# iDC-NEU/NeutronStarLite

Hardware: NVIDIA H100
Metric: gcn_aggregated_edges_per_sec (higher is better)
Workload: dtype f32

## Files before the change

### include/nts_b200.h

```cpp
#ifndef NTS_B200_H
#define NTS_B200_H

#include <stddef.h>
#include <stdint.h>

#ifdef __cplusplus
extern "C" {
#endif

typedef uint32_t nts_vid_t;

int nts_version(void);
const char *nts_last_error(void);
int nts_device_count(void);
int nts_set_device(int device);
int nts_device_sm_count(int *sm_count);
int nts_device_synchronize(void);
int nts_device_reset(void);

void *nts_malloc_device(size_t bytes);
int nts_free_device(void *ptr);
void *nts_malloc_pinned(size_t bytes);
int nts_free_pinned(void *ptr);
void *nts_pinned_device_pointer(void *host_ptr);
int nts_memcpy_h2d(void *dst_device, const void *src_host, size_t bytes, void *stream, int sync);
int nts_memcpy_d2h(void *dst_host, const void *src_device, size_t bytes, void *stream, int sync);
int nts_memcpy_d2d(void *dst_device, const void *src_device, size_t bytes, void *stream);
int nts_zero(void *device_ptr, size_t bytes, void *stream);

void *nts_stream_create(int non_blocking);
int nts_stream_destroy(void *stream);
int nts_stream_synchronize(void *stream);
void *nts_event_create(int with_timing);
int nts_event_destroy(void *event);
int nts_event_record(void *event, void *stream);
int nts_stream_wait_event(void *stream, void *event);
int nts_event_elapsed_ms(void *start, void *stop, float *ms);

int nts_segment_gather_sum(const float *input, float *output, const float *weight,
                           const nts_vid_t *indices, const nts_vid_t *offsets, nts_vid_t index_base,
                           nts_vid_t n_rows, uint64_t n_edges, nts_vid_t feature_size, void *stream);

int nts_gather_by_dst_from_src(const float *input, float *output, const float *weight_forward,
                               const nts_vid_t *row_indices, const nts_vid_t *column_offset,
                               nts_vid_t src_start, nts_vid_t src_end, nts_vid_t dst_start,
                               nts_vid_t dst_end, nts_vid_t edges, nts_vid_t batch_size,
                               nts_vid_t feature_size, int with_weight, void *stream);

int nts_gather_by_src_from_dst(const float *input, float *output, const float *weight_backward,
                               const nts_vid_t *row_offset, const nts_vid_t *column_indices,
                               nts_vid_t src_start, nts_vid_t src_end, nts_vid_t dst_start,
                               nts_vid_t dst_end, nts_vid_t edges, nts_vid_t batch_size,
                               nts_vid_t feature_size, int with_weight, void *stream);

int nts_segment_gather_sum_range(const float *input, float *output, const float *weight, const nts_vid_t *indices,
                                 const nts_vid_t *offsets, const nts_vid_t *slot_of, nts_vid_t index_base,
                                 nts_vid_t n_rows, uint64_t edge_begin, uint64_t edge_end, nts_vid_t feature_size,
                                 void *stream);

int nts_segment_gather_sum_bf16(const void *input, nts_vid_t input_ld, float *output, const float *weight,
                                const nts_vid_t *indices, const nts_vid_t *offsets, nts_vid_t n_rows, uint64_t n_edges,
                                nts_vid_t feature_size, void *stream);

typedef struct nts_gather_plan nts_gather_plan;
int nts_gather_plan_pick_slabs(nts_vid_t gather_rows, uint64_t n_edges, nts_vid_t n_rows, nts_vid_t feature_size,
                               uint64_t l2_budget_bytes );
nts_gather_plan *nts_gather_plan_create_hybrid(const nts_vid_t *offsets, const nts_vid_t *indices,
                                               const float *weight, const nts_vid_t *slot_of, nts_vid_t index_base,
                                               nts_vid_t n_rows, uint64_t n_edges, nts_vid_t gather_rows, int n_slabs,
                                               int n_hub_cols, int n_hub_rows, void *stream);
nts_gather_plan *nts_gather_plan_create_tuned_ex(const nts_vid_t *offsets, const nts_vid_t *indices,
                                                 const float *weight, const nts_vid_t *slot_of, nts_vid_t index_base,
                                                 nts_vid_t n_rows, uint64_t n_edges, nts_vid_t gather_rows,
                                                 nts_vid_t feature_size, int gather_dtype, int run_flags,
                                                 void *stream);
typedef struct nts_plan_part {
  const nts_vid_t *offsets, *indices;
  const float *weight;
  const nts_vid_t *slot_of;
  nts_vid_t index_base, index_add, n_rows, row_add;
  uint64_t n_edges;
} nts_plan_part;
nts_gather_plan *nts_gather_plan_create_parts(const nts_plan_part *parts, int n_parts, nts_vid_t n_rows,
                                              nts_vid_t gather_rows, int n_slabs, nts_vid_t feature_size, void *stream);
float nts_gather_plan_tuned_ms(const nts_gather_plan *plan);
int nts_gather_plan_destroy(nts_gather_plan *plan);
int nts_gather_plan_slabs(const nts_gather_plan *plan);
int nts_gather_plan_hubs(const nts_gather_plan *plan, int *cols, int *rows);
int nts_gather_plan_overlap(const nts_gather_plan *plan);
int nts_gather_plan_set_overlap(nts_gather_plan *plan, int overlap);
uint64_t nts_gather_plan_bytes(const nts_gather_plan *plan);
enum { NTS_PLAN_ACCUMULATE = 0, NTS_PLAN_OVERWRITE = 1, NTS_PLAN_COPY_INPUT = 2 };
int nts_gather_plan_run_ex(nts_gather_plan *plan, const float *input, nts_vid_t input_ld, float *output,
                           nts_vid_t feature_size, int flags, void *stream);
int nts_gather_plan_last_launch(const nts_gather_plan *plan, int *launches, int *grid, int *k, int *u, int *outv);
enum { NTS_DTYPE_F32 = 0, NTS_DTYPE_BF16 = 1 };
int nts_gather_plan_run_bf16_ex(nts_gather_plan *plan, const void *input, int input_dtype, nts_vid_t input_ld,
                                float *output, nts_vid_t feature_size, int flags, void *stream);
int nts_gather_plan_set_tuning(int u, int min_blocks, int edges_per_warp);
int nts_gather_plan_set_variant(int variant);

int nts_segment_gather_sum_slots(const float *input, float *output, const float *weight,
                                 const nts_vid_t *indices, const nts_vid_t *offsets,
                                 const nts_vid_t *slot_of, nts_vid_t n_rows, uint64_t n_edges,
                                 nts_vid_t feature_size, void *stream);

int nts_segment_gather_sum_heads(const float *input, float *output, const float *weight,
                                 const nts_vid_t *indices, const nts_vid_t *offsets, const nts_vid_t *slot_of,
                                 nts_vid_t index_base, nts_vid_t n_rows, uint64_t n_edges,
                                 nts_vid_t feature_size, nts_vid_t heads, void *stream);

int nts_aggregate_set_variant(int variant, int edges_per_warp);
int nts_aggregate_last_launch(int *grid, int *block, int *smem_bytes, int *variant);
int nts_aggregate_last_shape(int *vec, int *k, int *u, int *min_blocks, int *tiles);
uint64_t nts_kernel_launch_count(void);

int nts_scatter_src_mirror_to_msg(float *message, const float *src_mirror_feature,
                                  const nts_vid_t *row_indices, const nts_vid_t *column_offset,
                                  const nts_vid_t *mirror_index, nts_vid_t batch_size,
                                  nts_vid_t feature_size, void *stream);
int nts_gather_msg_to_src_mirror(float *src_mirror_feature, const float *message,
                                 const nts_vid_t *row_indices, const nts_vid_t *column_offset,
                                 const nts_vid_t *mirror_index, nts_vid_t batch_size,
                                 nts_vid_t feature_size, void *stream);
int nts_scatter_dst_to_msg(float *message, const float *dst_feature, const nts_vid_t *row_indices,
                           const nts_vid_t *column_offset, nts_vid_t batch_size,
                           nts_vid_t feature_size, void *stream);
int nts_gather_msg_to_dst(float *dst_feature, const float *message, const nts_vid_t *row_indices,
                          const nts_vid_t *column_offset, nts_vid_t batch_size,
                          nts_vid_t feature_size, void *stream);
int nts_edge_softmax_forward(float *msg_output, const float *msg_input, float *msg_cached,
                             const nts_vid_t *row_indices, const nts_vid_t *column_offset,
                             nts_vid_t batch_size, nts_vid_t feature_size, void *stream);
int nts_edge_softmax_backward(float *msg_input_grad, const float *msg_output_grad,
                              const float *msg_cached, const nts_vid_t *row_indices,
                              const nts_vid_t *column_offset, nts_vid_t batch_size,
                              nts_vid_t feature_size, void *stream);
int nts_scatter_grad_back_to_message(const float *input, float *message_grad,
                                     const nts_vid_t *row_indices, const nts_vid_t *column_offset,
                                     nts_vid_t batch_size, nts_vid_t feature_size, void *stream);

int nts_aggregate_dst_fuse_weight_backward(float *mirror_grad, float *edge_weight_grad,
                                           const float *mirror, const float *edge_weight,
                                           const float *dst_grad, const nts_vid_t *row_indices,
                                           const nts_vid_t *column_offset,
                                           const nts_vid_t *mirror_index, nts_vid_t batch_size,
                                           nts_vid_t feature_size, void *stream);
int nts_aggregate_dst_fuse_weight_backward_heads(float *mirror_grad, float *edge_weight_grad,
                                                 const float *mirror, const float *edge_weight,
                                                 const float *dst_grad, const nts_vid_t *row_indices,
                                                 const nts_vid_t *column_offset,
                                                 const nts_vid_t *mirror_index, nts_vid_t batch_size,
                                                 nts_vid_t feature_size, nts_vid_t heads, void *stream);

int nts_gat_softmax_stats(float *seg_max, float *seg_sum, const float *src_score, const float *dst_score,
                          const nts_vid_t *row_indices, const nts_vid_t *column_offset,
                          const nts_vid_t *mirror_index, nts_vid_t batch_size, nts_vid_t heads,
                          float negative_slope, void *stream);
int nts_gat_fused_aggregate_forward(const float *mirror, float *output, const float *src_score,
                                    const float *dst_score, const float *seg_max, const float *seg_sum,
                                    const nts_vid_t *row_indices, const nts_vid_t *column_offset,
                                    const nts_vid_t *mirror_index, nts_vid_t batch_size, uint64_t n_edges,
                                    nts_vid_t feature_size, nts_vid_t heads, float negative_slope, void *stream);
int nts_gat_fused_aggregate_backward(float *mirror_grad, float *src_score_grad, float *dst_score_grad,
                                     const float *mirror, const float *src_score, const float *dst_score,
                                     const float *seg_max, const float *seg_sum, const float *out_dot_grad,
                                     const float *dst_grad, const nts_vid_t *row_indices,
                                     const nts_vid_t *column_offset, const nts_vid_t *mirror_index,
                                     nts_vid_t batch_size, nts_vid_t feature_size, nts_vid_t heads,
                                     float negative_slope, void *stream);
int nts_gat_fused_aggregate_backward_two_pass(float *mirror_grad, float *src_score_grad, float *dst_score_grad,
                                              float *dst_pack, const float *mirror, const float *src_score,
                                              const float *dst_score, const float *seg_max, const float *seg_sum,
                                              const float *out_dot_grad, const float *dst_grad,
                                              const nts_vid_t *row_indices, const nts_vid_t *column_offset,
                                              const nts_vid_t *mirror_index, const nts_vid_t *slot_row_offset,
                                              const nts_vid_t *slot_column_indices, nts_vid_t batch_size,
                                              nts_vid_t mirror_size, nts_vid_t feature_size, nts_vid_t heads,
                                              float negative_slope, void *stream);
int nts_gat_fused_aggregate_forward_bf16(const void *mirror, float *output, const float *src_score,
                                         const float *dst_score, const float *seg_max, const float *seg_sum,
                                         const nts_vid_t *row_indices, const nts_vid_t *column_offset,
                                         const nts_vid_t *mirror_index, nts_vid_t batch_size, uint64_t n_edges,
                                         nts_vid_t feature_size, nts_vid_t ld, nts_vid_t heads, float negative_slope,
                                         void *stream);
int nts_gat_fused_aggregate_backward_two_pass_bf16(float *mirror_grad, float *src_score_grad, float *dst_score_grad,
                                                   float *dst_pack, const void *mirror, const float *src_score,
                                                   const float *dst_score, const float *seg_max, const float *seg_sum,
                                                   const float *out_dot_grad, const void *dst_grad,
                                                   const nts_vid_t *row_indices, const nts_vid_t *column_offset,
                                                   const nts_vid_t *mirror_index, const nts_vid_t *slot_row_offset,
                                                   const nts_vid_t *slot_column_indices, nts_vid_t batch_size,
                                                   nts_vid_t mirror_size, nts_vid_t feature_size, nts_vid_t ld,
                                                   nts_vid_t heads, float negative_slope, void *stream);
int nts_rows_to_bf16(const void *src, int src_dtype, nts_vid_t lds, void *dst, nts_vid_t n_rows, nts_vid_t feature_size,
                     nts_vid_t ld, void *stream);

int nts_deserialize_records(float *mirror, const float *records, nts_vid_t n_records,
                            nts_vid_t feature_size, nts_vid_t partition_start,
                            nts_vid_t partition_end, void *stream);
int nts_aggregate_records(float *aggregate, const float *records, nts_vid_t n_records,
                          nts_vid_t feature_size, nts_vid_t partition_start,
                          nts_vid_t partition_end, void *stream);

int nts_gather_rows(float *dst, const float *src, const nts_vid_t *rows, nts_vid_t n_rows,
                    nts_vid_t feature_size, void *stream);
int nts_gather_rows_sharded(float *dst, const float *const *shards, const nts_vid_t *shard_offsets, int n_shards,
                            nts_vid_t shard_pitch, const nts_vid_t *ids, nts_vid_t n, nts_vid_t feature_size,
                            void *stream);
int nts_gather_rows_sharded_bf16(void *dst, int dst_dtype, nts_vid_t dst_ld, const void *const *shards,
                                 const nts_vid_t *shard_offsets, int n_shards, nts_vid_t shard_pitch,
                                 const nts_vid_t *ids, nts_vid_t n, nts_vid_t feature_size, void *stream);
int nts_segment_gather_sum_sharded(float *output, const void *const *shards, int shard_dtype,
                                   const nts_vid_t *shard_offsets, int n_shards, nts_vid_t shard_pitch,
                                   const float *weight, const nts_vid_t *indices, const nts_vid_t *offsets,
                                   nts_vid_t n_rows, uint64_t edge_begin, uint64_t edge_end, nts_vid_t feature_size,
                                   void *stream);
int nts_gat_softmax_stats_sharded(float *seg_max, float *seg_sum, const void *const *score_shards,
                                  const nts_vid_t *shard_offsets, int n_shards, nts_vid_t score_pitch,
                                  const float *dst_score, const nts_vid_t *indices, const nts_vid_t *offsets,
                                  nts_vid_t n_rows, uint64_t edge_begin, uint64_t edge_end, nts_vid_t heads,
                                  float negative_slope, void *stream);
int nts_gat_aggregate_sharded(float *output, const void *const *shards, int shard_dtype,
                              const nts_vid_t *shard_offsets, int n_shards, nts_vid_t shard_pitch,
                              const void *const *score_shards, nts_vid_t score_pitch, const float *dst_score,
                              const float *seg_max, const float *seg_sum, const nts_vid_t *indices,
                              const nts_vid_t *offsets, nts_vid_t n_rows, uint64_t edge_begin, uint64_t edge_end,
                              nts_vid_t feature_size, nts_vid_t heads, float negative_slope, void *stream);
int nts_scatter_add_rows(float *dst, const float *src, const nts_vid_t *rows, nts_vid_t n_rows,
                         nts_vid_t feature_size, void *stream);
int nts_scatter_add_rows_atomic(float *dst, const float *src, const nts_vid_t *rows, nts_vid_t n_rows,
                                nts_vid_t feature_size, void *stream);

int nts_adam_update(float *W, float *M, float *V, const float *grad, uint64_t n, float weight_decay, float beta1,
                    float beta2, float alpha, float epsilon, void *stream);
int nts_embedding_step(float *rows, float *adam_m, float *adam_v, uint32_t *mask, uint32_t *positions,
                       uint32_t *touched, const void *const *outboxes, int n_ranks, nts_vid_t capacity,
                       nts_vid_t row_lo, nts_vid_t row_hi, nts_vid_t pitch, nts_vid_t feature_size,
                       float weight_decay, float beta1, float beta2, float alpha, float epsilon, void *stream);

#define NTS_IPC_HANDLE_BYTES 64
int nts_ipc_get_handle(void *device_ptr, unsigned char handle[NTS_IPC_HANDLE_BYTES]);
void *nts_ipc_open_handle(const unsigned char handle[NTS_IPC_HANDLE_BYTES]);
int nts_ipc_close_handle(void *peer_ptr);
int nts_signal_set(uint32_t *flag, uint32_t value, void *stream);
int nts_signal_wait_geq(const uint32_t *flag, uint32_t value, void *stream);

typedef struct nts_exchange nts_exchange;
typedef struct nts_exchange_chunk {
  const nts_vid_t *column_offset;
  const nts_vid_t *slots;
  const float *weight_forward;
  const nts_vid_t *row_offset_compact;
  const nts_vid_t *column_indices;
  const float *weight_backward;
  uint64_t edges;
} nts_exchange_chunk;
typedef struct nts_exchange_desc {
  int partitions, rank;
  nts_vid_t owned_vertices, dst_start;
  const nts_vid_t *local_column_offset, *local_row_indices, *local_row_offset, *local_column_indices;
  const float *local_weight_forward, *local_weight_backward;
  nts_vid_t local_edges;
  const nts_exchange_chunk *chunks;
  const nts_vid_t *need_count;
  const nts_vid_t *send_count;
  const nts_vid_t *send_rows_all;
  const nts_vid_t *fwd_push_offset;
  const nts_vid_t *bwd_push_offset;
  const nts_vid_t *local_need;
  nts_vid_t local_need_count;
} nts_exchange_desc;

nts_exchange *nts_exchange_create(const nts_exchange_desc *desc);
int nts_exchange_destroy(nts_exchange *ex);
uint64_t nts_exchange_required_floats(const nts_exchange *ex, nts_vid_t feature_size);
uint64_t nts_exchange_required_floats_bf16(const nts_exchange *ex, nts_vid_t feature_size);
uint64_t nts_exchange_capacity_floats(const nts_exchange *ex);
int nts_exchange_release_peers(nts_exchange *ex);
int nts_exchange_reserve(nts_exchange *ex, uint64_t floats_per_buffer, int n_buffers);
int nts_exchange_handles(nts_exchange *ex, unsigned char window_handle[64], unsigned char flags_handle[64]);
int nts_exchange_open_peers(nts_exchange *ex, const unsigned char *window_handles, const unsigned char *flag_handles);
int nts_exchange_forward(nts_exchange *ex, const float *x, float *y, nts_vid_t feature_size, void *stream);
int nts_exchange_backward(nts_exchange *ex, const float *g, float *dx, nts_vid_t feature_size, void *stream);
int nts_exchange_forward_bf16(nts_exchange *ex, const void *x, int x_dtype, float *y, nts_vid_t feature_size,
                              void *stream);
int nts_exchange_backward_bf16(nts_exchange *ex, const float *g, float *dx, nts_vid_t feature_size, void *stream);
int nts_exchange_set_trace(nts_exchange *ex, int enable);
int nts_exchange_last_timeline(nts_exchange *ex, float *ms, int capacity);
int nts_exchange_last_paths(const nts_exchange *ex, int *kind, int *epoch, int *buffer, int *mode,
                            uint32_t *kernel_peers, uint32_t *dma_peers, int *push_vec, uint32_t *plan_chunks,
                            int *bf16_staging);
int nts_exchange_fetch_mirrors(nts_exchange *ex, const float *x, float *mirror, nts_vid_t feature_size, void *stream);
int nts_exchange_return_mirror_grads(nts_exchange *ex, const float *mirror_grad, float *dx, nts_vid_t feature_size,
                                     void *stream);

typedef struct nts_host_chunk {
  const nts_vid_t *column_offset, *row_indices, *row_offset, *column_indices;
  const float *edge_weight_forward, *edge_weight_backward;
  nts_vid_t src_start, src_end, dst_start, dst_end;
  uint64_t edges;
} nts_host_chunk;
typedef struct nts_exchange_plan nts_exchange_plan;
nts_exchange_plan *nts_exchange_plan_create(const nts_host_chunk *chunks, int partitions, int rank);
void nts_exchange_plan_destroy(nts_exchange_plan *plan);
const nts_vid_t *nts_exchange_plan_need(const nts_exchange_plan *plan, int i, nts_vid_t *count);
uint64_t nts_exchange_plan_packed_rows(const nts_exchange_plan *plan);
int nts_exchange_plan_pack_needs(const nts_exchange_plan *plan, nts_vid_t *need_counts, nts_vid_t *need_rows);
int nts_exchange_plan_set_peer_needs(nts_exchange_plan *plan, int j, const nts_vid_t *need_counts,
                                     const nts_vid_t *need_rows);
int nts_exchange_plan_finalize(nts_exchange_plan *plan);
typedef struct nts_exchange_plan_view {
  int partitions, rank;
  nts_vid_t owned_vertices, recv_total, send_total, backward_rows;
  uint64_t remote_edges;
  const nts_vid_t *need_count, *send_count, *peer_bwd_offset;
  const nts_vid_t *fwd_push_offset, *bwd_push_offset;
  const nts_vid_t *remote_column_offset, *remote_slots;
  const float *remote_weight;
  const nts_vid_t *backward_offsets, *backward_indices;
  const float *backward_weight;
  const nts_vid_t *send_rows_all;
} nts_exchange_plan_view;
int nts_exchange_plan_get_view(const nts_exchange_plan *plan, nts_exchange_plan_view *view);
int nts_exchange_plan_chunk(const nts_exchange_plan *plan, int i, const nts_vid_t **slots,
                            const nts_vid_t **row_offset_compact);
typedef struct nts_device_chunk {
  const nts_vid_t *column_offset, *row_indices, *row_offset, *column_indices;
  const float *edge_weight_forward, *edge_weight_backward;
} nts_device_chunk;
nts_exchange *nts_exchange_create_from_plan(nts_exchange_plan *plan, const nts_device_chunk *device_chunks);

int nts_host_degrees(const nts_vid_t *edges_src_dst, uint64_t n_edges, nts_vid_t n_vertices,
                     nts_vid_t *out_degree, nts_vid_t *in_degree);
int nts_host_partition_offsets(const nts_vid_t *edges_src_dst, uint64_t n_edges, nts_vid_t n_vertices,
                               int partitions, nts_vid_t *partition_offset);
int nts_host_chunk_edge_counts(const nts_vid_t *edges_src_dst, uint64_t n_edges,
                               const nts_vid_t *partition_offset, int partitions, int rank,
                               uint64_t *counts);
int nts_host_build_chunk(const nts_vid_t *edges_src_dst, uint64_t n_edges, nts_vid_t n_vertices,
                         const nts_vid_t *partition_offset, int partitions, int rank, int src_partition,
                         const nts_vid_t *out_degree, const nts_vid_t *in_degree,
                         nts_vid_t *column_offset, nts_vid_t *row_indices, float *edge_weight_forward,
                         nts_vid_t *row_offset, nts_vid_t *column_indices, float *edge_weight_backward,
                         unsigned char *source_active);
int nts_host_mirror_index(const nts_vid_t *edges_src_dst, uint64_t n_edges, nts_vid_t n_vertices,
                          const nts_vid_t *partition_offset, int rank, nts_vid_t *mirror_index,
                          nts_vid_t *owned);

typedef struct nts_graph_build nts_graph_build;
enum { NTS_GRAPH_BUILD_DIST = 1 };
enum { NTS_INDEX_I32 = 0, NTS_INDEX_I64 = 1 };
nts_graph_build *nts_graph_build_from_file(const char *path, nts_vid_t n_vertices, int partitions, int rank,
                                           const nts_vid_t *partition_offset, uint64_t block_edges, int flags,
                                           void *stream);
nts_graph_build *nts_graph_build_from_device(const void *src, const void *dst, int index_dtype, uint64_t n_edges,
                                             nts_vid_t n_vertices, int partitions, int rank,
                                             const nts_vid_t *partition_offset, const void *out_degree,
                                             const void *in_degree, int flags, void *stream);
int nts_graph_build_info(const nts_graph_build *build, nts_vid_t *partition_offset, uint64_t *chunk_edges,
                         nts_vid_t *owned_mirrors, uint64_t *scratch_peak_bytes, double *pass_seconds);
int nts_graph_build_export_chunk(const nts_graph_build *build, int i, nts_vid_t *column_offset, nts_vid_t *row_indices,
                                 float *edge_weight_forward, nts_vid_t *row_offset, nts_vid_t *column_indices,
                                 float *edge_weight_backward, unsigned char *source_active, void *stream);
int nts_graph_build_export_dist(const nts_graph_build *build, nts_vid_t *mirror_index, nts_vid_t *column_offset,
                                nts_vid_t *row_indices, void *stream);
int nts_graph_build_export_degrees(const nts_graph_build *build, nts_vid_t *out_degree, nts_vid_t *in_degree,
                                   void *stream);
int nts_graph_build_destroy(nts_graph_build *build);

#define NTS_SAMPLER_INCLUDE_DST 1u
typedef struct nts_sampler nts_sampler;
typedef struct nts_sample_hop_view {
  nts_vid_t n_dst, n_src;
  uint64_t n_edges;
  const nts_vid_t *dst;
  const nts_vid_t *column_offset;
  const nts_vid_t *row_indices;
  const nts_vid_t *row_global;
  const float *weight;
  const nts_vid_t *src;
  const nts_vid_t *row_offset;
  const nts_vid_t *column_indices;
  const float *weight_backward;
} nts_sample_hop_view;
nts_sampler *nts_sampler_create(const nts_vid_t *column_offset, const nts_vid_t *row_indices, const float *edge_weight,
                                nts_vid_t n_vertices, uint64_t n_edges, nts_vid_t max_seeds, int hops,
                                const int *fanout, void *stream);
nts_sampler *nts_sampler_create_ex(const nts_vid_t *column_offset, const nts_vid_t *row_indices,
                                   const float *edge_weight, nts_vid_t n_vertices, uint64_t n_edges,
                                   nts_vid_t max_seeds, int hops, const int *fanout, uint32_t flags, void *stream);
nts_sampler *nts_sampler_create_sharded(const nts_vid_t *const *column_offsets, const nts_vid_t *const *row_indices,
                                        const float *const *edge_weights, const nts_vid_t *shard_offsets,
                                        int n_shards, nts_vid_t max_seeds, int hops, const int *fanout,
                                        uint32_t flags, void *stream);
int nts_sampler_sample(nts_sampler *sampler, const nts_vid_t *seeds, nts_vid_t n_seeds, uint64_t seed, uint64_t step,
                       void *stream);
int nts_sampler_hop_view(const nts_sampler *sampler, int hop, nts_sample_hop_view *view);
int nts_sampler_hop_dst_pos(const nts_sampler *sampler, int hop, const nts_vid_t **dst_pos);
uint64_t nts_sampler_bytes(const nts_sampler *sampler);
int nts_sampler_destroy(nts_sampler *sampler);
int nts_sample_transpose(const nts_vid_t *column_offset, const nts_vid_t *row_indices, const float *weight,
                         nts_vid_t n_dst, nts_vid_t n_src, uint64_t n_edges, nts_vid_t *row_offset,
                         nts_vid_t *column_indices, float *weight_backward, void *stream);

int nts_merge_chunk_csc(const nts_vid_t *const *column_offsets, const nts_vid_t *const *row_indices,
                        const float *const *edge_weights, int n_chunks, nts_vid_t n_dst, uint64_t n_edges,
                        nts_vid_t *column_offset, nts_vid_t *row_indices_out, float *edge_weight_out, void *stream);

int nts_host_read_feature_label_mask(const char *feature_path, const char *label_path, const char *mask_path,
                                     nts_vid_t feature_size, nts_vid_t v_begin, nts_vid_t v_end, float *features,
                                     int64_t *labels, int32_t *masks);
int nts_host_read_feature_binary(const char *path, nts_vid_t feature_size, nts_vid_t v_begin, nts_vid_t v_end,
                                 float *features);

#ifdef __cplusplus
}
#endif
#endif
```

### neutronstarlite_b200/_lib.py

```python
from __future__ import annotations

import ctypes as C
import os
import re

import numpy as np
import torch

PKG = os.path.dirname(os.path.abspath(__file__))
ROOT = os.path.dirname(PKG)
LIB_PATH = os.path.join(PKG, "lib", "libnts_b200.so")
HEADER = os.path.join(ROOT, "include", "nts_b200.h")

_vp = C.c_void_p
_u32 = C.c_uint32
_u64 = C.c_uint64
_int = C.c_int
_sz = C.c_size_t

SIGNATURES = {
    "nts_version": (_int, []),
    "nts_last_error": (C.c_char_p, []),
    "nts_device_count": (_int, []),
    "nts_set_device": (_int, [_int]),
    "nts_device_sm_count": (_int, [C.POINTER(_int)]),
    "nts_device_synchronize": (_int, []),
    "nts_device_reset": (_int, []),
    "nts_malloc_device": (_vp, [_sz]),
    "nts_free_device": (_int, [_vp]),
    "nts_malloc_pinned": (_vp, [_sz]),
    "nts_free_pinned": (_int, [_vp]),
    "nts_pinned_device_pointer": (_vp, [_vp]),
    "nts_memcpy_h2d": (_int, [_vp, _vp, _sz, _vp, _int]),
    "nts_memcpy_d2h": (_int, [_vp, _vp, _sz, _vp, _int]),
    "nts_memcpy_d2d": (_int, [_vp, _vp, _sz, _vp]),
    "nts_zero": (_int, [_vp, _sz, _vp]),
    "nts_stream_create": (_vp, [_int]),
    "nts_stream_destroy": (_int, [_vp]),
    "nts_stream_synchronize": (_int, [_vp]),
    "nts_event_create": (_vp, [_int]),
    "nts_event_destroy": (_int, [_vp]),
    "nts_event_record": (_int, [_vp, _vp]),
    "nts_stream_wait_event": (_int, [_vp, _vp]),
    "nts_event_elapsed_ms": (_int, [_vp, _vp, C.POINTER(C.c_float)]),
    "nts_segment_gather_sum": (_int, [_vp, _vp, _vp, _vp, _vp, _u32, _u32, _u64, _u32, _vp]),
    "nts_gather_by_dst_from_src": (_int, [_vp, _vp, _vp, _vp, _vp, _u32, _u32, _u32, _u32, _u32, _u32, _u32, _int, _vp]),
    "nts_gather_by_src_from_dst": (_int, [_vp, _vp, _vp, _vp, _vp, _u32, _u32, _u32, _u32, _u32, _u32, _u32, _int, _vp]),
    "nts_segment_gather_sum_range": (_int, [_vp, _vp, _vp, _vp, _vp, _vp, _u32, _u32, _u64, _u64, _u32, _vp]),
    "nts_segment_gather_sum_bf16": (_int, [_vp, _u32, _vp, _vp, _vp, _vp, _u32, _u64, _u32, _vp]),
    "nts_segment_gather_sum_sharded": (_int, [_vp, _vp, _int, _vp, _int, _u32, _vp, _vp, _vp, _u32, _u64, _u64, _u32,
                                              _vp]),
    "nts_gat_softmax_stats_sharded": (_int, [_vp, _vp, _vp, _vp, _int, _u32, _vp, _vp, _vp, _u32, _u64, _u64, _u32,
                                             C.c_float, _vp]),
    "nts_gat_aggregate_sharded": (_int, [_vp, _vp, _int, _vp, _int, _u32, _vp, _u32, _vp, _vp, _vp, _vp, _vp, _u32,
                                         _u64, _u64, _u32, _u32, C.c_float, _vp]),
    "nts_gather_plan_pick_slabs": (_int, [_u32, _u64, _u32, _u32, _u64]),
    "nts_gather_plan_create_hybrid": (_vp, [_vp, _vp, _vp, _vp, _u32, _u32, _u64, _u32, _int, _int, _int, _vp]),
    "nts_gather_plan_create_parts": (_vp, [_vp, _int, _u32, _u32, _int, _u32, _vp]),
    "nts_gather_plan_tuned_ms": (C.c_float, [_vp]),
    "nts_gather_plan_destroy": (_int, [_vp]),
    "nts_gather_plan_slabs": (_int, [_vp]),
    "nts_gather_plan_hubs": (_int, [_vp, C.POINTER(_int), C.POINTER(_int)]),
    "nts_gather_plan_overlap": (_int, [_vp]),
    "nts_gather_plan_set_overlap": (_int, [_vp, _int]),
    "nts_gather_plan_bytes": (_u64, [_vp]),
    "nts_gather_plan_run_ex": (_int, [_vp, _vp, _u32, _vp, _u32, _int, _vp]),
    "nts_gather_plan_run_bf16_ex": (_int, [_vp, _vp, _int, _u32, _vp, _u32, _int, _vp]),
    "nts_gather_plan_create_tuned_ex": (_vp, [_vp, _vp, _vp, _vp, _u32, _u32, _u64, _u32, _u32, _int, _int, _vp]),
    "nts_gather_plan_last_launch": (_int, [_vp] + [C.POINTER(_int)] * 5),
    "nts_gather_plan_set_tuning": (_int, [_int, _int, _int]),
    "nts_gather_plan_set_variant": (_int, [_int]),
    "nts_segment_gather_sum_slots": (_int, [_vp, _vp, _vp, _vp, _vp, _vp, _u32, _u64, _u32, _vp]),
    "nts_segment_gather_sum_heads": (_int, [_vp, _vp, _vp, _vp, _vp, _vp, _u32, _u32, _u64, _u32, _u32, _vp]),
    "nts_aggregate_set_variant": (_int, [_int, _int]),
    "nts_aggregate_last_launch": (_int, [C.POINTER(_int)] * 4),
    "nts_aggregate_last_shape": (_int, [C.POINTER(_int)] * 5),
    "nts_kernel_launch_count": (_u64, []),
    "nts_scatter_src_mirror_to_msg": (_int, [_vp, _vp, _vp, _vp, _vp, _u32, _u32, _vp]),
    "nts_gather_msg_to_src_mirror": (_int, [_vp, _vp, _vp, _vp, _vp, _u32, _u32, _vp]),
    "nts_scatter_dst_to_msg": (_int, [_vp, _vp, _vp, _vp, _u32, _u32, _vp]),
    "nts_gather_msg_to_dst": (_int, [_vp, _vp, _vp, _vp, _u32, _u32, _vp]),
    "nts_edge_softmax_forward": (_int, [_vp, _vp, _vp, _vp, _vp, _u32, _u32, _vp]),
    "nts_edge_softmax_backward": (_int, [_vp, _vp, _vp, _vp, _vp, _u32, _u32, _vp]),
    "nts_scatter_grad_back_to_message": (_int, [_vp, _vp, _vp, _vp, _u32, _u32, _vp]),
    "nts_aggregate_dst_fuse_weight_backward": (_int, [_vp, _vp, _vp, _vp, _vp, _vp, _vp, _vp, _u32, _u32, _vp]),
    "nts_aggregate_dst_fuse_weight_backward_heads": (_int, [_vp] * 8 + [_u32, _u32, _u32, _vp]),
    "nts_gat_softmax_stats": (_int, [_vp] * 7 + [_u32, _u32, C.c_float, _vp]),
    "nts_gat_fused_aggregate_forward": (_int, [_vp] * 9 + [_u32, _u64, _u32, _u32, C.c_float, _vp]),
    "nts_gat_fused_aggregate_backward": (_int, [_vp] * 13 + [_u32, _u32, _u32, C.c_float, _vp]),
    "nts_gat_fused_aggregate_backward_two_pass": (_int, [_vp] * 16 + [_u32, _u32, _u32, _u32, C.c_float, _vp]),
    "nts_gat_fused_aggregate_forward_bf16": (_int, [_vp] * 9 + [_u32, _u64, _u32, _u32, _u32, C.c_float, _vp]),
    "nts_gat_fused_aggregate_backward_two_pass_bf16": (_int, [_vp] * 16 + [_u32] * 5 + [C.c_float, _vp]),
    "nts_rows_to_bf16": (_int, [_vp, _int, _u32, _vp, _u32, _u32, _u32, _vp]),
    "nts_deserialize_records": (_int, [_vp, _vp, _u32, _u32, _u32, _u32, _vp]),
    "nts_aggregate_records": (_int, [_vp, _vp, _u32, _u32, _u32, _u32, _vp]),
    "nts_gather_rows": (_int, [_vp, _vp, _vp, _u32, _u32, _vp]),
    "nts_gather_rows_sharded": (_int, [_vp, _vp, _vp, _int, _u32, _vp, _u32, _u32, _vp]),
    "nts_gather_rows_sharded_bf16": (_int, [_vp, _int, _u32, _vp, _vp, _int, _u32, _vp, _u32, _u32, _vp]),
    "nts_scatter_add_rows": (_int, [_vp, _vp, _vp, _u32, _u32, _vp]),
    "nts_scatter_add_rows_atomic": (_int, [_vp, _vp, _vp, _u32, _u32, _vp]),
    "nts_ipc_get_handle": (_int, [_vp, C.c_char_p]),
    "nts_ipc_open_handle": (_vp, [C.c_char_p]),
    "nts_ipc_close_handle": (_int, [_vp]),
    "nts_adam_update": (_int, [_vp, _vp, _vp, _vp, _u64] + [C.c_float] * 5 + [_vp]),
    "nts_embedding_step": (_int, [_vp] * 7 + [_int, _u32, _u32, _u32, _u32, _u32] + [C.c_float] * 5 + [_vp]),
    "nts_signal_set": (_int, [_vp, _u32, _vp]),
    "nts_signal_wait_geq": (_int, [_vp, _u32, _vp]),
    "nts_host_degrees": (_int, [_vp, _u64, _u32, _vp, _vp]),
    "nts_host_partition_offsets": (_int, [_vp, _u64, _u32, _int, _vp]),
    "nts_host_chunk_edge_counts": (_int, [_vp, _u64, _vp, _int, _int, _vp]),
    "nts_host_build_chunk": (_int, [_vp, _u64, _u32, _vp, _int, _int, _int, _vp, _vp, _vp, _vp, _vp, _vp, _vp, _vp, _vp]),
    "nts_host_mirror_index": (_int, [_vp, _u64, _u32, _vp, _int, _vp, _vp]),
    "nts_host_read_feature_label_mask": (_int, [C.c_char_p, C.c_char_p, C.c_char_p, _u32, _u32, _u32, _vp, _vp, _vp]),
    "nts_host_read_feature_binary": (_int, [C.c_char_p, _u32, _u32, _u32, _vp]),
    "nts_graph_build_from_file": (_vp, [C.c_char_p, _u32, _int, _int, _vp, _u64, _int, _vp]),
    "nts_graph_build_from_device": (_vp, [_vp, _vp, _int, _u64, _u32, _int, _int, _vp, _vp, _vp, _int, _vp]),
    "nts_graph_build_info": (_int, [_vp] * 6),
    "nts_graph_build_export_chunk": (_int, [_vp, _int] + [_vp] * 8),
    "nts_graph_build_export_dist": (_int, [_vp] * 5),
    "nts_graph_build_export_degrees": (_int, [_vp] * 4),
    "nts_graph_build_destroy": (_int, [_vp]),
}



class ExchangeChunk(C.Structure):
    _fields_ = [
        ("column_offset", _vp), ("slots", _vp), ("weight_forward", _vp), ("row_offset_compact", _vp),
        ("column_indices", _vp), ("weight_backward", _vp), ("edges", _u64),
    ]


class ExchangeDesc(C.Structure):
    _fields_ = [
        ("partitions", _int), ("rank", _int), ("owned_vertices", _u32), ("dst_start", _u32),
        ("local_column_offset", _vp), ("local_row_indices", _vp), ("local_row_offset", _vp),
        ("local_column_indices", _vp), ("local_weight_forward", _vp), ("local_weight_backward", _vp),
        ("local_edges", _u32),
        ("chunks", C.POINTER(ExchangeChunk)),
        ("need_count", C.POINTER(_u32)), ("send_count", C.POINTER(_u32)),
        ("send_rows_all", _vp), ("fwd_push_offset", C.POINTER(_u32)), ("bwd_push_offset", C.POINTER(_u32)),
        ("local_need", _vp), ("local_need_count", _u32),
    ]


class DeviceChunk(C.Structure):
    _fields_ = [
        ("column_offset", _vp), ("row_indices", _vp), ("row_offset", _vp), ("column_indices", _vp),
        ("edge_weight_forward", _vp), ("edge_weight_backward", _vp),
    ]


SIGNATURES.update({
    "nts_exchange_create": (_vp, [C.POINTER(ExchangeDesc)]),
    "nts_exchange_destroy": (_int, [_vp]),
    "nts_exchange_required_floats": (_u64, [_vp, _u32]),
    "nts_exchange_capacity_floats": (_u64, [_vp]),
    "nts_exchange_release_peers": (_int, [_vp]),
    "nts_exchange_reserve": (_int, [_vp, _u64, _int]),
    "nts_exchange_handles": (_int, [_vp, C.c_char_p, C.c_char_p]),
    "nts_exchange_open_peers": (_int, [_vp, C.c_char_p, C.c_char_p]),
    "nts_exchange_forward": (_int, [_vp, _vp, _vp, _u32, _vp]),
    "nts_exchange_backward": (_int, [_vp, _vp, _vp, _u32, _vp]),
    "nts_exchange_forward_bf16": (_int, [_vp, _vp, _int, _vp, _u32, _vp]),
    "nts_exchange_backward_bf16": (_int, [_vp, _vp, _vp, _u32, _vp]),
    "nts_exchange_required_floats_bf16": (_u64, [_vp, _u32]),
    "nts_exchange_set_trace": (_int, [_vp, _int]),
    "nts_exchange_last_timeline": (_int, [_vp, C.POINTER(C.c_float), _int]),
    "nts_exchange_last_paths": (_int, [_vp] + [C.POINTER(_int)] * 4 + [C.POINTER(_u32)] * 2 +
                                [C.POINTER(_int), C.POINTER(_u32), C.POINTER(_int)]),
    "nts_exchange_fetch_mirrors": (_int, [_vp, _vp, _vp, _u32, _vp]),
    "nts_exchange_return_mirror_grads": (_int, [_vp, _vp, _vp, _u32, _vp]),
})



class HostChunk(C.Structure):
    _fields_ = [
        ("column_offset", _vp), ("row_indices", _vp), ("row_offset", _vp), ("column_indices", _vp),
        ("edge_weight_forward", _vp), ("edge_weight_backward", _vp),
        ("src_start", _u32), ("src_end", _u32), ("dst_start", _u32), ("dst_end", _u32), ("edges", _u64),
    ]


class ExchangePlanView(C.Structure):
    _fields_ = [
        ("partitions", _int), ("rank", _int),
        ("owned_vertices", _u32), ("recv_total", _u32), ("send_total", _u32), ("backward_rows", _u32),
        ("remote_edges", _u64),
        ("need_count", C.POINTER(_u32)), ("send_count", C.POINTER(_u32)), ("peer_bwd_offset", C.POINTER(_u32)),
        ("fwd_push_offset", C.POINTER(_u32)), ("bwd_push_offset", C.POINTER(_u32)),
        ("remote_column_offset", C.POINTER(_u32)), ("remote_slots", C.POINTER(_u32)),
        ("remote_weight", C.POINTER(C.c_float)),
        ("backward_offsets", C.POINTER(_u32)), ("backward_indices", C.POINTER(_u32)),
        ("backward_weight", C.POINTER(C.c_float)),
        ("send_rows_all", C.POINTER(_u32)),
    ]


SIGNATURES.update({
    "nts_exchange_plan_create": (_vp, [C.POINTER(HostChunk), _int, _int]),
    "nts_exchange_plan_destroy": (None, [_vp]),
    "nts_exchange_plan_need": (C.POINTER(_u32), [_vp, _int, C.POINTER(_u32)]),
    "nts_exchange_plan_packed_rows": (_u64, [_vp]),
    "nts_exchange_plan_pack_needs": (_int, [_vp, _vp, _vp]),
    "nts_exchange_plan_set_peer_needs": (_int, [_vp, _int, _vp, _vp]),
    "nts_exchange_plan_finalize": (_int, [_vp]),
    "nts_exchange_plan_get_view": (_int, [_vp, C.POINTER(ExchangePlanView)]),
    "nts_exchange_plan_chunk": (_int, [_vp, _int, C.POINTER(C.POINTER(_u32)), C.POINTER(C.POINTER(_u32))]),
    "nts_exchange_create_from_plan": (_vp, [_vp, C.POINTER(DeviceChunk)]),
})


class SampleHopView(C.Structure):
    _fields_ = [
        ("n_dst", _u32), ("n_src", _u32), ("n_edges", _u64),
        ("dst", _vp), ("column_offset", _vp), ("row_indices", _vp), ("row_global", _vp), ("weight", _vp),
        ("src", _vp), ("row_offset", _vp), ("column_indices", _vp), ("weight_backward", _vp),
    ]


SIGNATURES.update({
    "nts_sampler_create": (_vp, [_vp, _vp, _vp, _u32, _u64, _u32, _int, C.POINTER(_int), _vp]),
    "nts_sampler_create_ex": (_vp, [_vp, _vp, _vp, _u32, _u64, _u32, _int, C.POINTER(_int), _u32, _vp]),
    "nts_sampler_sample": (_int, [_vp, _vp, _u32, _u64, _u64, _vp]),
    "nts_sampler_hop_view": (_int, [_vp, _int, C.POINTER(SampleHopView)]),
    "nts_sampler_hop_dst_pos": (_int, [_vp, _int, C.POINTER(_vp)]),
    "nts_sampler_bytes": (_u64, [_vp]),
    "nts_sampler_destroy": (_int, [_vp]),
    "nts_sample_transpose": (_int, [_vp, _vp, _vp, _u32, _u32, _u64, _vp, _vp, _vp, _vp]),
    "nts_sampler_create_sharded": (_vp, [C.POINTER(_vp), C.POINTER(_vp), C.POINTER(_vp), C.POINTER(_u32), _int, _u32,
                                         _int, C.POINTER(_int), _u32, _vp]),
    "nts_merge_chunk_csc": (_int, [C.POINTER(_vp), C.POINTER(_vp), C.POINTER(_vp), _int, _u32, _u64, _vp, _vp, _vp,
                                   _vp]),
})

_lib = None


class NtsError(RuntimeError):
    pass


def header_symbols():
    text = open(HEADER).read()
    text = re.sub(r"/\*.*?\*/", "", text, flags=re.S)
    return sorted(set(re.findall(r"\b(nts_[a-z0-9_]+)\s*\(", text)))


def load():
    global _lib
    if _lib is not None:
        return _lib
    if not os.path.exists(LIB_PATH):
        raise NtsError("libnts_b200.so not found at %s - run `python -m neutronstarlite_b200.build` "
                       "(there is no CPU fallback)" % LIB_PATH)
    lib = C.CDLL(LIB_PATH, mode=C.RTLD_GLOBAL)
    for name, (res, args) in SIGNATURES.items():
        fn = getattr(lib, name)
        fn.restype = res
        fn.argtypes = args
    _lib = lib
    return lib


def last_error():
    return load().nts_last_error().decode(errors="replace")


def check(rc, what=""):
    if rc != 0:
        raise NtsError("libnts_b200 %s failed (rc=%d): %s" % (what, rc, last_error()))


def call(name, *args):
    rc = getattr(load(), name)(*args)
    check(rc, name)


def checked(handle, what):
    if not handle:
        raise NtsError("%s failed: %s" % (what, last_error()))
    return handle


def stream(device=None):
    return torch.cuda.current_stream(device).cuda_stream


class _DeviceArray:

    def __init__(self, ptr, n, typestr):
        self.__cuda_array_interface__ = {"shape": (int(n),), "typestr": typestr, "data": (int(ptr), False),
                                         "version": 2, "strides": None}


_TYPESTR = {torch.int32: "<i4", torch.float32: "<f4"}


def borrowed(ptr, n, dtype, device):
    if n == 0:
        return torch.empty(0, dtype=dtype, device=device)
    return torch.as_tensor(_DeviceArray(ptr, n, _TYPESTR[dtype]), device=device)


def device_ids(ids, bound, device, name, what):
    if torch.is_tensor(ids) and ids.is_cuda:
        if ids.dtype.is_floating_point or ids.dtype.is_complex or ids.dtype == torch.bool:
            raise NtsError("%s must be an integer tensor, not %s" % (name, ids.dtype))
        if ids.numel() and (int(ids.min()) < 0 or int(ids.max()) >= bound):
            raise NtsError("%s must be in [0, %d)" % (what, bound))
        return ids.reshape(-1).to(device=device, dtype=torch.int32).contiguous()
    a = np.asarray(ids.numpy() if torch.is_tensor(ids) else ids).reshape(-1).astype(np.int64)
    if a.size and (a.min() < 0 or a.max() >= bound):
        raise NtsError("%s must be in [0, %d)" % (what, bound))
    return torch.from_numpy(a.astype(np.int32)).to(device)
```

### neutronstarlite_b200/csrc/nts_plan.cu

```cuda
#include <cub/cub.cuh>
#include <cuda_bf16.h>

#include <algorithm>
#include <type_traits>
#include <vector>

#include "nts_common.cuh"

struct nts_gather_plan {
  uint32_t n_rows = 0;
  uint64_t n_edges = 0;
  uint32_t gather_rows = 0;
  int slabs = 1;
  uint32_t slab_rows = 0;
  uint2 *pairs = nullptr;
  uint32_t *voff = nullptr;
  std::vector<uint64_t> slab_edge;
  float *workspace = nullptr;
  size_t workspace_floats = 0;
  __nv_bfloat16 *workspace_bf16 = nullptr;
  size_t workspace_bf16_elems = 0;
  int hub_cols = 0, hub_rows = 0;
  uint32_t *hub_col_ids = nullptr;
  uint32_t *hub_row_ids = nullptr;
  uint32_t lda_c = 0, lda_r = 0;
  float *dense = nullptr;
  size_t dense_floats = 0;
  int overlap = 0;
  int last_grid = 0, last_launches = 0, last_k = 0, last_u = 0, last_outv = 0;
  float tuned_ms = 0.f;
};

namespace nts {

static int g_plan_u = 0, g_plan_minb = 0, g_plan_q = 0, g_plan_variant = 0;

__device__ __forceinline__ uint32_t plan_gathered_row(const nts_plan_part &pt, uint32_t e) {
  const uint32_t id = __ldg(pt.indices + e);
  return (pt.slot_of ? __ldg(pt.slot_of + id) : id - pt.index_base) + pt.index_add;
}

constexpr uint32_t kNoHub = 0xffffffffu;

template <class KeyT>
__global__ void plan_keys_kernel(nts_plan_part pt, uint32_t e_off, uint32_t n_rows, uint32_t slab_rows, uint32_t slabs,
                                 const uint32_t *__restrict__ col_slot, const uint32_t *__restrict__ row_slot,
                                 uint32_t lda_c, uint64_t dc_cells, uint32_t lda_r, KeyT *__restrict__ key,
                                 uint32_t *__restrict__ val) {
  for (uint64_t e = (uint64_t)blockIdx.x * blockDim.x + threadIdx.x; e < pt.n_edges; e += (uint64_t)gridDim.x * blockDim.x) {
    const uint32_t r = find_row(pt.offsets, pt.n_rows, (uint32_t)e) + pt.row_add;
    const uint32_t g = plan_gathered_row(pt, (uint32_t)e);
    uint32_t s = g / slab_rows;
    if (s >= slabs)
      s = slabs - 1;
    KeyT k = (KeyT)s * n_rows + r;
    if constexpr (sizeof(KeyT) == 8) {
      const uint64_t n_keys = (uint64_t)slabs * n_rows;
      const uint32_t cs = __ldg(col_slot + g), rs = __ldg(row_slot + r);
      if (cs != kNoHub)
        k = n_keys + (uint64_t)cs * lda_c + r;
      else if (rs != kNoHub)
        k = n_keys + dc_cells + (uint64_t)g * lda_r + rs;
    }
    key[e_off + e] = k;
    val[e_off + e] = e_off + (uint32_t)e;
  }
}

__global__ void plan_pairs_kernel(const uint32_t *__restrict__ perm, const nts_plan_part *__restrict__ parts,
                                  uint32_t n_edges, uint2 *__restrict__ pairs) {
  for (uint64_t i = (uint64_t)blockIdx.x * blockDim.x + threadIdx.x; i < n_edges; i += (uint64_t)gridDim.x * blockDim.x) {
    uint32_t e = perm ? __ldg(perm + i) : (uint32_t)i;
    const nts_plan_part *pt = parts;
    for (; e >= pt->n_edges; pt++)
      e -= (uint32_t)pt->n_edges;
    const float wt = pt->weight ? __ldg(pt->weight + e) : 1.f;
    pairs[i] = make_uint2(plan_gathered_row(*pt, e), __float_as_uint(wt));
  }
}

template <class KeyT>
__global__ void plan_offsets_kernel(const KeyT *__restrict__ sorted_key, uint32_t n_edges, uint32_t n_keys,
                                    uint32_t *__restrict__ voff) {
  for (uint64_t k = (uint64_t)blockIdx.x * blockDim.x + threadIdx.x; k <= n_keys; k += (uint64_t)gridDim.x * blockDim.x) {
    uint32_t lo = 0, hi = n_edges;
    while (lo < hi) {
      uint32_t mid = lo + ((hi - lo) >> 1);
      if (__ldg(sorted_key + mid) < (KeyT)k)
        lo = mid + 1;
      else
        hi = mid;
    }
    voff[k] = lo;
  }
}

__global__ void plan_ref_count_kernel(const uint32_t *__restrict__ idx, const uint32_t *__restrict__ slot_of,
                                      uint32_t base, uint32_t n_edges, uint32_t *__restrict__ cnt) {
  for (uint64_t e = (uint64_t)blockIdx.x * blockDim.x + threadIdx.x; e < n_edges; e += (uint64_t)gridDim.x * blockDim.x) {
    const uint32_t id = __ldg(idx + e);
    atomicAdd(cnt + (slot_of ? __ldg(slot_of + id) : id - base), 1u);
  }
}

__global__ void plan_cell_sum_kernel(const uint64_t *__restrict__ cell_key, const uint32_t *__restrict__ run_start,
                                     const uint32_t *__restrict__ run_len, uint32_t n_runs,
                                     const uint32_t *__restrict__ perm, const float *__restrict__ w, uint64_t n_keys,
                                     float *__restrict__ dense) {
  const uint32_t lane = threadIdx.x & 31;
  for (uint64_t run = ((uint64_t)blockIdx.x * blockDim.x + threadIdx.x) >> 5; run < n_runs;
       run += ((uint64_t)gridDim.x * blockDim.x) >> 5) {
    const uint32_t b = __ldg(run_start + run), n = __ldg(run_len + run);
    float s = 0.f;
    for (uint32_t j = lane; j < n; j += 32)
      s += w ? __ldg(w + __ldg(perm + b + j)) : 1.f;
#pragma unroll
    for (int o = 16; o > 0; o >>= 1)
      s += __shfl_xor_sync(0xffffffffu, s, o);
    if (lane == 0)
      dense[__ldg(cell_key + run) - n_keys] = s;
  }
}

__global__ void pad_rows_kernel(const float *__restrict__ src, uint32_t lds, float *__restrict__ dst, uint32_t n_rows,
                                uint32_t F, uint32_t ld) {
  const uint64_t total = (uint64_t)n_rows * ld;
  for (uint64_t i = (uint64_t)blockIdx.x * blockDim.x + threadIdx.x; i < total; i += (uint64_t)gridDim.x * blockDim.x) {
    const uint64_t r = i / ld;
    const uint32_t c = (uint32_t)(i - r * ld);
    dst[i] = c < F ? __ldg(src + r * lds + c) : 0.f;
  }
}

template <class S>
__global__ void bf16_rows_kernel(const S *__restrict__ src, uint32_t lds, uint4 *__restrict__ dst, uint32_t n_rows,
                                 uint32_t F, uint32_t ld) {
  const uint32_t ld8 = ld / 8;
  const uint64_t total = (uint64_t)n_rows * ld8;
  for (uint64_t i = (uint64_t)blockIdx.x * blockDim.x + threadIdx.x; i < total; i += (uint64_t)gridDim.x * blockDim.x) {
    const uint64_t r = i / ld8;
    const uint32_t c = (uint32_t)(i - r * ld8) * 8;
    const S *s = src + r * lds;
    uint32_t w[4];
#pragma unroll
    for (int j = 0; j < 4; j++) {
      const uint32_t c0 = c + 2 * j, c1 = c0 + 1;
      if constexpr (std::is_same<S, float>::value) {
        const __nv_bfloat162 h = __floats2bfloat162_rn(c0 < F ? __ldg(s + c0) : 0.f, c1 < F ? __ldg(s + c1) : 0.f);
        w[j] = *reinterpret_cast<const uint32_t *>(&h);
      } else {
        const uint16_t *u = reinterpret_cast<const uint16_t *>(s);
        w[j] = (c0 < F ? (uint32_t)__ldg(u + c0) : 0u) | ((c1 < F ? (uint32_t)__ldg(u + c1) : 0u) << 16);
      }
    }
    dst[i] = make_uint4(w[0], w[1], w[2], w[3]);
  }
}

constexpr int kPlanWarps = 8;

template <int OUTV, bool ATOMIC>
__device__ __forceinline__ void flush_chunk(float *__restrict__ orow, uint32_t col, uint32_t F, float4 a) {
  if constexpr (OUTV == 4) {
    float4 *p = reinterpret_cast<float4 *>(orow + col);
    if constexpr (ATOMIC) {
      asm volatile("red.global.add.v4.f32 [%0], {%1, %2, %3, %4};" ::"l"(p), "f"(a.x), "f"(a.y), "f"(a.z), "f"(a.w)
                   : "memory");
    } else {
      float4 o = *p;
      o.x += a.x, o.y += a.y, o.z += a.z, o.w += a.w;
      *p = o;
    }
  } else if constexpr (OUTV == 2) {
    float2 *p = reinterpret_cast<float2 *>(orow + col);
    if constexpr (ATOMIC) {
      asm volatile("red.global.add.v2.f32 [%0], {%1, %2};" ::"l"(p), "f"(a.x), "f"(a.y) : "memory");
      if (col + 2 < F)
        asm volatile("red.global.add.v2.f32 [%0], {%1, %2};" ::"l"(p + 1), "f"(a.z), "f"(a.w) : "memory");
    } else {
      float2 o = p[0];
      o.x += a.x, o.y += a.y;
      p[0] = o;
      if (col + 2 < F) {
        float2 o1 = p[1];
        o1.x += a.z, o1.y += a.w;
        p[1] = o1;
      }
    }
  } else {
    const float v[4] = {a.x, a.y, a.z, a.w};
#pragma unroll
    for (int i = 0; i < 4; i++)
      if (col + i < F) {
        if constexpr (ATOMIC)
          atomicAdd(orow + col + i, v[i]);
        else
          orow[col + i] += v[i];
      }
  }
}

template <class T> struct GatherT;
template <> struct GatherT<float> {
  using chunk = float4;
  static constexpr int V = 4;
  __device__ static __forceinline__ void widen(const float4 &c, float (&v)[4]) {
    v[0] = c.x, v[1] = c.y, v[2] = c.z, v[3] = c.w;
  }
};
template <> struct GatherT<__nv_bfloat16> {
  using chunk = uint4;
  static constexpr int V = 8;
  __device__ static __forceinline__ void widen(const uint4 &c, float (&v)[8]) {
    const uint32_t u[4] = {c.x, c.y, c.z, c.w};
#pragma unroll
    for (int i = 0; i < 4; i++) {
      v[2 * i] = __uint_as_float(u[i] << 16);
      v[2 * i + 1] = __uint_as_float(u[i] & 0xffff0000u);
    }
  }
};

template <class T, int K, int U, int OUTV, int G>
__device__ __forceinline__ void planned_gather_body(unsigned char *smem_raw, uint32_t vblock,
                                                    const typename GatherT<T>::chunk *__restrict__ in, uint32_t ldc,
                                                    float *__restrict__ out, uint32_t F,
                                                    const uint2 *__restrict__ pairs, const uint32_t *__restrict__ off,
                                                    uint32_t n_rows, uint32_t e_begin, uint32_t e_end, uint32_t Q,
                                                    uint32_t tiles, uint32_t tile_vecs) {
  static_assert(G == 1 || K == 1, "virtual warps are for rows narrower than a warp");
  using Chunk = typename GatherT<T>::chunk;
  constexpr int V = GatherT<T>::V;
  constexpr uint32_t GS = 32 / G;
  const uint32_t lane = threadIdx.x & (GS - 1);
  const uint32_t vwarp_in_block = threadIdx.x / GS;
  const uint64_t gwarp = (uint64_t)vblock * (kPlanWarps * G) + vwarp_in_block;
  const uint32_t tile = (uint32_t)(gwarp % tiles);
  const uint64_t q = gwarp / tiles;
  const uint64_t e0_64 = e_begin + q * (uint64_t)Q;

  uint64_t *bar = reinterpret_cast<uint64_t *>(smem_raw);
  uint2 *s_pair = reinterpret_cast<uint2 *>(smem_raw + 16);
  uint32_t cta_e_base = 0, bulk_bytes = 0;
  {
    const uint64_t cta_w0 = (uint64_t)vblock * (kPlanWarps * G);
    const uint64_t first_q = cta_w0 / tiles;
    const uint64_t last_q = (cta_w0 + kPlanWarps * G - 1) / tiles;
    uint64_t ce0 = e_begin + first_q * (uint64_t)Q;
    uint64_t ce1 = e_begin + (last_q + 1) * (uint64_t)Q;
    if (ce1 > e_end)
      ce1 = e_end;
    if (ce0 < ce1) {
      cta_e_base = (uint32_t)(ce0 & ~1ull);
      const uint32_t n_el = (uint32_t)(ce1 - cta_e_base);
      bulk_bytes = (n_el * 8u) & ~15u;
      if (threadIdx.x == 0) {
        mbar_init(bar, 1);
        asm volatile("fence.mbarrier_init.release.cluster;" ::: "memory");
        if (n_el & 1u)
          s_pair[n_el - 1] = __ldg(pairs + cta_e_base + n_el - 1);
      }
      __syncthreads();
      if (threadIdx.x == 0 && bulk_bytes) {
        mbar_expect_tx(bar, bulk_bytes);
        bulk_g2s(s_pair, pairs + cta_e_base, bulk_bytes, bar);
      }
    }
  }
  if (e0_64 >= e_end)
    return;
  const uint32_t e0 = (uint32_t)e0_64;
  const uint32_t e1 = (e0_64 + Q < e_end) ? e0 + Q : e_end;

  const uint32_t c0 = tile * tile_vecs + lane;
  bool act[K];
#pragma unroll
  for (int k = 0; k < K; k++)
    act[k] = (k * GS + lane) < tile_vecs && (c0 + k * GS) < ldc;

  uint32_t row = find_row(off, n_rows, e0);
  uint32_t row_end = __ldg(off + row + 1);
  bool row_started_inside = __ldg(off + row) >= e0;

  float acc[K][V];
#pragma unroll
  for (int k = 0; k < K; k++)
#pragma unroll
    for (int j = 0; j < V; j++)
      acc[k][j] = 0.f;

  auto flush = [&](bool whole) {
    float *orow = out + (size_t)row * F;
#pragma unroll
    for (int k = 0; k < K; k++) {
#pragma unroll
      for (int h = 0; h < V; h += 4) {
        const uint32_t col = (c0 + k * GS) * V + h;
        const float4 a = make_float4(acc[k][h], acc[k][h + 1], acc[k][h + 2], acc[k][h + 3]);
        if (act[k] && col < F) {
          if (whole)
            flush_chunk<OUTV, false>(orow, col, F, a);
          else
            flush_chunk<OUTV, true>(orow, col, F, a);
        }
      }
#pragma unroll
      for (int j = 0; j < V; j++)
        acc[k][j] = 0.f;
    }
  };
  auto advance = [&](uint32_t ee) {
    flush(row_started_inside);
    do {
      row++;
      row_end = __ldg(off + row + 1);
    } while (ee >= row_end);
    row_started_inside = true;
  };

  if (bulk_bytes)
    mbar_wait(bar, 0);

  const uint2 *sp = s_pair - cta_e_base;
  uint32_t e = e0;
  auto fma_chunk = [&](int k, float w, const Chunk &c) {
    float x[V];
    GatherT<T>::widen(c, x);
#pragma unroll
    for (int j = 0; j < V; j++)
      acc[k][j] = fmaf(w, x[j], acc[k][j]);
  };
  for (; e + U <= e1; e += U) {
    Chunk v[U][K];
    float wu[U];
#pragma unroll
    for (int u = 0; u < U; u++) {
      const uint2 pr = sp[e + u];
      wu[u] = __uint_as_float(pr.y);
      const Chunk *p = in + (size_t)pr.x * ldc + c0;
#pragma unroll
      for (int k = 0; k < K; k++)
        if (act[k])
          v[u][k] = __ldg(p + k * GS);
    }
#pragma unroll
    for (int u = 0; u < U; u++) {
      if (e + u >= row_end)
        advance(e + u);
#pragma unroll
      for (int k = 0; k < K; k++)
        if (act[k])
          fma_chunk(k, wu[u], v[u][k]);
    }
  }
  for (; e < e1; e++) {
    const uint2 pr = sp[e];
    const float wj = __uint_as_float(pr.y);
    const Chunk *p = in + (size_t)pr.x * ldc + c0;
    Chunk v1[K];
#pragma unroll
    for (int k = 0; k < K; k++)
      if (act[k])
        v1[k] = __ldg(p + k * GS);
    if (e >= row_end)
      advance(e);
#pragma unroll
    for (int k = 0; k < K; k++)
      if (act[k])
        fma_chunk(k, wj, v1[k]);
  }
  flush(row_started_inside && row_end <= e1);
}

template <class T, int K, int U, int OUTV, int MINB, int G = 1>
__global__ void __launch_bounds__(kPlanWarps * 32, MINB)
    planned_gather_sum_kernel(const typename GatherT<T>::chunk *__restrict__ in, uint32_t ldc, float *__restrict__ out,
                              uint32_t F, const uint2 *__restrict__ pairs, const uint32_t *__restrict__ off,
                              uint32_t n_rows, uint32_t e_begin, uint32_t e_end, uint32_t Q, uint32_t tiles,
                              uint32_t tile_vecs) {
  extern __shared__ __align__(16) unsigned char smem_raw[];
  planned_gather_body<T, K, U, OUTV, G>(smem_raw, blockIdx.x, in, ldc, out, F, pairs, off, n_rows, e_begin, e_end, Q,
                                        tiles, tile_vecs);
}

struct PlanShape;
template <int K, int STAGES, int OUTV, int MINB>
__global__ void __launch_bounds__(kPlanWarps * 32, MINB)
    planned_gather_sum_tma_kernel(const float4 *__restrict__ in, uint32_t ld4, float *__restrict__ out, uint32_t F,
                                  const uint2 *__restrict__ pairs, const uint32_t *__restrict__ off, uint32_t n_rows,
                                  uint32_t e_begin, uint32_t e_end, uint32_t Q, uint32_t tiles, uint32_t tile_vecs,
                                  uint32_t pair_bytes) {
  const uint32_t lane = threadIdx.x & 31;
  const uint32_t warp_in_block = threadIdx.x >> 5;
  const uint64_t gwarp = (uint64_t)blockIdx.x * kPlanWarps + warp_in_block;
  const uint32_t tile = (uint32_t)(gwarp % tiles);
  const uint64_t q = gwarp / tiles;
  const uint64_t e0_64 = e_begin + q * (uint64_t)Q;

  extern __shared__ __align__(16) unsigned char smem_raw[];
  uint64_t *bar = reinterpret_cast<uint64_t *>(smem_raw);
  uint2 *s_pair = reinterpret_cast<uint2 *>(smem_raw + 16);
  const uint32_t ring_bytes = 8u * STAGES + 8u * (STAGES & 1) + STAGES * tile_vecs * 16u;
  unsigned char *ring = smem_raw + 16 + pair_bytes + (size_t)warp_in_block * ring_bytes;
  uint64_t *sbar = reinterpret_cast<uint64_t *>(ring);
  float4 *sbuf = reinterpret_cast<float4 *>(ring + 8u * STAGES + 8u * (STAGES & 1));
  uint32_t cta_e_base = 0, bulk_bytes = 0;
  {
    const uint64_t cta_w0 = (uint64_t)blockIdx.x * kPlanWarps;
    const uint64_t first_q = cta_w0 / tiles;
    const uint64_t last_q = (cta_w0 + kPlanWarps - 1) / tiles;
    uint64_t ce0 = e_begin + first_q * (uint64_t)Q;
    uint64_t ce1 = e_begin + (last_q + 1) * (uint64_t)Q;
    if (ce1 > e_end)
      ce1 = e_end;
    if (lane == 0)
      for (int s = 0; s < STAGES; s++)
        mbar_init(sbar + s, 1);
    if (ce0 < ce1) {
      cta_e_base = (uint32_t)(ce0 & ~1ull);
      const uint32_t n_el = (uint32_t)(ce1 - cta_e_base);
      bulk_bytes = (n_el * 8u) & ~15u;
      if (threadIdx.x == 0) {
        mbar_init(bar, 1);
        if (n_el & 1u)
          s_pair[n_el - 1] = __ldg(pairs + cta_e_base + n_el - 1);
      }
    }
    asm volatile("fence.mbarrier_init.release.cluster;" ::: "memory");
    __syncthreads();
    if (threadIdx.x == 0 && bulk_bytes) {
      mbar_expect_tx(bar, bulk_bytes);
      bulk_g2s(s_pair, pairs + cta_e_base, bulk_bytes, bar);
    }
  }
  if (e0_64 >= e_end)
    return;
  const uint32_t e0 = (uint32_t)e0_64;
  const uint32_t e1 = (e0_64 + Q < e_end) ? e0 + Q : e_end;
  const uint32_t c0 = tile * tile_vecs + lane;
  const uint32_t my_vecs = min(tile_vecs, ld4 - tile * tile_vecs);
  const uint32_t row_bytes = my_vecs * 16u;
  bool act[K];
#pragma unroll
  for (int k = 0; k < K; k++)
    act[k] = (k * 32 + lane) < my_vecs;

  uint32_t row = find_row(off, n_rows, e0);
  uint32_t row_end = __ldg(off + row + 1);
  bool row_started_inside = __ldg(off + row) >= e0;
  float4 acc[K];
#pragma unroll
  for (int k = 0; k < K; k++)
    zero_vec(acc[k]);
  auto flush = [&](bool whole) {
    float *orow = out + (size_t)row * F;
#pragma unroll
    for (int k = 0; k < K; k++) {
      const uint32_t col = (c0 + k * 32) * 4;
      if (act[k] && col < F) {
        if (whole)
          flush_chunk<OUTV, false>(orow, col, F, acc[k]);
        else
          flush_chunk<OUTV, true>(orow, col, F, acc[k]);
      }
      zero_vec(acc[k]);
    }
  };
  auto advance = [&](uint32_t ee) {
    flush(row_started_inside);
    do {
      row++;
      row_end = __ldg(off + row + 1);
    } while (ee >= row_end);
    row_started_inside = true;
  };
  if (bulk_bytes)
    mbar_wait(bar, 0);
  const uint2 *sp = s_pair - cta_e_base;
  auto issue = [&](uint32_t e, uint32_t stage) {
    const uint32_t src_row = sp[e].x;
    mbar_expect_tx(sbar + stage, row_bytes);
    bulk_g2s(sbuf + (size_t)stage * tile_vecs, in + (size_t)src_row * ld4 + tile * tile_vecs, row_bytes, sbar + stage);
  };
  if (lane == 0)
    for (uint32_t s = 0; s < STAGES && e0 + s < e1; s++)
      issue(e0 + s, s);
  uint32_t stage = 0, parity = 0;
  for (uint32_t e = e0; e < e1; e++) {
    const float w = __uint_as_float(sp[e].y);
    mbar_wait(sbar + stage, parity);
    const float4 *b = sbuf + (size_t)stage * tile_vecs + lane;
    float4 v[K];
#pragma unroll
    for (int k = 0; k < K; k++)
      if (act[k])
        v[k] = b[k * 32];
    if (e >= row_end)
      advance(e);
#pragma unroll
    for (int k = 0; k < K; k++)
      if (act[k])
        fma_vec(acc[k], w, v[k]);
    __syncwarp();
    if (lane == 0 && e + STAGES < e1)
      issue(e + STAGES, stage);
    if (++stage == STAGES) {
      stage = 0;
      parity ^= 1u;
    }
  }
  flush(row_started_inside && row_end <= e1);
}

template <int K, int STAGES, int OUTV, int MINB>
static int launch_planned_tma(nts_gather_plan *pl, const PlanShape &sh, const float4 *in, uint32_t ld4, float *out,
                              uint32_t F, uint32_t Q, cudaStream_t st);

struct PlanShape {
  int k, u, outv, minb, g;
  uint32_t tiles, tile_vecs;
};

template <class T, int K, int U, int OUTV, int MINB, int G = 1>
static int launch_planned(nts_gather_plan *pl, const PlanShape &sh, const T *in_rows, uint32_t ldc, float *out,
                          uint32_t F, uint32_t Q, cudaStream_t st) {
  auto kern = planned_gather_sum_kernel<T, K, U, OUTV, MINB, G>;
  const auto *in = reinterpret_cast<const typename GatherT<T>::chunk *>(in_rows);
  const size_t smem = 16 + ((size_t)kPlanWarps * G * Q + 4) * 8;
  NTS_CUDA_OK(cudaFuncSetAttribute(kern, cudaFuncAttributeMaxDynamicSharedMemorySize, (int)smem));
  pl->last_launches = 0;
  for (int s = 0; s < pl->slabs; s++) {
    const uint64_t eb = pl->slab_edge[s], ee = pl->slab_edge[s + 1];
    if (ee <= eb)
      continue;
    const uint64_t quanta = (ee - eb + Q - 1) / Q;
    const uint64_t blocks = (quanta * sh.tiles + kPlanWarps * G - 1) / (kPlanWarps * G);
    NTS_ARG_CHECK(blocks <= 0x7fffffffull, "aggregation grid too large");
    kern<<<(unsigned)blocks, kPlanWarps * 32, smem, st>>>(in, ldc, out, F, pl->pairs, pl->voff + (size_t)s * pl->n_rows,
                                                          pl->n_rows, (uint32_t)eb, (uint32_t)ee, Q, sh.tiles,
                                                          sh.tile_vecs);
    NTS_LAUNCH_CHECK();
    pl->last_grid = (int)blocks;
    pl->last_launches++;
  }
  return 0;
}

template <int K, int STAGES, int OUTV, int MINB>
static int launch_planned_tma(nts_gather_plan *pl, const PlanShape &sh, const float4 *in, uint32_t ld4, float *out,
                              uint32_t F, uint32_t Q, cudaStream_t st) {
  auto kern = planned_gather_sum_tma_kernel<K, STAGES, OUTV, MINB>;
  const uint32_t pair_bytes = (kPlanWarps * Q + 4) * 8;
  const uint32_t ring_bytes = 8u * STAGES + 8u * (STAGES & 1) + STAGES * sh.tile_vecs * 16u;
  const size_t smem = 16 + pair_bytes + (size_t)kPlanWarps * ring_bytes;
  NTS_ARG_CHECK(smem <= 227 * 1024, "row-staging ring does not fit shared memory");
  NTS_CUDA_OK(cudaFuncSetAttribute(kern, cudaFuncAttributeMaxDynamicSharedMemorySize, (int)smem));
  pl->last_launches = 0;
  for (int s = 0; s < pl->slabs; s++) {
    const uint64_t eb = pl->slab_edge[s], ee = pl->slab_edge[s + 1];
    if (ee <= eb)
      continue;
    const uint64_t quanta = (ee - eb + Q - 1) / Q;
    const uint64_t blocks = (quanta * sh.tiles + kPlanWarps - 1) / kPlanWarps;
    NTS_ARG_CHECK(blocks <= 0x7fffffffull, "aggregation grid too large");
    kern<<<(unsigned)blocks, kPlanWarps * 32, smem, st>>>(in, ld4, out, F, pl->pairs, pl->voff + (size_t)s * pl->n_rows,
                                                          pl->n_rows, (uint32_t)eb, (uint32_t)ee, Q, sh.tiles,
                                                          sh.tile_vecs, pair_bytes);
    NTS_LAUNCH_CHECK();
    pl->last_grid = (int)blocks;
    pl->last_launches++;
  }
  return 0;
}

#define NTS_PLAN_TMA_CASE(K_, S_, B_)                                                                               \
  if (sh.k == K_ && stages == S_ && sh.minb == B_) {                                                                \
    if (sh.outv == 4)                                                                                               \
      return launch_planned_tma<K_, S_, 4, B_>(pl, sh, in4, ld4, out, F, Q, st);                                    \
    if (sh.outv == 2)                                                                                               \
      return launch_planned_tma<K_, S_, 2, B_>(pl, sh, in4, ld4, out, F, Q, st);                                    \
    return launch_planned_tma<K_, S_, 1, B_>(pl, sh, in4, ld4, out, F, Q, st);                                      \
  }

#define NTS_PLAN_CASE_G(U_, B_, G_)                                                                                 \
  if (sh.k == 1 && sh.u == U_ && sh.minb == B_ && sh.g == G_) {                                                     \
    if (sh.outv == 4)                                                                                               \
      return launch_planned<T, 1, U_, 4, B_, G_>(pl, sh, in, ldc, out, F, Q, st);                                   \
    if (sh.outv == 2)                                                                                               \
      return launch_planned<T, 1, U_, 2, B_, G_>(pl, sh, in, ldc, out, F, Q, st);                                   \
    return launch_planned<T, 1, U_, 1, B_, G_>(pl, sh, in, ldc, out, F, Q, st);                                     \
  }

#define NTS_PLAN_CASE(K_, U_, B_)                                                                                   \
  if (sh.k == K_ && sh.u == U_ && sh.minb == B_) {                                                                  \
    if (sh.outv == 4)                                                                                               \
      return launch_planned<T, K_, U_, 4, B_>(pl, sh, in, ldc, out, F, Q, st);                                       \
    if (sh.outv == 2)                                                                                               \
      return launch_planned<T, K_, U_, 2, B_>(pl, sh, in, ldc, out, F, Q, st);                                       \
    return launch_planned<T, K_, U_, 1, B_>(pl, sh, in, ldc, out, F, Q, st);                                         \
  }

constexpr int kHubBM = 128, kHubBN = 128, kHubBK = 16, kHubThreads = 256;

__device__ __forceinline__ void p_cp_async16(void *smem_dst, const void *gmem_src, bool full) {
  asm volatile("cp.async.cg.shared.global [%0], [%1], 16, %2;" ::"r"(smem_u32(smem_dst)), "l"(gmem_src),
               "r"(full ? 16 : 0)
               : "memory");
}

template <int TN, class TB> struct HubSmem {
  static constexpr uint32_t kBN = 16 * TN;
  float As[2][kHubBK][kHubBM];
  TB Bs[2][kHubBK][kBN];
};

template <class TB, int OUTV, bool SPLIT, bool STORE, int TN, int KKU>
__device__ __forceinline__ void hub_gemm_tile(HubSmem<TN, TB> &sm, uint32_t tile, const float *__restrict__ At,
                                              uint32_t lda, uint32_t M, uint32_t k_lo, uint32_t k_hi, uint32_t k_split,
                                              const TB *__restrict__ B, uint32_t ldb,
                                              const uint32_t *__restrict__ colmap, float *__restrict__ out, uint32_t F,
                                              const uint32_t *__restrict__ rowmap, uint32_t m_tiles, uint32_t n_tiles) {
  static_assert(!(SPLIT && STORE), "split-K partials must be added, not stored");
  constexpr bool kBf16 = std::is_same<TB, __nv_bfloat16>::value;
  constexpr uint32_t kBV = 16 / sizeof(TB);
  constexpr uint32_t kBN = HubSmem<TN, TB>::kBN;
  constexpr uint32_t kBChunks = kHubBK * kBN / kBV;
  auto &As = sm.As;
  auto &Bs = sm.Bs;
  const uint32_t t = threadIdx.x;
  const uint32_t n_tile = tile % n_tiles, rest = tile / n_tiles;
  const uint32_t m0 = (rest % m_tiles) * kHubBM, n0 = n_tile * kBN;
  const uint32_t k_begin = k_lo + (rest / m_tiles) * k_split;
  const uint32_t k_end = min(k_hi, k_begin + k_split);
  if (k_begin >= k_end)
    return;
  const uint32_t n_kt = (k_end - k_begin + kHubBK - 1) / kHubBK;

  auto load = [&](uint32_t kt, int buf) {
#pragma unroll
    for (int i = 0; i < 2; i++) {
      const uint32_t c = t + i * kHubThreads, kk = c >> 5, c4 = (c & 31) * 4;
      const uint32_t k = k_begin + kt * kHubBK + kk;
      const bool a_ok = k < k_end && m0 + c4 < lda;
      p_cp_async16(&As[buf][kk][c4], a_ok ? At + (size_t)k * lda + m0 + c4 : At, a_ok);
    }
#pragma unroll
    for (int i = 0; i < (int)((kBChunks + kHubThreads - 1) / kHubThreads); i++) {
      constexpr uint32_t kRowChunks = kBN / kBV;
      const uint32_t c = t + i * kHubThreads, kk = c / kRowChunks, cv = (c % kRowChunks) * kBV;
      if (kBChunks % kHubThreads != 0 && c >= kBChunks)
        break;
      const uint32_t k = k_begin + kt * kHubBK + kk;
      const bool b_ok = k < k_end && n0 + cv < ldb;
      const uint32_t brow = b_ok ? (colmap ? __ldg(colmap + k) : k) : 0;
      p_cp_async16(&Bs[buf][kk][cv], B + (size_t)brow * ldb + (b_ok ? n0 + cv : 0), b_ok);
    }
    asm volatile("cp.async.commit_group;" ::: "memory");
  };
  auto read_b4 = [&](int buf, int kk, uint32_t n) -> float4 {
    if constexpr (kBf16) {
      const uint2 u = *reinterpret_cast<const uint2 *>(&Bs[buf][kk][n]);
      return make_float4(__uint_as_float(u.x << 16), __uint_as_float(u.x & 0xffff0000u), __uint_as_float(u.y << 16),
                         __uint_as_float(u.y & 0xffff0000u));
    } else {
      return *reinterpret_cast<const float4 *>(&Bs[buf][kk][n]);
    }
  };

  const uint32_t tx = t & 15, ty = t >> 4;
  float acc[8][TN];
#pragma unroll
  for (int i = 0; i < 8; i++)
#pragma unroll
    for (int j = 0; j < TN; j++)
      acc[i][j] = 0.f;

  load(0, 0);
  for (uint32_t kt = 0; kt < n_kt; kt++) {
    const int buf = kt & 1;
    if (kt + 1 < n_kt) {
      load(kt + 1, buf ^ 1);
      asm volatile("cp.async.wait_group 1;" ::: "memory");
    } else {
      asm volatile("cp.async.wait_group 0;" ::: "memory");
    }
    __syncthreads();
#pragma unroll(KKU)
    for (int kk = 0; kk < kHubBK; kk++) {
      const float4 a0 = *reinterpret_cast<const float4 *>(&As[buf][kk][ty * 4]);
      const float4 a1 = *reinterpret_cast<const float4 *>(&As[buf][kk][64 + ty * 4]);
      const float a[8] = {a0.x, a0.y, a0.z, a0.w, a1.x, a1.y, a1.z, a1.w};
      float b[TN];
#pragma unroll
      for (int h = 0; h < TN / 4; h++) {
        const float4 bh = read_b4(buf, kk, h * 64 + tx * 4);
        b[4 * h] = bh.x, b[4 * h + 1] = bh.y, b[4 * h + 2] = bh.z, b[4 * h + 3] = bh.w;
      }
#pragma unroll
      for (int i = 0; i < 8; i++)
#pragma unroll
        for (int j = 0; j < TN; j++)
          acc[i][j] = fmaf(a[i], b[j], acc[i][j]);
    }
    __syncthreads();
  }

#pragma unroll
  for (int i = 0; i < 8; i++) {
    const uint32_t m = m0 + (i >> 2) * 64 + ty * 4 + (i & 3);
    if (m >= M)
      continue;
    float *orow = out + (size_t)(rowmap ? __ldg(rowmap + m) : m) * F;
#pragma unroll
    for (int j = 0; j < TN / 4; j++) {
      const uint32_t col = n0 + j * 64 + tx * 4;
      const float4 a = make_float4(acc[i][j * 4], acc[i][j * 4 + 1], acc[i][j * 4 + 2], acc[i][j * 4 + 3]);
      if (col < F) {
        if constexpr (STORE)
          store_chunk_checked<OUTV>(orow, col, F, a);
        else
          flush_chunk<OUTV, SPLIT>(orow, col, F, a);
      }
    }
  }
}

template <class TB, int OUTV, bool SPLIT, bool STORE>
__global__ void __launch_bounds__(kHubThreads, 2)
    hub_block_gemm_kernel(const float *__restrict__ At, uint32_t lda, uint32_t M, uint32_t K, uint32_t k_split,
                          const TB *__restrict__ B, uint32_t ldb, const uint32_t *__restrict__ colmap,
                          float *__restrict__ out, uint32_t F, const uint32_t *__restrict__ rowmap, uint32_t m_tiles,
                          uint32_t n_tiles) {
  __shared__ __align__(16) HubSmem<8, TB> sm;
  hub_gemm_tile<TB, OUTV, SPLIT, STORE, 8, kHubBK>(sm, blockIdx.x, At, lda, M, 0, K, k_split, B, ldb, colmap, out, F,
                                                   rowmap, m_tiles, n_tiles);
}

static uint32_t hub_row_k_split(uint32_t K, uint32_t m_tiles, uint32_t n_tiles) {
  const uint64_t want = (uint64_t)sm_count() * 2 * 4;
  const uint64_t splits = (want + (uint64_t)m_tiles * n_tiles - 1) / ((uint64_t)m_tiles * n_tiles);
  const uint32_t k_split = (uint32_t)((K + splits - 1) / splits);
  return std::max<uint32_t>((k_split + kHubBK - 1) / kHubBK * kHubBK, 16 * kHubBK);
}

template <class TB, int OUTV>
static int launch_hub_blocks(nts_gather_plan *pl, const TB *in, uint32_t ldb, float *out, uint32_t F, bool rows,
                             bool overwrite, cudaStream_t st) {
  const uint32_t n_tiles = (F + kHubBN - 1) / kHubBN;
  if (pl->hub_cols) {
    const uint32_t m_tiles = (pl->n_rows + kHubBM - 1) / kHubBM;
    const uint64_t blocks = (uint64_t)m_tiles * n_tiles;
    NTS_ARG_CHECK(blocks <= 0x7fffffffull, "hub column block grid too large");
    auto kern = overwrite ? hub_block_gemm_kernel<TB, OUTV, false, true> : hub_block_gemm_kernel<TB, OUTV, false, false>;
    kern<<<(unsigned)blocks, kHubThreads, 0, st>>>(pl->dense, pl->lda_c, pl->n_rows, (uint32_t)pl->hub_cols,
                                                   (uint32_t)pl->hub_cols, in, ldb, pl->hub_col_ids, out, F, nullptr,
                                                   m_tiles, n_tiles);
    NTS_LAUNCH_CHECK();
  }
  if (pl->hub_rows && rows) {
    const uint32_t m_tiles = (pl->hub_rows + kHubBM - 1) / kHubBM;
    const uint32_t K = pl->gather_rows;
    const uint32_t k_split = hub_row_k_split(K, m_tiles, n_tiles);
    const uint64_t splits = (K + k_split - 1) / k_split;
    hub_block_gemm_kernel<TB, OUTV, true, false><<<(unsigned)(splits * m_tiles * n_tiles), kHubThreads, 0, st>>>(
        pl->dense + (size_t)pl->hub_cols * pl->lda_c, pl->lda_r, (uint32_t)pl->hub_rows, K, k_split, in, ldb, nullptr,
        out, F, pl->hub_row_ids, m_tiles, n_tiles);
    NTS_LAUNCH_CHECK();
  }
  return 0;
}

struct HubRowArgs {
  const float *At;
  uint32_t lda, M;
  uint32_t k_lo, k_hi, k_split;
  const uint32_t *rowmap;
  uint32_t m_tiles, n_tiles, n_gemm;
  uint32_t period;
};

template <class T, int K, int U, int OUTV, int MINB, int G>
__global__ void __launch_bounds__(kPlanWarps * 32, MINB)
    planned_slab_hub_kernel(const typename GatherT<T>::chunk *__restrict__ in, uint32_t ldc, float *__restrict__ out,
                            uint32_t F, const uint2 *__restrict__ pairs, const uint32_t *__restrict__ off,
                            uint32_t n_rows, uint32_t e_begin, uint32_t e_end, uint32_t Q, uint32_t tiles,
                            uint32_t tile_vecs, const HubRowArgs hub) {
  static_assert(kPlanWarps * 32 == kHubThreads, "both bodies run 256 threads");
  constexpr int TN = MINB <= 2 ? 8 : 4;
  extern __shared__ __align__(16) unsigned char smem_raw[];
  const uint32_t b = blockIdx.x, grp = b / hub.period;
  if (grp < hub.n_gemm && b - grp * hub.period == hub.period - 1)
    hub_gemm_tile<T, OUTV, true, false, TN, TN == 8 ? kHubBK : 4>(
        *reinterpret_cast<HubSmem<TN, T> *>(smem_raw), grp, hub.At, hub.lda, hub.M, hub.k_lo, hub.k_hi, hub.k_split,
        reinterpret_cast<const T *>(in), ldc * GatherT<T>::V, nullptr, out, F, hub.rowmap, hub.m_tiles, hub.n_tiles);
  else
    planned_gather_body<T, K, U, OUTV, G>(smem_raw, b - min(grp, hub.n_gemm), in, ldc, out, F, pairs, off, n_rows,
                                          e_begin, e_end, Q, tiles, tile_vecs);
}

template <class T, int K, int U, int OUTV, int MINB, int G = 1>
static int launch_fused(nts_gather_plan *pl, const PlanShape &sh, const T *in_rows, uint32_t ldc, float *out,
                        uint32_t F, uint32_t Q, cudaStream_t st) {
  constexpr int TN = MINB <= 2 ? 8 : 4;
  auto kern = planned_slab_hub_kernel<T, K, U, OUTV, MINB, G>;
  const auto *in = reinterpret_cast<const typename GatherT<T>::chunk *>(in_rows);
  const size_t smem = std::max(16 + ((size_t)kPlanWarps * G * Q + 4) * 8, sizeof(HubSmem<TN, T>));
  NTS_CUDA_OK(cudaFuncSetAttribute(kern, cudaFuncAttributeMaxDynamicSharedMemorySize, (int)smem));
  HubRowArgs hub;
  hub.At = pl->dense + (size_t)pl->hub_cols * pl->lda_c;
  hub.lda = pl->lda_r;
  hub.M = (uint32_t)pl->hub_rows;
  hub.rowmap = pl->hub_row_ids;
  hub.m_tiles = (hub.M + kHubBM - 1) / kHubBM;
  hub.n_tiles = (F + 16 * TN - 1) / (16 * TN);
  hub.k_split = hub_row_k_split(pl->gather_rows, hub.m_tiles, hub.n_tiles);
  pl->last_launches = 0;
  for (int s = 0; s < pl->slabs; s++) {
    hub.k_lo = (uint32_t)std::min<uint64_t>((uint64_t)s * pl->slab_rows, pl->gather_rows);
    hub.k_hi = s + 1 == pl->slabs ? pl->gather_rows
                                  : (uint32_t)std::min<uint64_t>((uint64_t)(s + 1) * pl->slab_rows, pl->gather_rows);
    const uint64_t splits = hub.k_hi > hub.k_lo ? (hub.k_hi - hub.k_lo + hub.k_split - 1) / hub.k_split : 0;
    const uint64_t n_gemm = splits * hub.m_tiles * hub.n_tiles;
    const uint64_t eb = pl->slab_edge[s], ee = pl->slab_edge[s + 1];
    const uint64_t quanta = ee > eb ? (ee - eb + Q - 1) / Q : 0;
    const uint64_t blocks = n_gemm + (quanta * sh.tiles + kPlanWarps * G - 1) / (kPlanWarps * G);
    if (!blocks)
      continue;
    NTS_ARG_CHECK(blocks <= 0x7fffffffull, "aggregation grid too large");
    hub.n_gemm = (uint32_t)n_gemm;
    hub.period = n_gemm ? (uint32_t)(blocks / n_gemm) : 1;
    kern<<<(unsigned)blocks, kPlanWarps * 32, smem, st>>>(in, ldc, out, F, pl->pairs, pl->voff + (size_t)s * pl->n_rows,
                                                          pl->n_rows, (uint32_t)eb, (uint32_t)ee, Q, sh.tiles,
                                                          sh.tile_vecs, hub);
    NTS_LAUNCH_CHECK();
    pl->last_grid = (int)blocks;
    pl->last_launches++;
  }
  return 0;
}

#define NTS_PLAN_FUSED_CASE(K_, U_, B_, G_)                                                                         \
  if (sh.k == K_ && sh.u == U_ && sh.minb == B_ && sh.g == G_) {                                                    \
    if (sh.outv == 4)                                                                                               \
      return launch_fused<T, K_, U_, 4, B_, G_>(pl, sh, in, ldc, out, F, Q, st);                                    \
    if (sh.outv == 2)                                                                                               \
      return launch_fused<T, K_, U_, 2, B_, G_>(pl, sh, in, ldc, out, F, Q, st);                                    \
    return launch_fused<T, K_, U_, 1, B_, G_>(pl, sh, in, ldc, out, F, Q, st);                                      \
  }

template <class T>
static int run_gather(nts_gather_plan *pl, const T *in, uint32_t ld, float *output, uint32_t F, bool overwrite,
                      cudaStream_t st) {
  constexpr bool kBf16 = std::is_same<T, __nv_bfloat16>::value;
  PlanShape sh;
  const uint32_t ldc = ld / GatherT<T>::V;
  const uint32_t chunks = (ldc + 31) / 32;
  const uint32_t kmax = 5;
  sh.tiles = (chunks + kmax - 1) / kmax;
  sh.tile_vecs = (ldc + sh.tiles - 1) / sh.tiles;
  sh.k = (int)((sh.tile_vecs + 31) / 32);
  sh.tiles = (ldc + sh.tile_vecs - 1) / sh.tile_vecs;
  sh.outv = pick_vec(F, output);
  const bool fused = pl->overlap && pl->hub_rows;
  NTS_ARG_CHECK(!fused || g_plan_variant == 0, "the fused slab launches use the register-staging gather (variant 0)");
  if (overwrite && !pl->hub_cols)
    NTS_CUDA_OK(cudaMemsetAsync(output, 0, (size_t)pl->n_rows * F * sizeof(float), st));
  if (pl->hub_cols || pl->hub_rows) {
    const int rc = sh.outv == 4   ? launch_hub_blocks<T, 4>(pl, in, ld, output, F, !fused, overwrite, st)
                   : sh.outv == 2 ? launch_hub_blocks<T, 2>(pl, in, ld, output, F, !fused, overwrite, st)
                                  : launch_hub_blocks<T, 1>(pl, in, ld, output, F, !fused, overwrite, st);
    if (rc)
      return rc;
  }
  sh.g = ldc <= 8 ? 4 : (ldc <= 16 ? 2 : 1);
  if (g_plan_variant == 1 || getenv("NTS_PLAN_NO_SUBWARP"))
    sh.g = 1;
  sh.minb = sh.k >= 3 ? 2 : (sh.k == 2 ? 3 : 4);
  sh.u = sh.k == 4 ? 2 : 4;
  if constexpr (kBf16) {
    sh.minb = sh.k >= 4 ? 2 : (sh.k >= 2 ? 3 : 4);
    sh.u = sh.k == 1 ? 4 : 2;
  }
  {
    static int env_read = 0;
    if (!env_read) {
      env_read = 1;
      if (const char *t = getenv("NTS_PLAN_TUNE"))
        sscanf(t, "%d,%d,%d", &g_plan_u, &g_plan_minb, &g_plan_q);
    }
    if (g_plan_u > 0)
      sh.u = g_plan_u;
    if (g_plan_minb > 0)
      sh.minb = g_plan_minb;
  }
  uint32_t Q = g_plan_q > 0 ? (uint32_t)g_plan_q : 512u / sh.g;
  if (g_plan_q <= 0) {
    const uint64_t per_slab = pl->slab_edge[pl->slabs] / (uint64_t)pl->slabs + 1;
    const uint64_t want_warps = (uint64_t)sm_count() * 64 * sh.g;
    while (Q > 32 && ((per_slab + Q - 1) / Q) * sh.tiles < want_warps)
      Q >>= 1;
  }
  Q = (Q + 31u) & ~31u;
  if (Q * sh.g > 1024)
    Q = (1024 / sh.g) & ~31u;
  pl->last_k = sh.k, pl->last_u = sh.u, pl->last_outv = sh.outv;
  float *out = output;
  if (fused) {
    if constexpr (kBf16) {
      NTS_PLAN_FUSED_CASE(1, 4, 4, 2)
      NTS_PLAN_FUSED_CASE(1, 4, 4, 4)
      NTS_PLAN_FUSED_CASE(1, 4, 4, 1)
      NTS_PLAN_FUSED_CASE(2, 2, 3, 1)
      NTS_PLAN_FUSED_CASE(3, 2, 3, 1)
      NTS_PLAN_FUSED_CASE(4, 2, 2, 1)
      NTS_PLAN_FUSED_CASE(5, 2, 2, 1)
    } else {
      NTS_PLAN_FUSED_CASE(1, 4, 4, 2)
      NTS_PLAN_FUSED_CASE(1, 4, 4, 4)
      NTS_PLAN_FUSED_CASE(1, 4, 4, 1)
      NTS_PLAN_FUSED_CASE(2, 4, 3, 1)
      NTS_PLAN_FUSED_CASE(3, 4, 2, 1)
      NTS_PLAN_FUSED_CASE(4, 2, 2, 1)
      NTS_PLAN_FUSED_CASE(5, 4, 2, 1)
    }
    return fail(-1, "no fused slab/hub-row instantiation for this (chunks, U, occupancy) point", __FILE__, __LINE__);
  }
  if constexpr (kBf16) {
    NTS_PLAN_CASE_G(4, 4, 2)
    NTS_PLAN_CASE_G(4, 4, 4)
    NTS_PLAN_CASE_G(8, 2, 2)
    NTS_PLAN_CASE_G(8, 2, 4)
    if (sh.g != 1)
      return fail(-1, "no BF16 virtual-warp instantiation for this (U, occupancy) point", __FILE__, __LINE__);
    NTS_PLAN_CASE(1, 4, 4)
    NTS_PLAN_CASE(1, 8, 2)
    NTS_PLAN_CASE(2, 2, 3)
    NTS_PLAN_CASE(2, 4, 2)
    NTS_PLAN_CASE(3, 4, 2)
    NTS_PLAN_CASE(3, 2, 3)
    NTS_PLAN_CASE(3, 6, 1)
    NTS_PLAN_CASE(4, 2, 2)
    NTS_PLAN_CASE(4, 4, 2)
    NTS_PLAN_CASE(5, 2, 2)
    return fail(-1, "no BF16 planned-aggregation instantiation for this (chunks, U, occupancy) point", __FILE__,
                __LINE__);
  } else {
  const float4 *in4 = reinterpret_cast<const float4 *>(in);
  const uint32_t ld4 = ldc;
  if (g_plan_variant == 1) {
    const int stages = sh.u >= 8 ? 8 : (sh.u >= 4 ? 4 : 2);
    NTS_PLAN_TMA_CASE(1, 8, 4)
    NTS_PLAN_TMA_CASE(1, 4, 4)
    NTS_PLAN_TMA_CASE(1, 8, 3)
    NTS_PLAN_TMA_CASE(2, 4, 3)
    NTS_PLAN_TMA_CASE(2, 4, 2)
    NTS_PLAN_TMA_CASE(3, 4, 2)
    NTS_PLAN_TMA_CASE(4, 4, 2)
    NTS_PLAN_TMA_CASE(4, 2, 2)
    NTS_PLAN_TMA_CASE(5, 4, 2)
    NTS_PLAN_TMA_CASE(5, 2, 2)
    NTS_PLAN_TMA_CASE(5, 4, 1)
    NTS_PLAN_TMA_CASE(5, 8, 1)
    return fail(-1, "no TMA row-staging instantiation for this (chunks, stages, occupancy) point", __FILE__, __LINE__);
  }
  NTS_PLAN_CASE_G(4, 4, 2)
  NTS_PLAN_CASE_G(4, 4, 4)
  NTS_PLAN_CASE_G(8, 3, 2)
  NTS_PLAN_CASE_G(8, 3, 4)
  if (sh.g != 1)
    return fail(-1, "no virtual-warp instantiation for this (U, occupancy) point", __FILE__, __LINE__);
  NTS_PLAN_CASE(1, 8, 4)
  NTS_PLAN_CASE(1, 4, 4)
  NTS_PLAN_CASE(1, 8, 3)
  NTS_PLAN_CASE(1, 16, 2)
  NTS_PLAN_CASE(2, 4, 3)
  NTS_PLAN_CASE(2, 8, 2)
  NTS_PLAN_CASE(3, 4, 3)
  NTS_PLAN_CASE(3, 4, 2)
  NTS_PLAN_CASE(4, 2, 2)
  NTS_PLAN_CASE(4, 4, 2)
  NTS_PLAN_CASE(5, 2, 2)
  NTS_PLAN_CASE(5, 1, 3)
  NTS_PLAN_CASE(5, 2, 3)
  NTS_PLAN_CASE(5, 4, 1)
  NTS_PLAN_CASE(5, 4, 2)
  return fail(-1, "no planned-aggregation instantiation for this (chunks, U, occupancy) point", __FILE__, __LINE__);
  }
}

template <class E> static int ensure_workspace(E *&ws, size_t &have, size_t elems) {
  if (elems <= have)
    return 0;
  if (ws)
    NTS_CUDA_OK(cudaFree(ws));
  ws = nullptr;
  have = 0;
  NTS_CUDA_OK(cudaMalloc(reinterpret_cast<void **>(&ws), elems * sizeof(E)));
  have = elems;
  return 0;
}

static int run_prologue(nts_gather_plan *pl, const void *input, uint32_t lds, float *output, uint32_t F, int flags,
                        bool *done, cudaStream_t st) {
  *done = true;
  NTS_ARG_CHECK((flags & ~(NTS_PLAN_OVERWRITE | NTS_PLAN_COPY_INPUT)) == 0, "unknown plan run flags");
  if (pl->n_rows == 0 || F == 0)
    return 0;
  if (pl->n_edges == 0) {
    if (flags & NTS_PLAN_OVERWRITE) {
      NTS_ARG_CHECK(output != nullptr, "null output pointer");
      NTS_CUDA_OK(cudaMemsetAsync(output, 0, (size_t)pl->n_rows * F * sizeof(float), st));
    }
    return 0;
  }
  NTS_ARG_CHECK(input && output, "null feature pointer");
  NTS_ARG_CHECK(lds >= F, "row stride below the feature width");
  *done = false;
  return 0;
}

int run_plan(nts_gather_plan *pl, const float *input, uint32_t lds, float *output, uint32_t F, int flags,
             cudaStream_t st) {
  bool done = false;
  if (const int rc = run_prologue(pl, input, lds, output, F, flags, &done, st))
    return rc;
  if (done)
    return 0;
  if (lds % 4 == 0 && aligned_to(input, 16) && !(flags & NTS_PLAN_COPY_INPUT))
    return run_gather<float>(pl, input, lds, output, F, flags & NTS_PLAN_OVERWRITE, st);
  const uint32_t ld = (F + 3u) & ~3u;
  if (const int rc = ensure_workspace(pl->workspace, pl->workspace_floats, (size_t)pl->gather_rows * ld))
    return rc;
  const uint64_t total = (uint64_t)pl->gather_rows * ld;
  const unsigned blocks = (unsigned)std::min<uint64_t>((total + 255) / 256, (uint64_t)sm_count() * 32);
  pad_rows_kernel<<<blocks, 256, 0, st>>>(input, lds, pl->workspace, pl->gather_rows, F, ld);
  NTS_LAUNCH_CHECK();
  return run_gather<float>(pl, pl->workspace, ld, output, F, flags & NTS_PLAN_OVERWRITE, st);
}

int to_bf16_rows(const void *src, int dtype, uint32_t lds, void *dst, uint32_t n_rows, uint32_t F, uint32_t ld,
                 cudaStream_t st) {
  NTS_ARG_CHECK(dtype == NTS_DTYPE_F32 || dtype == NTS_DTYPE_BF16, "input dtype must be NTS_DTYPE_F32 or NTS_DTYPE_BF16");
  NTS_ARG_CHECK(ld % 8 == 0 && ld >= F && lds >= F && aligned_to(dst, 16), "bad BF16 row layout");
  if (!n_rows || !F)
    return 0;
  const uint64_t total = (uint64_t)n_rows * (ld / 8);
  const unsigned blocks = (unsigned)std::min<uint64_t>((total + 255) / 256, (uint64_t)sm_count() * 32);
  uint4 *d = static_cast<uint4 *>(dst);
  if (dtype == NTS_DTYPE_F32)
    bf16_rows_kernel<float><<<blocks, 256, 0, st>>>(static_cast<const float *>(src), lds, d, n_rows, F, ld);
  else
    bf16_rows_kernel<__nv_bfloat16><<<blocks, 256, 0, st>>>(static_cast<const __nv_bfloat16 *>(src), lds, d, n_rows,
                                                            F, ld);
  NTS_LAUNCH_CHECK();
  return 0;
}

int run_plan_bf16(nts_gather_plan *pl, const void *input, int dtype, uint32_t lds, float *output, uint32_t F,
                  cudaStream_t st, int flags) {
  NTS_ARG_CHECK(dtype == NTS_DTYPE_F32 || dtype == NTS_DTYPE_BF16, "input dtype must be NTS_DTYPE_F32 or NTS_DTYPE_BF16");
  NTS_ARG_CHECK(g_plan_variant == 0, "the TMA row-staging variant (nts_gather_plan_set_variant(1)) gathers FP32 rows only");
  bool done = false;
  if (const int rc = run_prologue(pl, input, lds, output, F, flags, &done, st))
    return rc;
  if (done)
    return 0;
  const bool overwrite = flags & NTS_PLAN_OVERWRITE;
  if (dtype == NTS_DTYPE_BF16 && lds % 8 == 0 && aligned_to(input, 16) && !(flags & NTS_PLAN_COPY_INPUT))
    return run_gather<__nv_bfloat16>(pl, static_cast<const __nv_bfloat16 *>(input), lds, output, F, overwrite, st);
  const uint32_t ld = (F + 7u) & ~7u;
  if (const int rc = ensure_workspace(pl->workspace_bf16, pl->workspace_bf16_elems, (size_t)pl->gather_rows * ld))
    return rc;
  if (const int rc = to_bf16_rows(input, dtype, lds, pl->workspace_bf16, pl->gather_rows, F, ld, st))
    return rc;
  return run_gather<__nv_bfloat16>(pl, pl->workspace_bf16, ld, output, F, overwrite, st);
}

static int pick_slabs_for_rows(nts_vid_t gather_rows, uint64_t n_edges, nts_vid_t n_rows, uint64_t row_bytes,
                               uint64_t l2_budget_bytes) {
  if (!l2_budget_bytes)
    l2_budget_bytes = 16ull << 20;
  const uint64_t bytes = (uint64_t)gather_rows * row_bytes;
  uint64_t s = (bytes + l2_budget_bytes - 1) / l2_budget_bytes;
  const uint64_t by_degree = n_rows ? n_edges / ((uint64_t)n_rows * 16ull) : 1;
  if (s > by_degree)
    s = by_degree;
  if (s > 64)
    s = 64;
  return s < 1 ? 1 : (int)s;
}

static bool hub_counts(const nts_vid_t *offsets, const nts_vid_t *indices, const nts_vid_t *slot_of, nts_vid_t base,
                       uint32_t n_rows, uint32_t E, uint32_t gather_rows, std::vector<uint32_t> &col_cnt,
                       std::vector<uint32_t> &seg, cudaStream_t st) {
  uint32_t *cnt = nullptr;
  std::vector<uint32_t> off(n_rows + 1);
  col_cnt.assign(gather_rows, 0);
  const unsigned blocks = (unsigned)std::min<uint64_t>(((uint64_t)E + 255) / 256, (uint64_t)sm_count() * 32);
  bool ok = cudaMalloc(reinterpret_cast<void **>(&cnt), (size_t)gather_rows * 4) == cudaSuccess &&
            cudaMemsetAsync(cnt, 0, (size_t)gather_rows * 4, st) == cudaSuccess;
  if (ok && E) {
    plan_ref_count_kernel<<<blocks, 256, 0, st>>>(indices, slot_of, base, E, cnt);
    count_launch();
  }
  ok = ok && cudaMemcpyAsync(col_cnt.data(), cnt, (size_t)gather_rows * 4, cudaMemcpyDeviceToHost, st) == cudaSuccess &&
       cudaMemcpyAsync(off.data(), offsets, ((size_t)n_rows + 1) * 4, cudaMemcpyDeviceToHost, st) == cudaSuccess &&
       cudaStreamSynchronize(st) == cudaSuccess;
  cudaFree(cnt);
  seg.resize(n_rows);
  for (uint32_t r = 0; r < n_rows; r++)
    seg[r] = off[r + 1] - off[r];
  return ok;
}

static std::vector<uint32_t> top_ids(const std::vector<uint32_t> &cnt, size_t h) {
  std::vector<uint32_t> ids(cnt.size());
  for (size_t i = 0; i < ids.size(); i++)
    ids[i] = (uint32_t)i;
  h = std::min(h, ids.size());
  std::partial_sort(ids.begin(), ids.begin() + h, ids.end(),
                    [&](uint32_t a, uint32_t b) { return cnt[a] != cnt[b] ? cnt[a] > cnt[b] : a < b; });
  ids.resize(h);
  return ids;
}

static nts_gather_plan *refuse_plan(const char *what) {
  fail(-1, what, __FILE__, __LINE__);
  return nullptr;
}

template <class KeyT>
static bool sort_plan(nts_gather_plan *pl, const nts_plan_part *parts, int n_parts, const nts_plan_part *d_parts,
                      int n_hub_cols, int n_hub_rows, cudaStream_t st) {
  constexpr bool hubs = sizeof(KeyT) == 8;
  const uint32_t E = (uint32_t)pl->n_edges, n_rows = pl->n_rows, G = pl->gather_rows;
  const uint64_t n_keys = (uint64_t)pl->slabs * n_rows;
  uint64_t dc_cells = 0;
  uint32_t *d_col_slot = nullptr, *d_row_slot = nullptr, *d_runs = nullptr;
  bool ok = true;
  if (hubs) {
    const nts_plan_part &pt = parts[0];
    std::vector<uint32_t> col_cnt, seg;
    if (!hub_counts(pt.offsets, pt.indices, pt.slot_of, pt.index_base, n_rows, E, G, col_cnt, seg, st))
      return false;
    const std::vector<uint32_t> cols = top_ids(col_cnt, (size_t)n_hub_cols), rows = top_ids(seg, (size_t)n_hub_rows);
    pl->hub_cols = (int)cols.size();
    pl->hub_rows = (int)rows.size();
    pl->lda_c = (n_rows + 3u) & ~3u;
    pl->lda_r = ((uint32_t)pl->hub_rows + 3u) & ~3u;
    dc_cells = (uint64_t)pl->hub_cols * pl->lda_c;
    pl->dense_floats = dc_cells + (pl->hub_rows ? (uint64_t)G * pl->lda_r : 0);
    std::vector<uint32_t> col_slot(G, kNoHub), row_slot(n_rows, kNoHub);
    for (size_t i = 0; i < cols.size(); i++)
      col_slot[cols[i]] = (uint32_t)i;
    for (size_t i = 0; i < rows.size(); i++)
      row_slot[rows[i]] = (uint32_t)i;
    ok = cudaMalloc(reinterpret_cast<void **>(&pl->dense), pl->dense_floats * 4) == cudaSuccess &&
         cudaMalloc(reinterpret_cast<void **>(&pl->hub_col_ids), cols.size() * 4 + 4) == cudaSuccess &&
         cudaMalloc(reinterpret_cast<void **>(&pl->hub_row_ids), rows.size() * 4 + 4) == cudaSuccess &&
         cudaMalloc(reinterpret_cast<void **>(&d_col_slot), (size_t)G * 4 + 4) == cudaSuccess &&
         cudaMalloc(reinterpret_cast<void **>(&d_row_slot), (size_t)n_rows * 4 + 4) == cudaSuccess &&
         cudaMalloc(reinterpret_cast<void **>(&d_runs), 4) == cudaSuccess &&
         cudaMemcpyAsync(pl->hub_col_ids, cols.data(), cols.size() * 4, cudaMemcpyHostToDevice, st) == cudaSuccess &&
         cudaMemcpyAsync(pl->hub_row_ids, rows.data(), rows.size() * 4, cudaMemcpyHostToDevice, st) == cudaSuccess &&
         cudaMemcpyAsync(d_col_slot, col_slot.data(), (size_t)G * 4, cudaMemcpyHostToDevice, st) == cudaSuccess &&
         cudaMemcpyAsync(d_row_slot, row_slot.data(), (size_t)n_rows * 4, cudaMemcpyHostToDevice, st) == cudaSuccess &&
         cudaMemsetAsync(pl->dense, 0, pl->dense_floats * 4, st) == cudaSuccess;
  }
  int bits = 1;
  while (bits < (int)(8 * sizeof(KeyT)) && (1ull << bits) < n_keys + pl->dense_floats)
    bits++;
  KeyT *key_in = nullptr, *key_out = nullptr;
  uint32_t *val_in = nullptr, *val_out = nullptr;
  void *tmp = nullptr;
  size_t tmp_bytes = 0;
  ok = ok && cudaMalloc(reinterpret_cast<void **>(&key_in), (size_t)E * sizeof(KeyT)) == cudaSuccess &&
       cudaMalloc(reinterpret_cast<void **>(&key_out), (size_t)E * sizeof(KeyT)) == cudaSuccess &&
       cudaMalloc(reinterpret_cast<void **>(&val_in), (size_t)E * 4) == cudaSuccess &&
       cudaMalloc(reinterpret_cast<void **>(&val_out), (size_t)E * 4) == cudaSuccess &&
       cub::DeviceRadixSort::SortPairs(nullptr, tmp_bytes, key_in, key_out, val_in, val_out, (int64_t)E, 0, bits, st) ==
           cudaSuccess &&
       cudaMalloc(&tmp, tmp_bytes ? tmp_bytes : 16) == cudaSuccess;
  uint32_t e_off = 0;
  for (int k = 0; k < n_parts && ok; k++) {
    const nts_plan_part &pt = parts[k];
    if (!pt.n_edges)
      continue;
    const unsigned blocks = (unsigned)std::min<uint64_t>((pt.n_edges + 255) / 256, (uint64_t)sm_count() * 32);
    plan_keys_kernel<KeyT><<<blocks, 256, 0, st>>>(pt, e_off, n_rows, pl->slab_rows, (uint32_t)pl->slabs, d_col_slot,
                                                   d_row_slot, pl->lda_c, dc_cells, pl->lda_r, key_in, val_in);
    count_launch();
    e_off += (uint32_t)pt.n_edges;
  }
  ok = ok && cub::DeviceRadixSort::SortPairs(tmp, tmp_bytes, key_in, key_out, val_in, val_out, (int64_t)E, 0, bits,
                                             st) == cudaSuccess;
  if (ok) {
    const unsigned kb = (unsigned)std::min<uint64_t>((n_keys + 256) / 256, (uint64_t)sm_count() * 32);
    plan_offsets_kernel<KeyT><<<kb, 256, 0, st>>>(key_out, E, (uint32_t)n_keys, pl->voff);
    count_launch();
    std::vector<uint32_t> h(pl->slabs + 1);
    ok = cudaStreamSynchronize(st) == cudaSuccess;
    for (int s = 0; s <= pl->slabs && ok; s++)
      ok = cudaMemcpy(&h[s], pl->voff + (size_t)s * n_rows, 4, cudaMemcpyDeviceToHost) == cudaSuccess;
    for (int s = 0; s <= pl->slabs; s++)
      pl->slab_edge[s] = h[s];
  }
  const uint32_t n_res = (uint32_t)pl->slab_edge[pl->slabs], n_dense = E - n_res;
  if (ok && n_res) {
    const unsigned blocks = (unsigned)std::min<uint64_t>(((uint64_t)n_res + 255) / 256, (uint64_t)sm_count() * 32);
    plan_pairs_kernel<<<blocks, 256, 0, st>>>(val_out, d_parts, n_res, pl->pairs);
    count_launch();
  }
  if constexpr (hubs) {
    if (ok && n_dense) {
      uint32_t n_runs = 0;
      size_t b1 = 0, b2 = 0;
      ok = cub::DeviceRunLengthEncode::Encode(nullptr, b1, key_out + n_res, key_in, val_in, d_runs, (int64_t)n_dense,
                                              st) == cudaSuccess &&
           cub::DeviceScan::ExclusiveSum(nullptr, b2, val_in, d_col_slot, (int64_t)n_dense, st) == cudaSuccess;
      if (ok && std::max(b1, b2) > tmp_bytes) {
        cudaFree(tmp);
        tmp_bytes = std::max(b1, b2);
        ok = cudaMalloc(&tmp, tmp_bytes) == cudaSuccess;
      }
      uint32_t *run_start = nullptr;
      ok = ok && cudaMalloc(reinterpret_cast<void **>(&run_start), (size_t)n_dense * 4) == cudaSuccess &&
           cub::DeviceRunLengthEncode::Encode(tmp, b1, key_out + n_res, key_in, val_in, d_runs, (int64_t)n_dense, st) ==
               cudaSuccess &&
           cudaMemcpyAsync(&n_runs, d_runs, 4, cudaMemcpyDeviceToHost, st) == cudaSuccess &&
           cudaStreamSynchronize(st) == cudaSuccess &&
           cub::DeviceScan::ExclusiveSum(tmp, b2, val_in, run_start, (int64_t)n_runs, st) == cudaSuccess;
      if (ok) {
        const unsigned rb = (unsigned)std::min<uint64_t>(((uint64_t)n_runs * 32 + 255) / 256, (uint64_t)sm_count() * 32);
        plan_cell_sum_kernel<<<rb, 256, 0, st>>>(key_in, run_start, val_in, n_runs, val_out + n_res, parts[0].weight,
                                                 n_keys, pl->dense);
        count_launch();
        ok = cudaStreamSynchronize(st) == cudaSuccess;
      }
      cudaFree(run_start);
    }
  }
  cudaFree(key_in), cudaFree(key_out), cudaFree(val_in), cudaFree(val_out), cudaFree(tmp);
  cudaFree(d_col_slot), cudaFree(d_row_slot), cudaFree(d_runs);
  return ok;
}

static nts_gather_plan *build_plan(const nts_plan_part *parts, int n_parts, nts_vid_t n_rows, nts_vid_t gather_rows,
                                   int n_slabs, int n_hub_cols, int n_hub_rows, cudaStream_t st) {
  uint64_t total = 0;
  for (int k = 0; k < n_parts; k++)
    total += parts[k].n_edges;
  if (total >= 0xffffffffull)
    return refuse_plan("plan edge count must fit uint32 offsets");
  if (n_slabs < 1 || gather_rows == 0)
    n_slabs = 1;
  if ((uint64_t)n_slabs * n_rows >= 0xffffffffull)
    return refuse_plan("slabs * rows must fit 32-bit segment keys");
  const bool hubs = gather_rows > 0 && (n_hub_cols > 0 || n_hub_rows > 0);
  if (hubs && n_parts != 1)
    return refuse_plan("hub blocks need a plan of a single part");
  nts_gather_plan *pl = new nts_gather_plan();
  pl->n_rows = n_rows;
  pl->n_edges = total;
  pl->gather_rows = gather_rows;
  pl->slabs = n_slabs;
  pl->slab_rows = gather_rows ? (gather_rows + n_slabs - 1) / n_slabs : 1;
  pl->slab_edge.assign(n_slabs + 1, 0);
  if (n_rows == 0 || total == 0)
    return pl;
  const uint32_t E = (uint32_t)total;
  nts_plan_part *d_parts = nullptr;
  bool ok = cudaMalloc(reinterpret_cast<void **>(&pl->pairs), (size_t)E * sizeof(uint2)) == cudaSuccess &&
            cudaMalloc(reinterpret_cast<void **>(&pl->voff), ((size_t)n_slabs * n_rows + 1) * 4) == cudaSuccess &&
            cudaMalloc(reinterpret_cast<void **>(&d_parts), n_parts * sizeof(nts_plan_part)) == cudaSuccess &&
            cudaMemcpyAsync(d_parts, parts, n_parts * sizeof(nts_plan_part), cudaMemcpyHostToDevice, st) == cudaSuccess;
  if (ok && n_slabs == 1 && !hubs && n_parts == 1 && parts[0].row_add == 0 && parts[0].n_rows == n_rows) {
    const unsigned blocks = (unsigned)std::min<uint64_t>(((uint64_t)E + 255) / 256, (uint64_t)sm_count() * 32);
    plan_pairs_kernel<<<blocks, 256, 0, st>>>(nullptr, d_parts, E, pl->pairs);
    count_launch();
    ok = cudaMemcpyAsync(pl->voff, parts[0].offsets, ((size_t)n_rows + 1) * 4, cudaMemcpyDeviceToDevice, st) ==
         cudaSuccess;
    pl->slab_edge[1] = E;
  } else if (ok) {
    ok = hubs ? sort_plan<uint64_t>(pl, parts, n_parts, d_parts, n_hub_cols, n_hub_rows, st)
              : sort_plan<uint32_t>(pl, parts, n_parts, d_parts, 0, 0, st);
  }
  if (ok)
    ok = cudaStreamSynchronize(st) == cudaSuccess && cudaGetLastError() == cudaSuccess;
  cudaFree(d_parts);
  if (!ok) {
    nts_gather_plan_destroy(pl);
    return refuse_plan("nts_gather_plan: device allocation or preprocessing failed");
  }
  return pl;
}

static constexpr double kHubFloor = 0.05;
static constexpr int kHubMax = 512;

nts_gather_plan *tune_plan(const nts_plan_part *parts, int n_parts, nts_vid_t n_rows, nts_vid_t gather_rows,
                           nts_vid_t feature_size, bool bf16, int run_flags, bool hubs_allowed, cudaStream_t st) {
  uint64_t n_edges = 0;
  for (int k = 0; k < n_parts; k++)
    n_edges += parts[k].n_edges;
  const uint64_t row_bytes = bf16 ? ((feature_size + 7ull) & ~7ull) * 2ull : ((feature_size + 3ull) & ~3ull) * 4ull;
  const int s_max = pick_slabs_for_rows(gather_rows, n_edges, n_rows, row_bytes, 16ull << 20);
  const char *hub_env = getenv("NTS_PLAN_HUBS");
  const bool try_hubs = hubs_allowed && !(hub_env && strcmp(hub_env, "0") == 0) && n_rows > 0 && gather_rows > 0;
  nts_gather_plan *best = build_plan(parts, n_parts, n_rows, gather_rows, 1, 0, 0, st);
  if (!best || (s_max <= 1 && !try_hubs) || n_edges == 0 || feature_size == 0)
    return best;
  float *x = nullptr, *y = nullptr;
  const size_t xb = (size_t)gather_rows * feature_size * (bf16 ? 2 : sizeof(float)),
               yb = (size_t)n_rows * feature_size * sizeof(float);
  bool ok = cudaMalloc(reinterpret_cast<void **>(&x), xb) == cudaSuccess &&
            cudaMalloc(reinterpret_cast<void **>(&y), yb) == cudaSuccess &&
            cudaMemsetAsync(x, 0, xb, st) == cudaSuccess && cudaMemsetAsync(y, 0, yb, st) == cudaSuccess;
  auto time_plan = [&](nts_gather_plan *pl, float *ms) {
    return time_min_of_two([&] {
      return bf16 ? run_plan_bf16(pl, x, NTS_DTYPE_BF16, feature_size, y, feature_size, st, run_flags)
                  : run_plan(pl, x, feature_size, y, feature_size, run_flags, st);
    }, st, ms) == 0;
  };
  float best_ms = 0.f;
  ok = ok && time_plan(best, &best_ms);
  auto consider = [&](int s, int hc, int hr, float *ms, int overlap = 0) -> int {
    nts_gather_plan *pl = build_plan(parts, n_parts, n_rows, gather_rows, s, hc, hr, st);
    if (pl)
      pl->overlap = overlap;
    if (!pl || !time_plan(pl, ms)) {
      nts_gather_plan_destroy(pl);
      return -1;
    }
    if (*ms < best_ms) {
      nts_gather_plan_destroy(best);
      best = pl;
      best_ms = *ms;
      return 1;
    }
    nts_gather_plan_destroy(pl);
    return 0;
  };
  for (int s = 2; ok && s_max > 1; s *= 2) {
    const int cand = s > s_max ? s_max : s;
    float ms = 0.f;
    const int r = consider(cand, 0, 0, &ms);
    if (r < 0 || (r == 0 && ms > 1.1f * best_ms))
      break;
    if (cand == s_max)
      break;
  }
  if (ok && try_hubs) {
    const nts_plan_part &pt = parts[0];
    std::vector<uint32_t> col_cnt, seg;
    ok = hub_counts(pt.offsets, pt.indices, pt.slot_of, pt.index_base, n_rows, (uint32_t)n_edges, gather_rows, col_cnt,
                    seg, st);
    int n_c = 0, n_r = 0;
    for (uint32_t c : col_cnt)
      n_c += c > kHubFloor * n_rows;
    for (uint32_t s : seg)
      n_r += s > kHubFloor * gather_rows;
    const int plain_slabs = best->slabs;
    float ms = 0.f;
    for (int c = 32; ok && c <= std::min(n_c, kHubMax); c *= 2)
      if (consider(best->slabs, c, 0, &ms) != 1)
        break;
    for (int r = 32; ok && r <= std::min(n_r, kHubMax); r *= 2)
      if (consider(best->slabs, best->hub_cols, r, &ms) != 1)
        break;
    if (best->hub_cols || best->hub_rows) {
      const int hc = best->hub_cols, hr = best->hub_rows;
      for (int s : {plain_slabs / 2, std::min(plain_slabs * 2, s_max)})
        if (s >= 1 && s != plain_slabs && s != best->slabs)
          consider(s, hc, hr, &ms);
    }
    const char *ov_env = getenv("NTS_PLAN_OVERLAP");
    if (ok && best->hub_rows && !(ov_env && strcmp(ov_env, "0") == 0)) {
      best->overlap = 1;
      float fused_ms = 0.f;
      if (time_plan(best, &fused_ms) && fused_ms < best_ms) {
        best_ms = fused_ms;
        for (int r = 2 * best->hub_rows; r <= std::min(n_r, kHubMax); r *= 2)
          if (consider(best->slabs, best->hub_cols, r, &ms, 1) != 1)
            break;
      } else {
        best->overlap = 0;
      }
    }
  }
  cudaFree(x), cudaFree(y);
  best->tuned_ms = best_ms;
  return best;
}

}

using namespace nts;

extern "C" {

int nts_gather_plan_pick_slabs(nts_vid_t gather_rows, uint64_t n_edges, nts_vid_t n_rows, nts_vid_t feature_size,
                               uint64_t l2_budget_bytes) {
  return pick_slabs_for_rows(gather_rows, n_edges, n_rows, ((feature_size + 3ull) & ~3ull) * 4ull, l2_budget_bytes);
}

static bool chunk_part(const nts_vid_t *offsets, const nts_vid_t *indices, const float *weight,
                       const nts_vid_t *slot_of, nts_vid_t index_base, nts_vid_t n_rows, uint64_t n_edges,
                       nts_plan_part *pt) {
  if (n_rows && n_edges && !(offsets && indices)) {
    refuse_plan("null graph array");
    return false;
  }
  *pt = {offsets, indices, weight, slot_of, index_base, 0, n_rows, 0, n_edges};
  return true;
}

nts_gather_plan *nts_gather_plan_create_hybrid(const nts_vid_t *offsets, const nts_vid_t *indices,
                                               const float *weight, const nts_vid_t *slot_of, nts_vid_t index_base,
                                               nts_vid_t n_rows, uint64_t n_edges, nts_vid_t gather_rows, int n_slabs,
                                               int n_hub_cols, int n_hub_rows, void *stream) {
  nts_plan_part pt;
  if (!chunk_part(offsets, indices, weight, slot_of, index_base, n_rows, n_edges, &pt))
    return nullptr;
  if (n_hub_cols < 0 || n_hub_rows < 0)
    return refuse_plan("negative hub count");
  return build_plan(&pt, 1, n_rows, gather_rows, n_slabs, n_hub_cols, n_hub_rows, as_stream(stream));
}

nts_gather_plan *nts_gather_plan_create_tuned_ex(const nts_vid_t *offsets, const nts_vid_t *indices,
                                                 const float *weight, const nts_vid_t *slot_of, nts_vid_t index_base,
                                                 nts_vid_t n_rows, uint64_t n_edges, nts_vid_t gather_rows,
                                                 nts_vid_t feature_size, int gather_dtype, int run_flags,
                                                 void *stream) {
  if ((gather_dtype != NTS_DTYPE_F32 && gather_dtype != NTS_DTYPE_BF16) || (run_flags & ~NTS_PLAN_OVERWRITE))
    return refuse_plan("nts_gather_plan_create_tuned_ex: gather_dtype must be NTS_DTYPE_F32 or NTS_DTYPE_BF16, "
                       "run_flags 0 or NTS_PLAN_OVERWRITE");
  nts_plan_part pt;
  if (!chunk_part(offsets, indices, weight, slot_of, index_base, n_rows, n_edges, &pt))
    return nullptr;
  return tune_plan(&pt, 1, n_rows, gather_rows, feature_size, gather_dtype == NTS_DTYPE_BF16, run_flags, true,
                   as_stream(stream));
}

nts_gather_plan *nts_gather_plan_create_parts(const nts_plan_part *parts, int n_parts, nts_vid_t n_rows,
                                              nts_vid_t gather_rows, int n_slabs, nts_vid_t feature_size, void *stream) {
  if (!parts || n_parts < 1)
    return refuse_plan("no plan parts");
  for (int k = 0; k < n_parts; k++) {
    if (parts[k].n_edges && !(parts[k].offsets && parts[k].indices))
      return refuse_plan("null graph array in a plan part");
    if ((uint64_t)parts[k].row_add + parts[k].n_rows > n_rows)
      return refuse_plan("plan part rows exceed the output rows");
  }
  if (n_slabs >= 1)
    return build_plan(parts, n_parts, n_rows, gather_rows, n_slabs, 0, 0, as_stream(stream));
  return tune_plan(parts, n_parts, n_rows, gather_rows, feature_size, false, 0, false, as_stream(stream));
}

float nts_gather_plan_tuned_ms(const nts_gather_plan *pl) { return pl ? pl->tuned_ms : 0.f; }

int nts_gather_plan_destroy(nts_gather_plan *pl) {
  if (!pl)
    return 0;
  cudaFree(pl->pairs);
  cudaFree(pl->voff);
  cudaFree(pl->workspace);
  cudaFree(pl->workspace_bf16);
  cudaFree(pl->dense);
  cudaFree(pl->hub_col_ids);
  cudaFree(pl->hub_row_ids);
  delete pl;
  return 0;
}

int nts_gather_plan_slabs(const nts_gather_plan *pl) { return pl ? pl->slabs : 0; }

int nts_gather_plan_hubs(const nts_gather_plan *pl, int *cols, int *rows) {
  NTS_ARG_CHECK(pl != nullptr, "null plan");
  if (cols)
    *cols = pl->hub_cols;
  if (rows)
    *rows = pl->hub_rows;
  return 0;
}

int nts_gather_plan_overlap(const nts_gather_plan *pl) { return pl ? pl->overlap : 0; }

int nts_gather_plan_set_overlap(nts_gather_plan *pl, int overlap) {
  NTS_ARG_CHECK(pl != nullptr, "null plan");
  NTS_ARG_CHECK(overlap == 0 || overlap == 1, "overlap must be 0 (sequential) or 1 (fused slab launches)");
  pl->overlap = overlap;
  return 0;
}

uint64_t nts_gather_plan_bytes(const nts_gather_plan *pl) {
  if (!pl)
    return 0;
  return pl->n_edges * 8ull + ((uint64_t)pl->slabs * pl->n_rows + 1) * 4ull + pl->workspace_floats * 4ull +
         pl->workspace_bf16_elems * 2ull + pl->dense_floats * 4ull + ((uint64_t)pl->hub_cols + pl->hub_rows) * 4ull;
}

int nts_gather_plan_last_launch(const nts_gather_plan *pl, int *launches, int *grid, int *k, int *u, int *outv) {
  NTS_ARG_CHECK(pl != nullptr, "null plan");
  if (launches)
    *launches = pl->last_launches;
  if (grid)
    *grid = pl->last_grid;
  if (k)
    *k = pl->last_k;
  if (u)
    *u = pl->last_u;
  if (outv)
    *outv = pl->last_outv;
  return 0;
}

int nts_gather_plan_run_ex(nts_gather_plan *pl, const float *input, nts_vid_t input_ld, float *output,
                           nts_vid_t feature_size, int flags, void *stream) {
  NTS_ARG_CHECK(input_ld >= feature_size, "input row pitch below the feature width");
  NTS_ARG_CHECK(output != nullptr || feature_size == 0, "null output pointer");
  NTS_ARG_CHECK(pl != nullptr, "null plan");
  return run_plan(pl, input, input_ld, output, feature_size, flags, as_stream(stream));
}

int nts_gather_plan_run_bf16_ex(nts_gather_plan *pl, const void *input, int input_dtype, nts_vid_t input_ld,
                                float *output, nts_vid_t feature_size, int flags, void *stream) {
  NTS_ARG_CHECK(input_ld >= feature_size, "input row pitch below the feature width");
  NTS_ARG_CHECK(output != nullptr || feature_size == 0, "null output pointer");
  NTS_ARG_CHECK(pl != nullptr, "null plan");
  return run_plan_bf16(pl, input, input_dtype, input_ld, output, feature_size, as_stream(stream), flags);
}

int nts_rows_to_bf16(const void *src, int src_dtype, nts_vid_t lds, void *dst, nts_vid_t n_rows, nts_vid_t feature_size,
                     nts_vid_t ld, void *stream) {
  NTS_ARG_CHECK((src && dst) || n_rows == 0 || feature_size == 0, "null pointer passed to nts_rows_to_bf16");
  return to_bf16_rows(src, src_dtype, lds, dst, n_rows, feature_size, ld, as_stream(stream));
}

int nts_gather_plan_set_variant(int variant) {
  NTS_ARG_CHECK(variant == 0 || variant == 1, "variant must be 0 (register staging) or 1 (TMA row staging)");
  g_plan_variant = variant;
  return 0;
}

int nts_gather_plan_set_tuning(int u, int min_blocks, int edges_per_warp) {
  NTS_ARG_CHECK(u >= 0 && min_blocks >= 0 && edges_per_warp >= 0 && edges_per_warp <= 4096, "bad tuning point");
  g_plan_u = u;
  g_plan_minb = min_blocks;
  g_plan_q = edges_per_warp;
  return 0;
}

}
```

### neutronstarlite_b200/ops.py

```python
from __future__ import annotations

import ctypes as C
import time as _time

import torch

from . import _lib
from ._lib import stream as _stream


def row_pitched(t):
    return t.dim() == 2 and (t.is_contiguous() or (t.stride(1) == 1 and t.stride(0) >= t.shape[1]))


_F32 = (torch.float32,)
_F32_BF16 = (torch.float32, torch.bfloat16)


def _check_input(t, name="input", pitched=False, dtypes=_F32):
    if not t.is_cuda:
        raise _lib.NtsError("%s must be a CUDA tensor (libnts_b200 has no CPU fallback)" % name)
    if t.dtype not in dtypes or t.dim() != 2:
        raise _lib.NtsError("%s must be a 2-D %s tensor" % (name, " or ".join(str(d)[len("torch."):] for d in dtypes)))
    if not (t.is_contiguous() or (pitched and row_pitched(t))):
        raise _lib.NtsError("%s must be contiguous" % name + (" or row-pitched" if pitched else ""))
    return t


def _check_gather_dtype(gather_dtype):
    if gather_dtype is not None and gather_dtype != torch.bfloat16:
        raise _lib.NtsError("gather_dtype must be None or torch.bfloat16, not %s" % (gather_dtype,))
    return gather_dtype


def _gathered_dtypes(gather_dtype):
    return _F32 if gather_dtype is None else _F32_BF16


_DTYPE_CODE = {torch.float32: 0, torch.bfloat16: 1}
PLAN_OVERWRITE, PLAN_COPY_INPUT = 1, 2


def _ptr(t):
    return 0 if t is None else t.data_ptr()


class KernelTimer:

    def __init__(self):
        self.records = []

    def bracket(self, tag, F, edges, rows):
        start = torch.cuda.Event(enable_timing=True)
        stop = torch.cuda.Event(enable_timing=True)
        self.records.append((tag, int(F), int(edges), int(rows), start, stop))
        return start, stop

    def summary(self):
        torch.cuda.synchronize()
        out = {}
        for tag, F, edges, rows, a, b in self.records:
            d = out.setdefault((tag, F), {"calls": 0, "ms": 0.0, "edges": 0, "rows": 0})
            d["calls"] += 1
            d["ms"] += a.elapsed_time(b)
            d["edges"] += edges
            d["rows"] += rows
        return out


_timer = None


def set_kernel_timer(timer):
    global _timer
    _timer = timer


class _timed:

    def __init__(self, tag, F, edges, rows):
        self.ev = _timer.bracket(tag, F, edges, rows) if _timer else None

    def __enter__(self):
        if self.ev:
            self.ev[0].record()

    def __exit__(self, *exc):
        if self.ev:
            self.ev[1].record()
        return False


def segment_gather_sum(out, x, weight, indices, offsets, index_base, n_rows, n_edges):
    _lib.call("nts_segment_gather_sum", _ptr(x), _ptr(out), _ptr(weight), _ptr(indices), _ptr(offsets),
              int(index_base), int(n_rows), int(n_edges), int(x.shape[1]), _stream())
    return out


class GatherPlan:

    def __init__(self, offsets, indices, weight, index_base, n_rows, n_edges, gather_rows, slabs, slot_of=None,
                 tune_for=0, hubs=(0, 0), gather_dtype=None, tune_accumulate=True):
        L = _lib.load()
        _check_gather_dtype(gather_dtype)
        t0 = _time.perf_counter()
        if slabs > 0:
            self.handle = L.nts_gather_plan_create_hybrid(_ptr(offsets), _ptr(indices), _ptr(weight), _ptr(slot_of),
                                                          int(index_base), int(n_rows), int(n_edges),
                                                          int(gather_rows), int(slabs), int(hubs[0]), int(hubs[1]),
                                                          _stream())
        else:
            self.handle = L.nts_gather_plan_create_tuned_ex(
                _ptr(offsets), _ptr(indices), _ptr(weight), _ptr(slot_of), int(index_base), int(n_rows), int(n_edges),
                int(gather_rows), int(tune_for), _DTYPE_CODE[gather_dtype or torch.float32],
                0 if tune_accumulate else PLAN_OVERWRITE, _stream())
        self.build_s = _time.perf_counter() - t0
        _lib.checked(self.handle, "gather plan construction")
        self.slabs = int(L.nts_gather_plan_slabs(self.handle))
        hc, hr = C.c_int(0), C.c_int(0)
        _lib.call("nts_gather_plan_hubs", self.handle, C.byref(hc), C.byref(hr))
        self.hub_cols, self.hub_rows = hc.value, hr.value
        self.n_rows, self.n_edges = int(n_rows), int(n_edges)

    @property
    def overlap(self):
        return bool(_lib.load().nts_gather_plan_overlap(self.handle))

    def set_overlap(self, overlap):
        _lib.call("nts_gather_plan_set_overlap", self.handle, int(bool(overlap)))

    def key(self):
        return ((self.slabs,) + ((self.hub_cols, self.hub_rows) if self.hub_cols or self.hub_rows else ())
                + (("overlap",) if self.overlap else ()))

    def run(self, x, out, gather_dtype=None, accumulate=True):
        if not row_pitched(x):
            raise _lib.NtsError("the gathered input must have contiguous rows (unit column stride)")
        F = int(x.shape[1])
        ld = F if x.is_contiguous() else int(x.stride(0))
        flags = 0 if accumulate else PLAN_OVERWRITE
        if ld != F and (x.storage_offset() + x.shape[0] * ld) * x.element_size() > x.untyped_storage().nbytes():
            flags |= PLAN_COPY_INPUT
        if _check_gather_dtype(gather_dtype) is not None:
            if x.dtype not in _DTYPE_CODE:
                raise _lib.NtsError("BF16 gathers take a float32 or bfloat16 input, not %s" % x.dtype)
            _lib.call("nts_gather_plan_run_bf16_ex", self.handle, _ptr(x), _DTYPE_CODE[x.dtype], ld, _ptr(out), F,
                      flags, _stream())
            return out
        if x.dtype == torch.bfloat16:
            raise _lib.NtsError("a bfloat16 input needs gather_dtype=torch.bfloat16")
        _lib.call("nts_gather_plan_run_ex", self.handle, _ptr(x), ld, _ptr(out), F, flags, _stream())
        return out

    def bytes(self):
        return int(_lib.load().nts_gather_plan_bytes(self.handle))

    def __del__(self):
        try:
            if getattr(self, "handle", None):
                _lib.load().nts_gather_plan_destroy(self.handle)
                self.handle = None
        except Exception:
            pass


import os as _os

PLAN_MIN_EDGES = 1 << 20
_plan_mode = {"0": "off", "1": "on"}.get(_os.environ.get("NTS_PLAN", ""), "auto")
_plan_slabs = int(_os.environ.get("NTS_PLAN_SLABS", "0"))


def set_plan_mode(mode, slabs=0):
    global _plan_mode, _plan_slabs
    if mode not in ("auto", "on", "off"):
        raise ValueError("plan mode must be auto, on or off")
    _plan_mode, _plan_slabs = mode, int(slabs)


def _chunk_direction(chunk, direction):
    if direction == "fwd":
        return (chunk.column_offset_gpu, chunk.row_indices_gpu, chunk.edge_weight_forward_gpu, chunk.src_range[0],
                chunk.batch_size_forward, chunk.batch_size_backward)
    return (chunk.row_offset_gpu, chunk.column_indices_gpu, chunk.edge_weight_backward_gpu, chunk.dst_range[0],
            chunk.batch_size_backward, chunk.batch_size_forward)


def _chunk_plan(chunk, direction, F, gather_dtype=None):
    if gather_dtype is None and (_plan_mode == "off" or (_plan_mode == "auto" and chunk.edge_size < PLAN_MIN_EDGES)):
        return None
    plans = chunk.__dict__.setdefault("_gather_plans", {})
    tuned = chunk.__dict__.setdefault("_gather_plan_for", {})
    key = (direction, _plan_slabs) if _plan_slabs else (direction, "F", int(F))
    if gather_dtype is not None and not _plan_slabs:
        key += ("bf16",)
    plan = plans.get(key) if _plan_slabs else tuned.get(key)
    if plan is None:
        offsets, indices, weight, index_base, n_rows, gather_rows = _chunk_direction(chunk, direction)
        plan = GatherPlan(offsets, indices, weight, index_base, n_rows, chunk.edge_size, gather_rows, _plan_slabs,
                          tune_for=int(F), gather_dtype=gather_dtype, tune_accumulate=False)
        share = (direction,) + plan.key()
        if share in plans:
            plan = plans[share]
        plans[share] = plan
        if not _plan_slabs:
            tuned[key] = plan
    return plan


def _bf16_plan(chunk, direction, F, with_weight, gather_dtype):
    if _check_gather_dtype(gather_dtype) is None:
        return _chunk_plan(chunk, direction, F) if with_weight else None
    if not with_weight:
        raise _lib.NtsError("BF16 gathers always apply the edge weights (with_weight=True)")
    return _chunk_plan(chunk, direction, F, gather_dtype)


def _plain_operands(out, x, accumulate):
    if not accumulate:
        out.zero_()
    return x.contiguous()


def _gather_chunk(direction, chunk, out, x, with_weight, gather_dtype, accumulate):
    plan = _bf16_plan(chunk, direction, x.shape[1], with_weight, gather_dtype)
    offsets, indices, weight, _, n_rows, _ = _chunk_direction(chunk, direction)
    with _timed(direction, x.shape[1], chunk.edge_size, n_rows):
        if plan is not None:
            return plan.run(x, out, gather_dtype, accumulate)
        x = _plain_operands(out, x, accumulate)
        entry, a, b = (("nts_gather_by_dst_from_src", indices, offsets) if direction == "fwd" else
                       ("nts_gather_by_src_from_dst", offsets, indices))
        _lib.call(entry, _ptr(x), _ptr(out), _ptr(weight), _ptr(a), _ptr(b), chunk.src_range[0], chunk.src_range[1],
                  chunk.dst_range[0], chunk.dst_range[1], chunk.edge_size, n_rows, int(x.shape[1]),
                  1 if with_weight else 0, _stream())
    return out


def gather_by_dst_from_src(chunk, out, x, with_weight=True, gather_dtype=None, accumulate=True):
    return _gather_chunk("fwd", chunk, out, x, with_weight, gather_dtype, accumulate)


def gather_by_src_from_dst(chunk, out, grad, with_weight=True, gather_dtype=None, accumulate=True):
    return _gather_chunk("bwd", chunk, out, grad, with_weight, gather_dtype, accumulate)


class ntsGraphOp:

    def __init__(self, partitioned_graph, active=None):
        self.partitioned_graph_ = partitioned_graph
        self.active_ = active

    def forward(self, f_input, f_input1=None):
        raise NotImplementedError

    def backward(self, output_grad):
        raise NotImplementedError

    def get_additional_grad(self):
        raise NotImplementedError("get_additional_grad is not implemented")


class ForwardSingleGPUfuseOp(ntsGraphOp):

    def __init__(self, partitioned_graph, active=None, gather_dtype=None):
        super().__init__(partitioned_graph, active)
        self.gather_dtype = _check_gather_dtype(gather_dtype)

    def forward(self, f_input, f_input1=None):
        x = _check_input(f_input, "input", True, _gathered_dtypes(self.gather_dtype))
        c = self.partitioned_graph_.graph_chunks[0]
        y = torch.empty((c.batch_size_forward, x.shape[1]), dtype=torch.float32, device=x.device)
        return gather_by_dst_from_src(c, y, x, gather_dtype=self.gather_dtype, accumulate=False)

    def backward(self, f_output_grad):
        g = _check_input(f_output_grad, "output_grad", pitched=True)
        c = self.partitioned_graph_.graph_chunks[0]
        dx = torch.empty((c.batch_size_backward, g.shape[1]), dtype=torch.float32, device=g.device)
        return gather_by_src_from_dst(c, dx, g, gather_dtype=self.gather_dtype, accumulate=False)


class MiniBatchFuseOp(ntsGraphOp):

    def __init__(self, sampled_subgraph, hop, table=False, gather_dtype=None):
        super().__init__(sampled_subgraph, None)
        self.block = sampled_subgraph.blocks[hop]
        self.hop, self.table = int(hop), bool(table)
        self.gather_dtype = _check_gather_dtype(gather_dtype)
        self.vertices = getattr(sampled_subgraph, "vertices", None)
        if self.table and (self.block.row_global is None or self.vertices is None):
            raise _lib.NtsError("table=True needs the block's global source ids (row_global) and the graph's vertex "
                                "count (SampledSubgraph.vertices)")

    def forward(self, f_input, f_input1=None):
        b = self.block
        if self.gather_dtype is None:
            x = _check_input(f_input, "input")
        else:
            x = _check_bf16_operand(_check_input(f_input, "input", True, _F32_BF16), "input")
        if self.table and x.shape[0] < self.vertices:
            raise _lib.NtsError("the feature table has %d rows, the sampled graph has %d vertices"
                                % (x.shape[0], self.vertices))
        if not self.table and x.shape[0] != b.n_src:
            raise _lib.NtsError("input has %d rows, hop %d has %d sources" % (x.shape[0], self.hop, b.n_src))
        y = torch.zeros((b.n_dst, x.shape[1]), dtype=torch.float32, device=x.device)
        idx = b.row_global if self.table else b.row_indices
        return self._k1(y, x, b.weight, idx, b.column_offset, b.n_dst, "minibatch_fwd")

    def backward(self, f_output_grad):
        if self.table:
            raise _lib.NtsError("a table gather (table=True) has no backward")
        g = _check_input(f_output_grad, "output_grad")
        b = self.block
        if g.shape[0] != b.n_dst:
            raise _lib.NtsError("output_grad has %d rows, hop %d has %d destinations" % (g.shape[0], self.hop, b.n_dst))
        dx = torch.zeros((b.n_src, g.shape[1]), dtype=torch.float32, device=g.device)
        return self._k1(dx, g, b.weight_backward, b.column_indices, b.row_offset, b.n_src, "minibatch_bwd")

    def _k1(self, out, x, weight, indices, offsets, n_rows, tag):
        n_edges = self.block.n_edges
        if self.gather_dtype is None:
            with _timed(tag, x.shape[1], n_edges, n_rows):
                return segment_gather_sum(out, x, weight, indices, offsets, 0, n_rows, n_edges)
        r = _bf16_rows(x, "minibatch_bf16_round")
        return segment_gather_sum_bf16(out, (r, int(r.stride(0))), weight, indices, offsets, n_rows, n_edges,
                                       tag + "_bf16")


def _check_bf16_operand(t, name):
    if t.dtype == torch.bfloat16 and (t.stride(0) % 8 != 0 or t.data_ptr() % 16 != 0):
        raise _lib.NtsError("a bfloat16 %s needs rows of a pitch that is a multiple of 8 values (e.g. a [:, :F] view "
                            "of [n, 8*ceil(F/8)] rows), 16-byte aligned; got pitch %d" % (name, t.stride(0)))
    return t


def _bf16_rows(t, tag, ld=None):
    if t.dtype == torch.bfloat16:
        return t
    n, F = t.shape
    ld = (F + 7) // 8 * 8 if ld is None else int(ld)
    r = torch.empty((n, ld), dtype=torch.bfloat16, device=t.device)
    with _timed(tag, F, 0, n):
        _lib.call("nts_rows_to_bf16", _ptr(t), _DTYPE_CODE[torch.float32], int(t.stride(0)), _ptr(r), n, F, ld,
                  _stream())
    return r


def segment_gather_sum_bf16(out, rows, weight, indices, offsets, n_rows, n_edges, tag="segment_gather_sum_bf16"):
    x, ld = rows
    with _timed(tag, out.shape[1], n_edges, n_rows):
        _lib.call("nts_segment_gather_sum_bf16", _ptr(x), ld, _ptr(out), _ptr(weight), _ptr(indices), _ptr(offsets),
                  int(n_rows), int(n_edges), int(out.shape[1]), _stream())
    return out


class ForwardGPUfuseOp(ntsGraphOp):

    def __init__(self, partitioned_graph, active=None, exchange=None, gather_dtype=None):
        super().__init__(partitioned_graph, active)
        self.gather_dtype = _check_gather_dtype(gather_dtype)
        if exchange is None:
            from .exchange import default_exchange
            exchange = default_exchange(partitioned_graph)
        self.exchange = exchange

    def forward(self, f_input, f_input1=None):
        x = _check_input(f_input, "input", dtypes=_gathered_dtypes(self.gather_dtype))
        if self.gather_dtype is None:
            return self.exchange.forward(x)
        return self.exchange.forward(x, gather_dtype=self.gather_dtype)

    def backward(self, f_output_grad):
        g = _check_input(f_output_grad, "output_grad")
        if self.gather_dtype is None:
            return self.exchange.backward(g)
        return self.exchange.backward(g, gather_dtype=self.gather_dtype)


class _EdgeOp(ntsGraphOp):
    def _topo(self):
        pg = self.partitioned_graph_
        if pg.column_offset_gpu is None or pg.row_indices_gpu is None:
            raise _lib.NtsError("whole-partition CSC missing: call PartitionedGraph.generate_all(dist=True, device=...)")
        return pg


class DistGPUGetDepNbrOp(ntsGraphOp):

    def __init__(self, partitioned_graph, active=None, exchange=None):
        super().__init__(partitioned_graph, active)
        if exchange is None:
            from .exchange import default_exchange
            exchange = default_exchange(partitioned_graph)
        self.exchange = exchange

    def forward(self, f_input, f_input1=None):
        return self.exchange.fetch_mirrors(_check_input(f_input))

    def backward(self, f_output_grad):
        return self.exchange.return_mirror_grads(_check_input(f_output_grad, "output_grad"))


class DistGPUScatterSrc(_EdgeOp):

    def forward(self, f_input, f_input1=None):
        pg = self._topo()
        x = _check_input(f_input)
        msg = torch.zeros((pg.owned_edges, x.shape[1]), dtype=torch.float32, device=x.device)
        _lib.call("nts_scatter_src_mirror_to_msg", _ptr(msg), _ptr(x), _ptr(pg.row_indices_gpu),
                  _ptr(pg.column_offset_gpu), _ptr(pg.mirror_index_gpu), pg.owned_vertices, x.shape[1], _stream())
        return msg

    def backward(self, f_output_grad):
        pg = self._topo()
        g = _check_input(f_output_grad, "output_grad")
        out = torch.zeros((pg.owned_mirrors, g.shape[1]), dtype=torch.float32, device=g.device)
        _lib.call("nts_gather_msg_to_src_mirror", _ptr(out), _ptr(g), _ptr(pg.row_indices_gpu),
                  _ptr(pg.column_offset_gpu), _ptr(pg.mirror_index_gpu), pg.owned_vertices, g.shape[1], _stream())
        return out


class DistGPUScatterDst(_EdgeOp):

    def forward(self, f_input, f_input1=None):
        pg = self._topo()
        x = _check_input(f_input)
        msg = torch.zeros((pg.owned_edges, x.shape[1]), dtype=torch.float32, device=x.device)
        _lib.call("nts_scatter_dst_to_msg", _ptr(msg), _ptr(x), _ptr(pg.row_indices_gpu),
                  _ptr(pg.column_offset_gpu), pg.owned_vertices, x.shape[1], _stream())
        return msg

    def backward(self, f_output_grad):
        pg = self._topo()
        g = _check_input(f_output_grad, "output_grad")
        out = torch.zeros((pg.owned_vertices, g.shape[1]), dtype=torch.float32, device=g.device)
        _lib.call("nts_gather_msg_to_dst", _ptr(out), _ptr(g), _ptr(pg.row_indices_gpu),
                  _ptr(pg.column_offset_gpu), pg.owned_vertices, g.shape[1], _stream())
        return out


class DistGPUAggregateDst(_EdgeOp):

    def forward(self, f_input, f_input1=None):
        pg = self._topo()
        m = _check_input(f_input)
        out = torch.zeros((pg.owned_vertices, m.shape[1]), dtype=torch.float32, device=m.device)
        _lib.call("nts_gather_msg_to_dst", _ptr(out), _ptr(m), _ptr(pg.row_indices_gpu),
                  _ptr(pg.column_offset_gpu), pg.owned_vertices, m.shape[1], _stream())
        return out

    def backward(self, f_output_grad):
        pg = self._topo()
        g = _check_input(f_output_grad, "output_grad")
        msg = torch.zeros((pg.owned_edges, g.shape[1]), dtype=torch.float32, device=g.device)
        _lib.call("nts_scatter_dst_to_msg", _ptr(msg), _ptr(g), _ptr(pg.row_indices_gpu),
                  _ptr(pg.column_offset_gpu), pg.owned_vertices, g.shape[1], _stream())
        return msg


class DistGPUEdgeSoftMax(_EdgeOp):

    def __init__(self, partitioned_graph, active=None):
        super().__init__(partitioned_graph, active)
        self.IntermediateResult = None

    def forward(self, f_input, f_input1=None):
        pg = self._topo()
        m = _check_input(f_input)
        out = torch.zeros_like(m)
        self.IntermediateResult = torch.zeros_like(m)
        _lib.call("nts_edge_softmax_forward", _ptr(out), _ptr(m), _ptr(self.IntermediateResult),
                  _ptr(pg.row_indices_gpu), _ptr(pg.column_offset_gpu), pg.owned_vertices, m.shape[1], _stream())
        return out

    def backward(self, f_output_grad):
        pg = self._topo()
        g = _check_input(f_output_grad, "output_grad")
        out = torch.zeros_like(g)
        _lib.call("nts_edge_softmax_backward", _ptr(out), _ptr(g), _ptr(self.IntermediateResult),
                  _ptr(pg.row_indices_gpu), _ptr(pg.column_offset_gpu), pg.owned_vertices, g.shape[1], _stream())
        return out


class DistGPUAggregateDstFuseWeight(_EdgeOp):

    def __init__(self, partitioned_graph, active=None):
        super().__init__(partitioned_graph, active)
        self._mirror = None
        self._a = None
        self.e_weight_grad = None

    def forward(self, f_input, e_weight=None):
        pg = self._topo()
        x = _check_input(f_input)
        a = _check_input(e_weight, "edge weight")
        self._mirror, self._a = x, a
        heads = int(a.shape[1])
        out = torch.zeros((pg.owned_vertices, x.shape[1]), dtype=torch.float32, device=x.device)
        _lib.call("nts_segment_gather_sum_heads", _ptr(x), _ptr(out), _ptr(a), _ptr(pg.row_indices_gpu),
                  _ptr(pg.column_offset_gpu), _ptr(pg.mirror_index_gpu), 0, pg.owned_vertices, pg.owned_edges,
                  x.shape[1], heads, _stream())
        return out

    def backward(self, f_output_grad):
        pg = self._topo()
        g = _check_input(f_output_grad, "output_grad")
        dm = torch.zeros((pg.owned_mirrors, g.shape[1]), dtype=torch.float32, device=g.device)
        self.e_weight_grad = torch.zeros_like(self._a)
        _lib.call("nts_aggregate_dst_fuse_weight_backward_heads", _ptr(dm), _ptr(self.e_weight_grad),
                  _ptr(self._mirror), _ptr(self._a), _ptr(g), _ptr(pg.row_indices_gpu), _ptr(pg.column_offset_gpu),
                  _ptr(pg.mirror_index_gpu), pg.owned_vertices, g.shape[1], int(self._a.shape[1]), _stream())
        return dm

    def get_additional_grad(self):
        return self.e_weight_grad


class _FusedGAT:

    def __init__(self, column_offset, slots, n_dst, n_src, n_edges, slope, gather_dtype):
        self.column_offset, self.slots = column_offset, slots
        self.n_dst, self.n_src, self.n_edges = int(n_dst), int(n_src), int(n_edges)
        self.slope, self.gather_dtype = slope, gather_dtype
        self.saved = None

    def forward(self, x, s, d):
        H, F = int(s.shape[1]), int(x.shape[1])
        seg_max = torch.empty((self.n_dst, H), dtype=torch.float32, device=x.device)
        seg_sum = torch.empty_like(seg_max)
        with _timed("gat_stats", F, self.n_edges, self.n_dst):
            _lib.call("nts_gat_softmax_stats", _ptr(seg_max), _ptr(seg_sum), _ptr(s), _ptr(d), _ptr(self.slots),
                      _ptr(self.column_offset), 0, self.n_dst, H, self.slope, _stream())
        if self.gather_dtype is None:
            ld = (F + 3) // 4 * 4 if H == 1 else F
            rows = x if ld == F else torch.nn.functional.pad(x, (0, ld - F))
            entry, widths = "nts_gat_fused_aggregate_forward", (ld,)
        else:
            ld = (F + 7) // 8 * 8
            rows = self._to_bf16_rows(x, ld)
            entry, widths = "nts_gat_fused_aggregate_forward_bf16", (F, ld)
        out = torch.zeros((self.n_dst, ld), dtype=torch.float32, device=x.device)
        with _timed("gat_fwd", F, self.n_edges, self.n_dst):
            _lib.call(entry, _ptr(rows), _ptr(out), _ptr(s), _ptr(d), _ptr(seg_max), _ptr(seg_sum), _ptr(self.slots),
                      _ptr(self.column_offset), 0, self.n_dst, self.n_edges, *widths, H, self.slope, _stream())
        if ld != F:
            out = out[:, :F].contiguous()
        self.saved = (x if self.gather_dtype is None else rows, s, d, seg_max, seg_sum, out)
        return out

    @staticmethod
    def _to_bf16_rows(t, ld):
        return _bf16_rows(t, "gat_bf16_round", ld)

    def _grads(self, g):
        rows, s, d, _, _, out = self.saved
        H, F = int(s.shape[1]), int(out.shape[1])
        o = out.detach()
        out_dot_g = (o * (g if g.dtype == torch.float32 else g[:, :F].float())).view(-1, H, F // H).sum(-1).contiguous()
        if rows.dtype == torch.float32:
            dm = torch.zeros_like(rows)
        else:
            dm = torch.zeros(rows.shape, dtype=torch.float32, device=g.device)
        return out_dot_g, dm, torch.zeros_like(s), torch.zeros_like(d)

    def backward_two_pass(self, g, slot_off, slot_dst):
        rows, s, d, seg_max, seg_sum, out = self.saved
        H, F = int(s.shape[1]), int(out.shape[1])
        if self.gather_dtype is None:
            gk, entry, widths = g, "nts_gat_fused_aggregate_backward_two_pass", (F,)
        else:
            gk = self._to_bf16_rows(g, rows.shape[1])
            entry, widths = "nts_gat_fused_aggregate_backward_two_pass_bf16", (F, int(rows.shape[1]))
        out_dot_g, dm, ds, dd = self._grads(gk)
        pack = torch.empty((self.n_dst, H, 4), dtype=torch.float32, device=g.device)
        with _timed("gat_bwd", F, 2 * self.n_edges, self.n_dst):
            _lib.call(entry, _ptr(dm), _ptr(ds), _ptr(dd), _ptr(pack), _ptr(rows), _ptr(s), _ptr(d), _ptr(seg_max),
                      _ptr(seg_sum), _ptr(out_dot_g), _ptr(gk), _ptr(self.slots), _ptr(self.column_offset), 0,
                      _ptr(slot_off), _ptr(slot_dst), self.n_dst, rows.shape[0], *widths, H, self.slope, _stream())
        if dm.shape[1] != F:
            dm = dm[:, :F].contiguous()
        return dm, ds, dd

    def backward_one_pass(self, g, row_indices, mirror_index):
        x, s, d, seg_max, seg_sum, out = self.saved
        out_dot_g, dm, ds, dd = self._grads(g)
        _lib.call("nts_gat_fused_aggregate_backward", _ptr(dm), _ptr(ds), _ptr(dd), _ptr(x), _ptr(s), _ptr(d),
                  _ptr(seg_max), _ptr(seg_sum), _ptr(out_dot_g), _ptr(g), _ptr(row_indices), _ptr(self.column_offset),
                  _ptr(mirror_index), self.n_dst, x.shape[1], int(s.shape[1]), self.slope, _stream())
        return dm, ds, dd


class DistGPUFusedGATOp(_EdgeOp):

    def __init__(self, partitioned_graph, active=None, negative_slope=0.2, two_pass_backward=True, gather_dtype=None):
        super().__init__(partitioned_graph, active)
        self.slope = float(negative_slope)
        self.two_pass_backward = bool(two_pass_backward)
        self.gather_dtype = _check_gather_dtype(gather_dtype)
        if self.gather_dtype is not None and not self.two_pass_backward:
            raise _lib.NtsError("BF16 gathers of the fused GAT layer need two_pass_backward=True")
        self._k7 = None

    @staticmethod
    def slot_indices(pg):
        cached = getattr(pg, "_slot_indices_gpu", None)
        if cached is None:
            cached = pg.mirror_index_gpu[pg.row_indices_gpu.long()].to(torch.int32).contiguous()
            pg._slot_indices_gpu = cached
        return cached

    @staticmethod
    def slot_csr(pg):
        cached = getattr(pg, "_slot_csr_gpu", None)
        if cached is not None:
            return cached
        col = pg.column_offset_gpu.long()
        V, M = pg.owned_vertices, pg.owned_mirrors
        slot = DistGPUFusedGATOp.slot_indices(pg).long()
        dst = torch.repeat_interleave(torch.arange(V, device=col.device), col[1:V + 1] - col[:V])
        order = torch.sort(slot, stable=True).indices
        csr_dst = dst[order].to(torch.int32).contiguous()
        off = torch.zeros(M + 1, dtype=torch.int64, device=col.device)
        off[1:] = torch.cumsum(torch.bincount(slot, minlength=M), 0)
        pg._slot_csr_gpu = (off.to(torch.int32).contiguous(), csr_dst)
        return pg._slot_csr_gpu

    def forward(self, mirror, src_score, dst_score):
        pg = self._topo()
        x = _check_input(mirror, "mirror")
        s = _check_input(src_score, "src_score")
        d = _check_input(dst_score, "dst_score")
        self._k7 = _FusedGAT(pg.column_offset_gpu, self.slot_indices(pg), pg.owned_vertices, x.shape[0],
                             pg.owned_edges, self.slope, self.gather_dtype)
        return self._k7.forward(x, s, d)

    @property
    def _saved(self):
        return None if self._k7 is None else self._k7.saved

    def backward(self, f_output_grad):
        pg = self._topo()
        g = _check_input(f_output_grad, "output_grad")
        if self.two_pass_backward:
            return self._k7.backward_two_pass(g, *self.slot_csr(pg))
        return self._k7.backward_one_pass(g, pg.row_indices_gpu, pg.mirror_index_gpu)


BF16_HEAD_WIDTH_ERROR = ("BF16 rows with heads > 1 need a head width D % 8 == 0 (a 16-byte chunk never straddles two "
                         "heads) and ld == feature_size")


def gat_bf16_shape_error(feature_size, heads):
    F, H = int(feature_size), int(heads)
    ld = (F + 7) // 8 * 8
    lib = _lib.load()
    for name, n_ptrs in (("nts_gat_fused_aggregate_forward_bf16", 9),
                         ("nts_gat_fused_aggregate_backward_two_pass_bf16", 16)):
        if getattr(lib, name)(*([None] * n_ptrs), 0, 0, F, ld, H, 0.2, None) != 0:
            return "%s: %s" % (name, _lib.last_error())
    return None


class MiniBatchGATOp(ntsGraphOp):

    def __init__(self, sampled_subgraph, hop, negative_slope=0.2, gather_dtype=None):
        super().__init__(sampled_subgraph, None)
        self.hop = int(hop)
        self.block = sampled_subgraph.blocks[self.hop]
        if self.block.dst_pos is None:
            raise _lib.NtsError("MiniBatchGATOp needs a block whose sources include its destinations (dst_pos): "
                                "sample with NeighborSampler(..., include_dst=True)")
        self.slope = float(negative_slope)
        self.gather_dtype = _check_gather_dtype(gather_dtype)
        self._k7 = None

    def forward(self, x_trans, src_score, dst_score):
        b = self.block
        x = _check_input(x_trans, "x_trans")
        s = _check_input(src_score, "src_score")
        d = _check_input(dst_score, "dst_score")
        if x.shape[0] != b.n_src or s.shape[0] != b.n_src:
            raise _lib.NtsError("x_trans and src_score need %d rows (hop %d sources), got %d and %d"
                                % (b.n_src, self.hop, x.shape[0], s.shape[0]))
        if d.shape[0] != b.n_dst:
            raise _lib.NtsError("dst_score needs %d rows (hop %d destinations), got %d"
                                % (b.n_dst, self.hop, d.shape[0]))
        H, F = int(s.shape[1]), int(x.shape[1])
        if d.shape[1] != H or H < 1 or F % H != 0:
            raise _lib.NtsError("scores need the same head count, and x_trans a width that is a multiple of it")
        if b.n_edges == 0:
            if self.gather_dtype is not None and H > 1 and (F // H) % 8 != 0:
                raise _lib.NtsError(BF16_HEAD_WIDTH_ERROR)
            self._shapes = (x, s, d)
            return torch.zeros((b.n_dst, F), dtype=torch.float32, device=x.device)
        self._k7 = _FusedGAT(b.column_offset, b.row_indices, b.n_dst, b.n_src, b.n_edges, self.slope,
                             self.gather_dtype)
        return self._k7.forward(x, s, d)

    def backward(self, f_output_grad):
        b = self.block
        g = _check_input(f_output_grad, "output_grad")
        if g.shape[0] != b.n_dst:
            raise _lib.NtsError("output_grad has %d rows, hop %d has %d destinations" % (g.shape[0], self.hop, b.n_dst))
        if self._k7 is None:
            x, s, d = self._shapes
            return torch.zeros_like(x), torch.zeros_like(s), torch.zeros_like(d)
        return self._k7.backward_two_pass(g, b.row_offset, b.column_indices)
```

Baseline: 16.17 billion.

## Add L2-sized 2D tiles for cold-source edges of warm rows in gather plan

Adds a new plan class that regroups residual (non-hub) edges whose destination is a 'warm' row and whose source is a cold column. These edges go into extra L2 tiles, with source columns bucketed into L2-sized chunks and outputs wrapped back by row modulo. A separate tiled kernel launch runs these edges with atomic flushes, aiming to keep both the source rows and the accumulated outputs resident in L2. The autotuner explores tile sizes unless NTS_PLAN_TILES=0. The trade-offs are extra launches, atomic output writes, a larger segment-offset array and a longer plan build.

```diff
diff --git a/include/nts_b200.h b/include/nts_b200.h
--- a/include/nts_b200.h
+++ b/include/nts_b200.h
@@ -69,6 +69,11 @@
                                                const float *weight, const nts_vid_t *slot_of, nts_vid_t index_base,
                                                nts_vid_t n_rows, uint64_t n_edges, nts_vid_t gather_rows, int n_slabs,
                                                int n_hub_cols, int n_hub_rows, void *stream);
+nts_gather_plan *nts_gather_plan_create_tiled(const nts_vid_t *offsets, const nts_vid_t *indices, const float *weight,
+                                              const nts_vid_t *slot_of, nts_vid_t index_base, nts_vid_t n_rows,
+                                              uint64_t n_edges, nts_vid_t gather_rows, int n_slabs, int n_hub_cols,
+                                              int n_hub_rows, nts_vid_t tile_hot, nts_vid_t tile_warm,
+                                              nts_vid_t tile_rows, void *stream);
 nts_gather_plan *nts_gather_plan_create_tuned_ex(const nts_vid_t *offsets, const nts_vid_t *indices,
                                                  const float *weight, const nts_vid_t *slot_of, nts_vid_t index_base,
                                                  nts_vid_t n_rows, uint64_t n_edges, nts_vid_t gather_rows,
@@ -88,6 +93,7 @@
 int nts_gather_plan_slabs(const nts_gather_plan *plan);
 int nts_gather_plan_hubs(const nts_gather_plan *plan, int *cols, int *rows);
 int nts_gather_plan_overlap(const nts_gather_plan *plan);
+int nts_gather_plan_tiles(const nts_gather_plan *plan, int *tiles, uint64_t *tile_edges, uint64_t *slab_edges);
 int nts_gather_plan_set_overlap(nts_gather_plan *plan, int overlap);
 uint64_t nts_gather_plan_bytes(const nts_gather_plan *plan);
 enum { NTS_PLAN_ACCUMULATE = 0, NTS_PLAN_OVERWRITE = 1, NTS_PLAN_COPY_INPUT = 2 };
diff --git a/neutronstarlite_b200/_lib.py b/neutronstarlite_b200/_lib.py
--- a/neutronstarlite_b200/_lib.py
+++ b/neutronstarlite_b200/_lib.py
@@ -56,6 +56,9 @@
                                          _u64, _u64, _u32, _u32, C.c_float, _vp]),
     "nts_gather_plan_pick_slabs": (_int, [_u32, _u64, _u32, _u32, _u64]),
     "nts_gather_plan_create_hybrid": (_vp, [_vp, _vp, _vp, _vp, _u32, _u32, _u64, _u32, _int, _int, _int, _vp]),
+    "nts_gather_plan_create_tiled": (_vp, [_vp, _vp, _vp, _vp, _u32, _u32, _u64, _u32, _int, _int, _int, _u32, _u32,
+                                         _u32, _vp]),
+    "nts_gather_plan_tiles": (_int, [_vp, C.POINTER(_int), C.POINTER(_u64), C.POINTER(_u64)]),
     "nts_gather_plan_create_parts": (_vp, [_vp, _int, _u32, _u32, _int, _u32, _vp]),
     "nts_gather_plan_tuned_ms": (C.c_float, [_vp]),
     "nts_gather_plan_destroy": (_int, [_vp]),
diff --git a/neutronstarlite_b200/csrc/nts_plan.cu b/neutronstarlite_b200/csrc/nts_plan.cu
--- a/neutronstarlite_b200/csrc/nts_plan.cu
+++ b/neutronstarlite_b200/csrc/nts_plan.cu
@@ -27,6 +27,8 @@
   float *dense = nullptr;
   size_t dense_floats = 0;
   int overlap = 0;
+  int l2_tiles = 0;
+  uint32_t tile_hot = 0, tile_warm = 0, tile_rows = 0;
   int last_grid = 0, last_launches = 0, last_k = 0, last_u = 0, last_outv = 0;
   float tuned_ms = 0.f;
 };
@@ -44,18 +46,24 @@
 
 template <class KeyT>
 __global__ void plan_keys_kernel(nts_plan_part pt, uint32_t e_off, uint32_t n_rows, uint32_t slab_rows, uint32_t slabs,
-                                 const uint32_t *__restrict__ col_slot, const uint32_t *__restrict__ row_slot,
-                                 uint32_t lda_c, uint64_t dc_cells, uint32_t lda_r, KeyT *__restrict__ key,
-                                 uint32_t *__restrict__ val) {
+                                 uint32_t l2_tiles, const uint32_t *__restrict__ tile_of,
+                                 const uint8_t *__restrict__ warm, const uint32_t *__restrict__ col_slot,
+                                 const uint32_t *__restrict__ row_slot, uint32_t lda_c, uint64_t dc_cells,
+                                 uint32_t lda_r, KeyT *__restrict__ key, uint32_t *__restrict__ val) {
   for (uint64_t e = (uint64_t)blockIdx.x * blockDim.x + threadIdx.x; e < pt.n_edges; e += (uint64_t)gridDim.x * blockDim.x) {
     const uint32_t r = find_row(pt.offsets, pt.n_rows, (uint32_t)e) + pt.row_add;
     const uint32_t g = plan_gathered_row(pt, (uint32_t)e);
     uint32_t s = g / slab_rows;
     if (s >= slabs)
       s = slabs - 1;
+    if (tile_of) {
+      const uint32_t t = __ldg(tile_of + g);
+      if (t != kNoHub && __ldg(warm + r))
+        s = slabs + t;
+    }
     KeyT k = (KeyT)s * n_rows + r;
     if constexpr (sizeof(KeyT) == 8) {
-      const uint64_t n_keys = (uint64_t)slabs * n_rows;
+      const uint64_t n_keys = (uint64_t)(slabs + l2_tiles) * n_rows;
       const uint32_t cs = __ldg(col_slot + g), rs = __ldg(row_slot + r);
       if (cs != kNoHub)
         k = n_keys + (uint64_t)cs * lda_c + r;
@@ -100,6 +108,19 @@
   for (uint64_t e = (uint64_t)blockIdx.x * blockDim.x + threadIdx.x; e < n_edges; e += (uint64_t)gridDim.x * blockDim.x) {
     const uint32_t id = __ldg(idx + e);
     atomicAdd(cnt + (slot_of ? __ldg(slot_of + id) : id - base), 1u);
+  }
+}
+
+__global__ void plan_residual_count_kernel(nts_plan_part pt, const uint32_t *__restrict__ col_slot,
+                                           const uint32_t *__restrict__ row_slot, uint32_t *__restrict__ src_cnt,
+                                           uint32_t *__restrict__ row_len) {
+  for (uint64_t e = (uint64_t)blockIdx.x * blockDim.x + threadIdx.x; e < pt.n_edges; e += (uint64_t)gridDim.x * blockDim.x) {
+    const uint32_t r = find_row(pt.offsets, pt.n_rows, (uint32_t)e);
+    const uint32_t g = plan_gathered_row(pt, (uint32_t)e);
+    if ((col_slot && __ldg(col_slot + g) != kNoHub) || (row_slot && __ldg(row_slot + r) != kNoHub))
+      continue;
+    atomicAdd(src_cnt + g, 1u);
+    atomicAdd(row_len + r, 1u);
   }
 }
 
@@ -221,13 +242,13 @@
   }
 };
 
-template <class T, int K, int U, int OUTV, int G>
+template <class T, int K, int U, int OUTV, int G, bool WRAP = false>
 __device__ __forceinline__ void planned_gather_body(unsigned char *smem_raw, uint32_t vblock,
                                                     const typename GatherT<T>::chunk *__restrict__ in, uint32_t ldc,
                                                     float *__restrict__ out, uint32_t F,
                                                     const uint2 *__restrict__ pairs, const uint32_t *__restrict__ off,
                                                     uint32_t n_rows, uint32_t e_begin, uint32_t e_end, uint32_t Q,
-                                                    uint32_t tiles, uint32_t tile_vecs) {
+                                                    uint32_t tiles, uint32_t tile_vecs, uint32_t out_rows = 0) {
   static_assert(G == 1 || K == 1, "virtual warps are for rows narrower than a warp");
   using Chunk = typename GatherT<T>::chunk;
   constexpr int V = GatherT<T>::V;
@@ -290,7 +311,7 @@
       acc[k][j] = 0.f;
 
   auto flush = [&](bool whole) {
-    float *orow = out + (size_t)row * F;
+    float *orow = out + (size_t)(WRAP ? row % out_rows : row) * F;
 #pragma unroll
     for (int k = 0; k < K; k++) {
 #pragma unroll
@@ -298,7 +319,7 @@
         const uint32_t col = (c0 + k * GS) * V + h;
         const float4 a = make_float4(acc[k][h], acc[k][h + 1], acc[k][h + 2], acc[k][h + 3]);
         if (act[k] && col < F) {
-          if (whole)
+          if (whole && !WRAP)
             flush_chunk<OUTV, false>(orow, col, F, a);
           else
             flush_chunk<OUTV, true>(orow, col, F, a);
@@ -381,6 +402,17 @@
   extern __shared__ __align__(16) unsigned char smem_raw[];
   planned_gather_body<T, K, U, OUTV, G>(smem_raw, blockIdx.x, in, ldc, out, F, pairs, off, n_rows, e_begin, e_end, Q,
                                         tiles, tile_vecs);
+}
+
+template <class T, int K, int U, int OUTV, int MINB, int G = 1>
+__global__ void __launch_bounds__(kPlanWarps * 32, MINB)
+    planned_tiles_kernel(const typename GatherT<T>::chunk *__restrict__ in, uint32_t ldc, float *__restrict__ out,
+                         uint32_t F, const uint2 *__restrict__ pairs, const uint32_t *__restrict__ off,
+                         uint32_t n_segs, uint32_t e_begin, uint32_t e_end, uint32_t Q, uint32_t tiles,
+                         uint32_t tile_vecs, uint32_t out_rows) {
+  extern __shared__ __align__(16) unsigned char smem_raw[];
+  planned_gather_body<T, K, U, OUTV, G, true>(smem_raw, blockIdx.x, in, ldc, out, F, pairs, off, n_segs, e_begin,
+                                              e_end, Q, tiles, tile_vecs, out_rows);
 }
 
 struct PlanShape;
@@ -519,7 +551,12 @@
 struct PlanShape {
   int k, u, outv, minb, g;
   uint32_t tiles, tile_vecs;
+  uint32_t l2_q;
 };
+
+template <class T, int K, int U, int OUTV, int MINB, int G>
+static int launch_tiles(nts_gather_plan *pl, const PlanShape &sh, const T *in_rows, uint32_t ldc, float *out,
+                        uint32_t F, cudaStream_t st);
 
 template <class T, int K, int U, int OUTV, int MINB, int G = 1>
 static int launch_planned(nts_gather_plan *pl, const PlanShape &sh, const T *in_rows, uint32_t ldc, float *out,
@@ -543,6 +580,29 @@
     pl->last_grid = (int)blocks;
     pl->last_launches++;
   }
+  return launch_tiles<T, K, U, OUTV, MINB, G>(pl, sh, in_rows, ldc, out, F, st);
+}
+
+template <class T, int K, int U, int OUTV, int MINB, int G>
+static int launch_tiles(nts_gather_plan *pl, const PlanShape &sh, const T *in_rows, uint32_t ldc, float *out,
+                        uint32_t F, cudaStream_t st) {
+  const uint64_t eb = pl->slab_edge[pl->slabs], ee = pl->slab_edge[pl->slabs + pl->l2_tiles];
+  if (ee <= eb)
+    return 0;
+  auto kern = planned_tiles_kernel<T, K, U, OUTV, MINB, G>;
+  const auto *in = reinterpret_cast<const typename GatherT<T>::chunk *>(in_rows);
+  const uint32_t Q = sh.l2_q;
+  const size_t smem = 16 + ((size_t)kPlanWarps * G * Q + 4) * 8;
+  NTS_CUDA_OK(cudaFuncSetAttribute(kern, cudaFuncAttributeMaxDynamicSharedMemorySize, (int)smem));
+  const uint64_t blocks = (((ee - eb + Q - 1) / Q) * sh.tiles + kPlanWarps * G - 1) / (kPlanWarps * G);
+  NTS_ARG_CHECK(blocks <= 0x7fffffffull, "aggregation grid too large");
+  kern<<<(unsigned)blocks, kPlanWarps * 32, smem, st>>>(in, ldc, out, F, pl->pairs,
+                                                        pl->voff + (size_t)pl->slabs * pl->n_rows,
+                                                        (uint32_t)pl->l2_tiles * pl->n_rows, (uint32_t)eb,
+                                                        (uint32_t)ee, Q, sh.tiles, sh.tile_vecs, pl->n_rows);
+  NTS_LAUNCH_CHECK();
+  pl->last_grid = (int)blocks;
+  pl->last_launches++;
   return 0;
 }
 
@@ -556,7 +616,7 @@
   NTS_ARG_CHECK(smem <= 227 * 1024, "row-staging ring does not fit shared memory");
   NTS_CUDA_OK(cudaFuncSetAttribute(kern, cudaFuncAttributeMaxDynamicSharedMemorySize, (int)smem));
   pl->last_launches = 0;
-  for (int s = 0; s < pl->slabs; s++) {
+  for (int s = 0; s < pl->slabs + pl->l2_tiles; s++) {
     const uint64_t eb = pl->slab_edge[s], ee = pl->slab_edge[s + 1];
     if (ee <= eb)
       continue;
@@ -836,7 +896,7 @@
     pl->last_grid = (int)blocks;
     pl->last_launches++;
   }
-  return 0;
+  return launch_tiles<T, K, U, OUTV, MINB, G>(pl, sh, in_rows, ldc, out, F, st);
 }
 
 #define NTS_PLAN_FUSED_CASE(K_, U_, B_, G_)                                                                         \
@@ -893,16 +953,18 @@
     if (g_plan_minb > 0)
       sh.minb = g_plan_minb;
   }
-  uint32_t Q = g_plan_q > 0 ? (uint32_t)g_plan_q : 512u / sh.g;
-  if (g_plan_q <= 0) {
-    const uint64_t per_slab = pl->slab_edge[pl->slabs] / (uint64_t)pl->slabs + 1;
-    const uint64_t want_warps = (uint64_t)sm_count() * 64 * sh.g;
-    while (Q > 32 && ((per_slab + Q - 1) / Q) * sh.tiles < want_warps)
-      Q >>= 1;
-  }
-  Q = (Q + 31u) & ~31u;
-  if (Q * sh.g > 1024)
-    Q = (1024 / sh.g) & ~31u;
+  auto quantum = [&](uint64_t per_launch) {
+    uint32_t q = g_plan_q > 0 ? (uint32_t)g_plan_q : 512u / sh.g;
+    if (g_plan_q <= 0) {
+      const uint64_t want_warps = (uint64_t)sm_count() * 64 * sh.g;
+      while (q > 32 && ((per_launch + q - 1) / q) * sh.tiles < want_warps)
+        q >>= 1;
+    }
+    q = (q + 31u) & ~31u;
+    return q * sh.g > 1024 ? (1024 / sh.g) & ~31u : q;
+  };
+  const uint32_t Q = quantum(pl->slab_edge[pl->slabs] / (uint64_t)pl->slabs + 1);
+  sh.l2_q = quantum(pl->slab_edge[pl->slabs + pl->l2_tiles] - pl->slab_edge[pl->slabs] + 1);
   pl->last_k = sh.k, pl->last_u = sh.u, pl->last_outv = sh.outv;
   float *out = output;
   if (fused) {
@@ -1129,14 +1191,50 @@
   return nullptr;
 }
 
+static bool pick_tiles(nts_gather_plan *pl, const nts_plan_part &pt, const uint32_t *d_col_slot,
+                       const uint32_t *d_row_slot, uint32_t **tile_of, uint8_t **warm, cudaStream_t st) {
+  const uint32_t n_rows = pl->n_rows, G = pl->gather_rows;
+  uint32_t *cnt = nullptr;
+  std::vector<uint32_t> src_cnt(G), row_len(n_rows);
+  bool ok = cudaMalloc(reinterpret_cast<void **>(&cnt), ((size_t)G + n_rows) * 4) == cudaSuccess &&
+            cudaMemsetAsync(cnt, 0, ((size_t)G + n_rows) * 4, st) == cudaSuccess;
+  if (ok) {
+    const unsigned blocks = (unsigned)std::min<uint64_t>((pt.n_edges + 255) / 256, (uint64_t)sm_count() * 32);
+    plan_residual_count_kernel<<<blocks, 256, 0, st>>>(pt, d_col_slot, d_row_slot, cnt, cnt + G);
+    count_launch();
+  }
+  ok = ok && cudaMemcpyAsync(src_cnt.data(), cnt, (size_t)G * 4, cudaMemcpyDeviceToHost, st) == cudaSuccess &&
+       cudaMemcpyAsync(row_len.data(), cnt + G, (size_t)n_rows * 4, cudaMemcpyDeviceToHost, st) == cudaSuccess &&
+       cudaStreamSynchronize(st) == cudaSuccess;
+  cudaFree(cnt);
+  if (!ok)
+    return false;
+  std::vector<uint32_t> tile(G, kNoHub);
+  std::vector<uint8_t> is_warm(n_rows, 0);
+  for (uint32_t g : top_ids(src_cnt, pl->tile_hot))
+    src_cnt[g] = 0;
+  uint32_t cold = 0;
+  for (uint32_t g = 0; g < G; g++)
+    if (src_cnt[g])
+      tile[g] = cold++ / pl->tile_rows;
+  for (uint32_t r : top_ids(row_len, pl->tile_warm))
+    is_warm[r] = row_len[r] > 0;
+  pl->l2_tiles = (int)((cold + pl->tile_rows - 1) / pl->tile_rows);
+  return cudaMalloc(reinterpret_cast<void **>(tile_of), (size_t)G * 4 + 4) == cudaSuccess &&
+         cudaMalloc(reinterpret_cast<void **>(warm), (size_t)n_rows + 4) == cudaSuccess &&
+         cudaMemcpyAsync(*tile_of, tile.data(), (size_t)G * 4, cudaMemcpyHostToDevice, st) == cudaSuccess &&
+         cudaMemcpyAsync(*warm, is_warm.data(), n_rows, cudaMemcpyHostToDevice, st) == cudaSuccess &&
+         cudaStreamSynchronize(st) == cudaSuccess;
+}
+
 template <class KeyT>
 static bool sort_plan(nts_gather_plan *pl, const nts_plan_part *parts, int n_parts, const nts_plan_part *d_parts,
                       int n_hub_cols, int n_hub_rows, cudaStream_t st) {
   constexpr bool hubs = sizeof(KeyT) == 8;
   const uint32_t E = (uint32_t)pl->n_edges, n_rows = pl->n_rows, G = pl->gather_rows;
-  const uint64_t n_keys = (uint64_t)pl->slabs * n_rows;
   uint64_t dc_cells = 0;
-  uint32_t *d_col_slot = nullptr, *d_row_slot = nullptr, *d_runs = nullptr;
+  uint32_t *d_col_slot = nullptr, *d_row_slot = nullptr, *d_runs = nullptr, *d_tile_of = nullptr;
+  uint8_t *d_warm = nullptr;
   bool ok = true;
   if (hubs) {
     const nts_plan_part &pt = parts[0];
@@ -1167,6 +1265,16 @@
          cudaMemcpyAsync(d_row_slot, row_slot.data(), (size_t)n_rows * 4, cudaMemcpyHostToDevice, st) == cudaSuccess &&
          cudaMemsetAsync(pl->dense, 0, pl->dense_floats * 4, st) == cudaSuccess;
   }
+  if (ok && pl->tile_rows)
+    ok = pick_tiles(pl, parts[0], d_col_slot, d_row_slot, &d_tile_of, &d_warm, st);
+  const uint64_t n_keys = (uint64_t)(pl->slabs + pl->l2_tiles) * n_rows;
+  if (ok && n_keys >= 0xffffffffull) {
+    cudaFree(d_col_slot), cudaFree(d_row_slot), cudaFree(d_runs), cudaFree(d_tile_of), cudaFree(d_warm);
+    fail(-1, "(slabs + tiles) * rows must fit 32-bit segment offsets", __FILE__, __LINE__);
+    return false;
+  }
+  pl->slab_edge.assign(pl->slabs + pl->l2_tiles + 1, 0);
+  ok = ok && cudaMalloc(reinterpret_cast<void **>(&pl->voff), ((size_t)n_keys + 1) * 4) == cudaSuccess;
   int bits = 1;
   while (bits < (int)(8 * sizeof(KeyT)) && (1ull << bits) < n_keys + pl->dense_floats)
     bits++;
@@ -1187,8 +1295,9 @@
     if (!pt.n_edges)
       continue;
     const unsigned blocks = (unsigned)std::min<uint64_t>((pt.n_edges + 255) / 256, (uint64_t)sm_count() * 32);
-    plan_keys_kernel<KeyT><<<blocks, 256, 0, st>>>(pt, e_off, n_rows, pl->slab_rows, (uint32_t)pl->slabs, d_col_slot,
-                                                   d_row_slot, pl->lda_c, dc_cells, pl->lda_r, key_in, val_in);
+    plan_keys_kernel<KeyT><<<blocks, 256, 0, st>>>(pt, e_off, n_rows, pl->slab_rows, (uint32_t)pl->slabs,
+                                                   (uint32_t)pl->l2_tiles, d_tile_of, d_warm, d_col_slot, d_row_slot,
+                                                   pl->lda_c, dc_cells, pl->lda_r, key_in, val_in);
     count_launch();
     e_off += (uint32_t)pt.n_edges;
   }
@@ -1198,14 +1307,15 @@
     const unsigned kb = (unsigned)std::min<uint64_t>((n_keys + 256) / 256, (uint64_t)sm_count() * 32);
     plan_offsets_kernel<KeyT><<<kb, 256, 0, st>>>(key_out, E, (uint32_t)n_keys, pl->voff);
     count_launch();
-    std::vector<uint32_t> h(pl->slabs + 1);
+    const int ranges = pl->slabs + pl->l2_tiles;
+    std::vector<uint32_t> h(ranges + 1);
     ok = cudaStreamSynchronize(st) == cudaSuccess;
-    for (int s = 0; s <= pl->slabs && ok; s++)
+    for (int s = 0; s <= ranges && ok; s++)
       ok = cudaMemcpy(&h[s], pl->voff + (size_t)s * n_rows, 4, cudaMemcpyDeviceToHost) == cudaSuccess;
-    for (int s = 0; s <= pl->slabs; s++)
+    for (int s = 0; s <= ranges; s++)
       pl->slab_edge[s] = h[s];
   }
-  const uint32_t n_res = (uint32_t)pl->slab_edge[pl->slabs], n_dense = E - n_res;
+  const uint32_t n_res = (uint32_t)pl->slab_edge[pl->slabs + pl->l2_tiles], n_dense = E - n_res;
   if (ok && n_res) {
     const unsigned blocks = (unsigned)std::min<uint64_t>(((uint64_t)n_res + 255) / 256, (uint64_t)sm_count() * 32);
     plan_pairs_kernel<<<blocks, 256, 0, st>>>(val_out, d_parts, n_res, pl->pairs);
@@ -1241,12 +1351,17 @@
     }
   }
   cudaFree(key_in), cudaFree(key_out), cudaFree(val_in), cudaFree(val_out), cudaFree(tmp);
-  cudaFree(d_col_slot), cudaFree(d_row_slot), cudaFree(d_runs);
+  cudaFree(d_col_slot), cudaFree(d_row_slot), cudaFree(d_runs), cudaFree(d_tile_of), cudaFree(d_warm);
   return ok;
 }
 
+struct TileCounts {
+  uint32_t hot = 0, warm = 0, rows = 0;
+};
+
 static nts_gather_plan *build_plan(const nts_plan_part *parts, int n_parts, nts_vid_t n_rows, nts_vid_t gather_rows,
-                                   int n_slabs, int n_hub_cols, int n_hub_rows, cudaStream_t st) {
+                                   int n_slabs, int n_hub_cols, int n_hub_rows, cudaStream_t st,
+                                   TileCounts tc = TileCounts()) {
   uint64_t total = 0;
   for (int k = 0; k < n_parts; k++)
     total += parts[k].n_edges;
@@ -1259,6 +1374,9 @@
   const bool hubs = gather_rows > 0 && (n_hub_cols > 0 || n_hub_rows > 0);
   if (hubs && n_parts != 1)
     return refuse_plan("hub blocks need a plan of a single part");
+  const bool tiled = gather_rows > 0 && tc.rows > 0 && tc.warm > 0;
+  if (tiled && n_parts != 1)
+    return refuse_plan("L2 tiles need a plan of a single part");
   nts_gather_plan *pl = new nts_gather_plan();
   pl->n_rows = n_rows;
   pl->n_edges = total;
@@ -1266,20 +1384,22 @@
   pl->slabs = n_slabs;
   pl->slab_rows = gather_rows ? (gather_rows + n_slabs - 1) / n_slabs : 1;
   pl->slab_edge.assign(n_slabs + 1, 0);
+  if (tiled)
+    pl->tile_hot = tc.hot, pl->tile_warm = tc.warm, pl->tile_rows = tc.rows;
   if (n_rows == 0 || total == 0)
     return pl;
   const uint32_t E = (uint32_t)total;
   nts_plan_part *d_parts = nullptr;
   bool ok = cudaMalloc(reinterpret_cast<void **>(&pl->pairs), (size_t)E * sizeof(uint2)) == cudaSuccess &&
-            cudaMalloc(reinterpret_cast<void **>(&pl->voff), ((size_t)n_slabs * n_rows + 1) * 4) == cudaSuccess &&
             cudaMalloc(reinterpret_cast<void **>(&d_parts), n_parts * sizeof(nts_plan_part)) == cudaSuccess &&
             cudaMemcpyAsync(d_parts, parts, n_parts * sizeof(nts_plan_part), cudaMemcpyHostToDevice, st) == cudaSuccess;
-  if (ok && n_slabs == 1 && !hubs && n_parts == 1 && parts[0].row_add == 0 && parts[0].n_rows == n_rows) {
+  if (ok && n_slabs == 1 && !hubs && !tiled && n_parts == 1 && parts[0].row_add == 0 && parts[0].n_rows == n_rows) {
     const unsigned blocks = (unsigned)std::min<uint64_t>(((uint64_t)E + 255) / 256, (uint64_t)sm_count() * 32);
     plan_pairs_kernel<<<blocks, 256, 0, st>>>(nullptr, d_parts, E, pl->pairs);
     count_launch();
-    ok = cudaMemcpyAsync(pl->voff, parts[0].offsets, ((size_t)n_rows + 1) * 4, cudaMemcpyDeviceToDevice, st) ==
-         cudaSuccess;
+    ok = cudaMalloc(reinterpret_cast<void **>(&pl->voff), ((size_t)n_rows + 1) * 4) == cudaSuccess &&
+         cudaMemcpyAsync(pl->voff, parts[0].offsets, ((size_t)n_rows + 1) * 4, cudaMemcpyDeviceToDevice, st) ==
+             cudaSuccess;
     pl->slab_edge[1] = E;
   } else if (ok) {
     ok = hubs ? sort_plan<uint64_t>(pl, parts, n_parts, d_parts, n_hub_cols, n_hub_rows, st)
@@ -1297,6 +1417,7 @@
 
 static constexpr double kHubFloor = 0.05;
 static constexpr int kHubMax = 512;
+static constexpr uint64_t kTileHotBytes = 50ull << 20, kTileSlabBytes = 48ull << 20;
 
 nts_gather_plan *tune_plan(const nts_plan_part *parts, int n_parts, nts_vid_t n_rows, nts_vid_t gather_rows,
                            nts_vid_t feature_size, bool bf16, int run_flags, bool hubs_allowed, cudaStream_t st) {
@@ -1324,8 +1445,8 @@
   };
   float best_ms = 0.f;
   ok = ok && time_plan(best, &best_ms);
-  auto consider = [&](int s, int hc, int hr, float *ms, int overlap = 0) -> int {
-    nts_gather_plan *pl = build_plan(parts, n_parts, n_rows, gather_rows, s, hc, hr, st);
+  auto consider = [&](int s, int hc, int hr, float *ms, int overlap = 0, TileCounts tc = TileCounts()) -> int {
+    nts_gather_plan *pl = build_plan(parts, n_parts, n_rows, gather_rows, s, hc, hr, st, tc);
     if (pl)
       pl->overlap = overlap;
     if (!pl || !time_plan(pl, ms)) {
@@ -1388,6 +1509,30 @@
       }
     }
   }
+  const char *tile_env = getenv("NTS_PLAN_TILES");
+  if (ok && hubs_allowed && n_rows > 0 && gather_rows > 0 && !(tile_env && strcmp(tile_env, "0") == 0)) {
+    const uint64_t out_row_bytes = ((feature_size + 3ull) & ~3ull) * 4ull;
+    TileCounts tc;
+    tc.hot = (uint32_t)std::min<uint64_t>(kTileHotBytes / row_bytes, gather_rows);
+    tc.rows = (uint32_t)std::max<uint64_t>(kTileSlabBytes / row_bytes, 1);
+    float ms = 0.f;
+    const int s = best->slabs, hc = best->hub_cols, hr = best->hub_rows, ov = best->overlap;
+    for (uint64_t mb = 12; mb <= 48; mb *= 2) {
+      tc.warm = (uint32_t)std::min<uint64_t>((mb << 20) / out_row_bytes, n_rows);
+      if (consider(s, hc, hr, &ms, ov, tc) != 1)
+        break;
+    }
+    if (best->l2_tiles) {
+      TileCounts b{best->tile_hot, best->tile_warm, best->tile_rows};
+      for (uint32_t rows : {b.rows / 2, b.rows * 2})
+        if (rows >= 1 && consider(s, hc, hr, &ms, ov, TileCounts{b.hot, b.warm, rows}) == 1)
+          break;
+      b = TileCounts{best->tile_hot, best->tile_warm, best->tile_rows};
+      for (uint32_t hot : {b.hot / 2, std::min<uint32_t>(b.hot * 2, gather_rows)})
+        if (hot != b.hot && consider(s, hc, hr, &ms, ov, TileCounts{hot, b.warm, b.rows}) == 1)
+          break;
+    }
+  }
   cudaFree(x), cudaFree(y);
   best->tuned_ms = best_ms;
   return best;
@@ -1425,6 +1570,21 @@
   if (n_hub_cols < 0 || n_hub_rows < 0)
     return refuse_plan("negative hub count");
   return build_plan(&pt, 1, n_rows, gather_rows, n_slabs, n_hub_cols, n_hub_rows, as_stream(stream));
+}
+
+nts_gather_plan *nts_gather_plan_create_tiled(const nts_vid_t *offsets, const nts_vid_t *indices, const float *weight,
+                                              const nts_vid_t *slot_of, nts_vid_t index_base, nts_vid_t n_rows,
+                                              uint64_t n_edges, nts_vid_t gather_rows, int n_slabs, int n_hub_cols,
+                                              int n_hub_rows, nts_vid_t tile_hot, nts_vid_t tile_warm,
+                                              nts_vid_t tile_rows, void *stream) {
+  nts_plan_part pt;
+  if (!chunk_part(offsets, indices, weight, slot_of, index_base, n_rows, n_edges, &pt))
+    return nullptr;
+  if (n_hub_cols < 0 || n_hub_rows < 0)
+    return refuse_plan("negative hub count");
+  TileCounts tc;
+  tc.hot = tile_hot, tc.warm = tile_warm, tc.rows = tile_rows;
+  return build_plan(&pt, 1, n_rows, gather_rows, n_slabs, n_hub_cols, n_hub_rows, as_stream(stream), tc);
 }
 
 nts_gather_plan *nts_gather_plan_create_tuned_ex(const nts_vid_t *offsets, const nts_vid_t *indices,
@@ -1486,6 +1646,19 @@
 
 int nts_gather_plan_overlap(const nts_gather_plan *pl) { return pl ? pl->overlap : 0; }
 
+int nts_gather_plan_tiles(const nts_gather_plan *pl, int *tiles, uint64_t *tile_edges, uint64_t *slab_edges) {
+  NTS_ARG_CHECK(pl != nullptr, "null plan");
+  const int s = pl->slabs, t = pl->l2_tiles;
+  const bool built = pl->slab_edge.size() == (size_t)(s + t + 1);
+  if (tiles)
+    *tiles = t;
+  if (tile_edges)
+    *tile_edges = built ? pl->slab_edge[s + t] - pl->slab_edge[s] : 0;
+  if (slab_edges)
+    *slab_edges = built ? pl->slab_edge[s] : 0;
+  return 0;
+}
+
 int nts_gather_plan_set_overlap(nts_gather_plan *pl, int overlap) {
   NTS_ARG_CHECK(pl != nullptr, "null plan");
   NTS_ARG_CHECK(overlap == 0 || overlap == 1, "overlap must be 0 (sequential) or 1 (fused slab launches)");
@@ -1496,7 +1669,7 @@
 uint64_t nts_gather_plan_bytes(const nts_gather_plan *pl) {
   if (!pl)
     return 0;
-  return pl->n_edges * 8ull + ((uint64_t)pl->slabs * pl->n_rows + 1) * 4ull + pl->workspace_floats * 4ull +
+  return pl->n_edges * 8ull + ((uint64_t)(pl->slabs + pl->l2_tiles) * pl->n_rows + 1) * 4ull + pl->workspace_floats * 4ull +
          pl->workspace_bf16_elems * 2ull + pl->dense_floats * 4ull + ((uint64_t)pl->hub_cols + pl->hub_rows) * 4ull;
 }
 
diff --git a/neutronstarlite_b200/ops.py b/neutronstarlite_b200/ops.py
--- a/neutronstarlite_b200/ops.py
+++ b/neutronstarlite_b200/ops.py
@@ -100,15 +100,15 @@
 class GatherPlan:
 
     def __init__(self, offsets, indices, weight, index_base, n_rows, n_edges, gather_rows, slabs, slot_of=None,
-                 tune_for=0, hubs=(0, 0), gather_dtype=None, tune_accumulate=True):
+                 tune_for=0, hubs=(0, 0), gather_dtype=None, tune_accumulate=True, tiles=(0, 0, 0)):
         L = _lib.load()
         _check_gather_dtype(gather_dtype)
         t0 = _time.perf_counter()
         if slabs > 0:
-            self.handle = L.nts_gather_plan_create_hybrid(_ptr(offsets), _ptr(indices), _ptr(weight), _ptr(slot_of),
-                                                          int(index_base), int(n_rows), int(n_edges),
-                                                          int(gather_rows), int(slabs), int(hubs[0]), int(hubs[1]),
-                                                          _stream())
+            self.handle = L.nts_gather_plan_create_tiled(_ptr(offsets), _ptr(indices), _ptr(weight), _ptr(slot_of),
+                                                         int(index_base), int(n_rows), int(n_edges), int(gather_rows),
+                                                         int(slabs), int(hubs[0]), int(hubs[1]), int(tiles[0]),
+                                                         int(tiles[1]), int(tiles[2]), _stream())
         else:
             self.handle = L.nts_gather_plan_create_tuned_ex(
                 _ptr(offsets), _ptr(indices), _ptr(weight), _ptr(slot_of), int(index_base), int(n_rows), int(n_edges),
@@ -120,6 +120,9 @@
         hc, hr = C.c_int(0), C.c_int(0)
         _lib.call("nts_gather_plan_hubs", self.handle, C.byref(hc), C.byref(hr))
         self.hub_cols, self.hub_rows = hc.value, hr.value
+        t, te, se = C.c_int(0), C.c_uint64(0), C.c_uint64(0)
+        _lib.call("nts_gather_plan_tiles", self.handle, C.byref(t), C.byref(te), C.byref(se))
+        self.l2_tiles, self.tile_edges, self.slab_edges = t.value, te.value, se.value
         self.n_rows, self.n_edges = int(n_rows), int(n_edges)
 
     @property
@@ -131,7 +134,8 @@
 
     def key(self):
         return ((self.slabs,) + ((self.hub_cols, self.hub_rows) if self.hub_cols or self.hub_rows else ())
-                + (("overlap",) if self.overlap else ()))
+                + (("overlap",) if self.overlap else ())
+                + (("tiles", self.l2_tiles, self.tile_edges) if self.l2_tiles else ()))
 
     def run(self, x, out, gather_dtype=None, accumulate=True):
         if not row_pitched(x):
```

Result: no change. 16.17 billion (median of 6 runs) (-0.0%).
